# Kuuro-neko/HAI719-Raytracing

Measured on AMD Instinct MI355X. Metric: Msamples/s (pixels x spp / s), Cornell+mesh 1080p@256spp, higher is better.
Workload: dtype f32

## Files before the change

hai719-raytracing_amd/__init__.py:

```python
from __future__ import annotations

import ctypes as C
import os
from typing import Optional

import numpy as np

_HERE = os.path.dirname(os.path.abspath(__file__))
REPO_ROOT = os.path.dirname(_HERE)
ASSET_ROOT = os.path.join(REPO_ROOT, "assets")
TILE = 8

FLAG_GAMMA = 1
FLAG_NO_LDS_TREE = 2
FLAG_WAVE_KERNEL = 4
FLAG_STREAM_KERNEL = 8
FLAG_NO_SHADOW_CULL = 16
FLAG_DUAL_KERNEL = 32
FLAG_EXACT_ONLY = 64
FLAG_MESH_BRUTE = 128

MAT_DIFFUSE, MAT_GLASS, MAT_MIRROR = 0, 1, 2
TEX_NONE, TEX_CHECKER, TEX_IMAGE = 0, 1, 2

# ... 309 lines not shown
        self._check(self._lib.hrt_host_scene_set_skybox(self._h, a.shape[1], a.shape[0], a.ctypes.data))

    def set_sky(self, dark: bool):
        self._check(self._lib.hrt_host_scene_set_sky(self._h, int(dark)))

    def set_kd_params(self, leaf_max: int = 0, max_depth: int = 0):
        self._check(self._lib.hrt_host_scene_set_kd_params(self._h, leaf_max, max_depth))

    def set_kd_builder(self, fn=None, user=None):
        if fn == "gpu":
            fn = C.cast(device_lib().hrt_kd_build_gpu, C.c_void_p)
        elif fn is not None and not isinstance(fn, (int, C.c_void_p)):
            self._kd_builder_keepalive = fn
            fn = C.cast(fn, C.c_void_p)
        self._check(self._lib.hrt_host_scene_set_kd_builder(self._h, fn, user))
        return self

    def flatten(self) -> C.c_void_p:
        d = SceneDescPtr()
        self._check(self._lib.hrt_host_scene_flatten(self._h, C.byref(d)))
        d._owner = self
        return d

    def kd_stats(self, mesh: int = 0) -> dict:
        out = (C.c_uint32 * 6)()
        self._check(self._lib.hrt_host_scene_kd_stats(self._h, mesh, out))
        keys = ["inner", "leaves", "empty_leaves", "depth", "leaf_tri_refs", "units"]
        return dict(zip(keys, list(out)))


def _irregular_stats(self, mesh: int = 0) -> dict:
    out = (C.c_uint32 * 8)()
    self._check(self._lib.hrt_host_scene_irregular_stats(self._h, mesh, out))
    return dict(zip(["out_of_tree", "slivers", "dropped", "pairs", "ref_leaves", "ref_depth", "dead", "entries"], list(out)))


HostScene.irregular_stats = _irregular_stats


def default_camera(aspect: float) -> Camera:
    cam = Camera()
    host_lib().hrt_host_default_camera(aspect, C.byref(cam))
    return cam


_inited = False


def init(device: int = 0):
    global _inited
    lib = device_lib()
    rc = lib.hrt_init(device)
    if rc < 0:
        raise HrtError(f"hrt_init({device}) failed ({rc}): {lib.hrt_last_error().decode()}")
    _inited = True


class DeviceScene:

    def __init__(self, desc: C.c_void_p):
        self._lib = device_lib()
        if not _inited:
            init(int(os.environ.get("LOCAL_RANK", "0")))
        self._h = C.c_void_p()
        self._check(self._lib.hrt_scene_create(desc, C.byref(self._h)))

    def _check(self, rc: int):
        if rc < 0:
            raise HrtError(f"hrt error {rc}: {self._lib.hrt_last_error().decode()}")
        return rc

    def close(self):
        if self._h:
            self._lib.hrt_scene_destroy(self._h)
            self._h = C.c_void_p()

    def __del__(self):
        try:
            self.close()
        except Exception:
            pass

    def render(self, cam: Camera, w: int, h: int, spp: int, seed: int = 1, flags: int = 0):
        out = np.empty((h, w, 3), dtype=np.float32)
        st = Stats()
        self._check(self._lib.hrt_render(self._h, C.byref(cam), w, h, spp, seed, flags, out.ctypes.data, C.byref(st)))
        return out, st

    def last_kernel(self) -> str:
        name = C.create_string_buffer(64)
        self._check(self._lib.hrt_debug_last_kernel(self._h, name, len(name)))
        return name.value.decode()

    def render_tiles(self, cam: Camera, w: int, h: int, spp: int, seed: int, flags: int, rank: int, world: int,
                     d_tiles_ptr: int, stream_ptr: int = 0):
        self._check(self._lib.hrt_render_tiles(self._h, C.byref(cam), w, h, spp, seed, flags, rank, world,
                                               C.c_void_p(d_tiles_ptr), C.c_void_p(stream_ptr)))

    def render_accumulate(self, cam: Camera, w: int, h: int, first_sample: int, n_samples: int, seed: int, flags: int,
                          rank: int, world: int, d_sum_tiles_ptr: int, stream_ptr: int = 0):
        self._check(self._lib.hrt_render_accumulate(self._h, C.byref(cam), w, h, first_sample, n_samples, seed, flags, rank,
                                                    world, C.c_void_p(d_sum_tiles_ptr), C.c_void_p(stream_ptr)))

    def render_adaptive(self, cam: Camera, w: int, h: int, min_spp: int, max_spp: int, threshold: float, seed: int = 1,
                        flags: int = 0, stats: Optional[Stats] = None):
        out = np.empty((h, w, 3), dtype=np.float32)
        spp = np.empty(((h + TILE - 1) // TILE, (w + TILE - 1) // TILE), dtype=np.uint32)
        p = Adaptive(min_spp, max_spp, threshold)
        self._check(self._lib.hrt_render_adaptive(self._h, C.byref(cam), w, h, C.byref(p), seed, flags, out.ctypes.data,
                                                   spp.ctypes.data, None if stats is None else C.byref(stats)))
        return out, spp

    def render_adaptive_tiles(self, cam: Camera, w: int, h: int, min_spp: int, max_spp: int, threshold: float, seed: int,
                              flags: int, rank: int, world: int, d_tiles_ptr: int, d_tile_spp_ptr: int, stream_ptr: int = 0):
        p = Adaptive(min_spp, max_spp, threshold)
        self._check(self._lib.hrt_render_adaptive_tiles(self._h, C.byref(cam), w, h, C.byref(p), seed, flags, rank, world,
                                                        C.c_void_p(d_tiles_ptr), C.c_void_p(d_tile_spp_ptr), C.c_void_p(stream_ptr)))

    def render_features(self, cam: Camera, w: int, h: int, first_sample: int, n_samples: int, seed: int = 1) -> np.ndarray:
        import torch
        d = torch.empty((h, w, FEATURE_FLOATS), dtype=torch.float32, device="cuda")
        s = torch.cuda.current_stream()
        self._check(self._lib.hrt_render_features(self._h, C.byref(cam), w, h, first_sample, n_samples, seed, C.c_void_p(d.data_ptr()),
                                                  C.c_void_p(s.cuda_stream)))
        s.synchronize()
        return d.cpu().numpy()

    def render_denoised(self, cam: Camera, w: int, h: int, spp: int, feature_spp: int, seed: int = 1, flags: int = 0,
                        params: Optional[DenoiseParams] = None, stats: Optional[Stats] = None) -> np.ndarray:
        out = np.empty((h, w, 3), dtype=np.float32)
        p = DenoiseParams() if params is None else params
        self._check(self._lib.hrt_render_denoised(self._h, C.byref(cam), w, h, spp, feature_spp, seed, flags, C.byref(p), out.ctypes.data,
                                                  None if stats is None else C.byref(stats)))
        return out

    def render_denoised_var(self, cam: Camera, w: int, h: int, spp: int, feature_spp: int, seed: int = 1, flags: int = 0,
                            params: Optional[DenoiseVarParams] = None, stats: Optional[Stats] = None, variance: bool = False):
        out = np.empty((h, w, 3), dtype=np.float32)
        var = np.empty((h, w), dtype=np.float32) if variance else None
        p = DenoiseVarParams() if params is None else params
        self._check(self._lib.hrt_render_denoised_var(self._h, C.byref(cam), w, h, spp, feature_spp, seed, flags, C.byref(p),
                                                      out.ctypes.data, None if var is None else var.ctypes.data,
                                                      None if stats is None else C.byref(stats)))
        return (out, var) if variance else out

    def render_temporal(self, history: "History", cam: Camera, w: int, h: int, spp: int, feature_spp: int, seed: int = 1, flags: int = 0,
                        tparams: Optional[TemporalParams] = None, dparams: Optional[DenoiseVarParams] = None,
                        stats: Optional[Stats] = None):
        out = np.empty((h, w, 3), dtype=np.float32)
        hist = np.empty((h, w), dtype=np.float32)
        tp = TemporalParams() if tparams is None else tparams
        self._check(self._lib.hrt_render_temporal(self._h, history._h, C.byref(cam), w, h, spp, feature_spp, seed, flags, C.byref(tp),
                                                  None if dparams is None else C.byref(dparams), out.ctypes.data, hist.ctypes.data,
                                                  None if stats is None else C.byref(stats)))
        return out, hist

    def trace_rays(self, rays, mode: str = "closest", flags: int = 0, normalize: bool = False):
        import torch
        if mode not in _QUERY_MODES:
            raise ValueError(f"trace_rays: mode must be one of {sorted(_QUERY_MODES)} (got {mode!r})")
        q = _QUERY_MODES[mode]
        flags = int(flags) | (RAYS_NORMALIZE if normalize else 0)
        is_torch = isinstance(rays, torch.Tensor)
        if is_torch:
            if (rays.device.type != "cuda" or rays.dtype != torch.float32 or rays.dim() != 2 or rays.shape[1] != RAY_FLOATS
                    or not rays.is_contiguous()):
                raise ValueError("trace_rays: a torch tensor must be a contiguous (n, 8) float32 tensor on the GPU")
            d_rays = rays
        else:
            a = np.ascontiguousarray(rays, dtype=np.float32)
            if a.ndim != 2 or a.shape[1] != RAY_FLOATS:
                raise ValueError(f"trace_rays: rays must have shape (n, {RAY_FLOATS}) (got {a.shape})")
            d_rays = torch.from_numpy(a).to("cuda")
        n, dev = d_rays.shape[0], d_rays.device
        if n > 0x7FFFFFFF:
            raise ValueError(f"trace_rays: at most 2^31 - 1 rays per call (got {n})")
        if q == QUERY_OCCLUDED:
            out = torch.empty((n,), dtype=torch.int32, device=dev)
        else:
            out = torch.empty((n, SHADE_FLOATS if q == QUERY_SHADE else CLOSEST_FLOATS), dtype=torch.float32, device=dev)
        s = torch.cuda.current_stream(dev)
        self._check(self._lib.hrt_trace_rays(self._h, C.c_void_p(d_rays.data_ptr()), n, q, flags, C.c_void_p(out.data_ptr()),
                                             C.c_void_p(s.cuda_stream)))
        if is_torch:
            return out
        r = out.cpu().numpy()
        return r.view(np.uint32) if q == QUERY_OCCLUDED else r

    def trace_radiance(self, rays, spp: int = 1, first_sample: int = 0, seed: int = 1, keys=None, out=None, accumulate: bool = False,
                       flags: int = 0, normalize: bool = False):
        import torch
        flags = int(flags) | (RAYS_NORMALIZE if normalize else 0) | (RADIANCE_ACCUMULATE if accumulate else 0)
        is_torch = isinstance(rays, torch.Tensor)
        if is_torch:
            if (rays.device.type != "cuda" or rays.dtype != torch.float32 or rays.dim() != 2 or rays.shape[1] != RAY_FLOATS
                    or not rays.is_contiguous()):
                raise ValueError("trace_radiance: a torch tensor must be a contiguous (n, 8) float32 tensor on the GPU")
            d_rays = rays
        else:
            a = np.ascontiguousarray(rays, dtype=np.float32)
            if a.ndim != 2 or a.shape[1] != RAY_FLOATS:
                raise ValueError(f"trace_radiance: rays must have shape (n, {RAY_FLOATS}) (got {a.shape})")
        n = rays.shape[0] if is_torch else a.shape[0]
        if n > 0x7FFFFFFF:
            raise ValueError(f"trace_radiance: at most 2^31 - 1 rays per call (got {n})")
        if keys is not None and not is_torch:
            k = np.ascontiguousarray(keys)
            if k.shape != (n,) or k.dtype not in (np.uint32, np.int32):
                raise ValueError(f"trace_radiance: keys must be (n,) uint32 (got {k.shape} {k.dtype})")
        if not is_torch:
            d_rays = torch.from_numpy(a).to("cuda")
        dev = d_rays.device
        d_keys = None
        if keys is not None:
            if is_torch:
                if (not isinstance(keys, torch.Tensor) or keys.device != dev or keys.dtype not in (torch.int32, torch.uint32)
                        or keys.shape != (n,) or not keys.is_contiguous()):
                    raise ValueError("trace_radiance: keys must be a contiguous (n,) int32 tensor on the rays' device")
                d_keys = keys
            else:
                d_keys = torch.from_numpy(k.view(np.int32)).to(dev)
        if out is None:
            if accumulate and first_sample != 0:
                raise ValueError("trace_radiance: accumulate after sample 0 needs the running sums in `out`")
            d_out = torch.zeros((n, 3), dtype=torch.float32, device=dev)
        elif is_torch:
            if (not isinstance(out, torch.Tensor) or out.device != dev or out.dtype != torch.float32 or out.shape != (n, 3)
                    or not out.is_contiguous()):
                raise ValueError("trace_radiance: out must be a contiguous (n, 3) float32 tensor on the rays' device")
            d_out = out
        else:
            o = np.asarray(out)
            if o.shape != (n, 3) or o.dtype != np.float32:
                raise ValueError(f"trace_radiance: out must be (n, 3) float32 (got {o.shape} {o.dtype})")
            d_out = torch.from_numpy(np.ascontiguousarray(o)).to(dev)
        s = torch.cuda.current_stream(dev)
        self._check(self._lib.hrt_trace_radiance(self._h, C.c_void_p(d_rays.data_ptr()),
                                                 None if d_keys is None else C.c_void_p(d_keys.data_ptr()), n, first_sample, spp,
                                                 seed, flags, C.c_void_p(d_out.data_ptr()), C.c_void_p(s.cuda_stream)))
        if is_torch:
            return d_out
        r = d_out.cpu().numpy()
        if out is not None:
            out[...] = r
            return out
        return r

    def render_views(self, cams, w: int, h: int, spp: int, seeds=None, flags: int = 0, out=None, stats: Optional[Stats] = None):
        cams = list(cams)
        n = len(cams)
        seeds = [1] * n if seeds is None else [int(x) for x in seeds]
        if len(seeds) != n:
            raise ValueError(f"render_views: {n} cameras but {len(seeds)} seeds")
        views = (View * max(n, 1))()
        for v, (cam, seed) in enumerate(zip(cams, seeds)):
            views[v].cam = cam
            views[v].seed = seed
        if out is not None:
            import torch
            if (not isinstance(out, torch.Tensor) or out.device.type != "cuda" or out.dtype != torch.float32
                    or tuple(out.shape) != (n, h, w, 3) or not out.is_contiguous()):
                raise ValueError(f"render_views: out must be a contiguous ({n}, {h}, {w}, 3) float32 tensor on the GPU")
            s = torch.cuda.current_stream(out.device)
            self._check(self._lib.hrt_render_views_device(self._h, views, n, w, h, spp, flags, C.c_void_p(out.data_ptr()),
                                                          C.c_void_p(s.cuda_stream)))
            return out
        frames = np.empty((n, h, w, 3), dtype=np.float32)
        self._check(self._lib.hrt_render_views(self._h, views, n, w, h, spp, flags, frames.ctypes.data,
                                               None if stats is None else C.byref(stats)))
        return frames

    def check_last_launch(self):
        self._check(self._lib.hrt_check_last_launch(self._h))

    def last_kernel_ms(self) -> float:
        ms = C.c_double()
        self._check(self._lib.hrt_last_kernel_ms(self._h, C.byref(ms)))
        return ms.value


class History:

    def __init__(self, scene: DeviceScene):
        self._lib = scene._lib
        self._scene = scene
        self._h = C.c_void_p()
        scene._check(self._lib.hrt_history_create(scene._h, C.byref(self._h)))

    def reset(self):
        self._lib.hrt_history_reset(self._h)

    def close(self):
        if self._h:
            self._lib.hrt_history_destroy(self._h)
            self._h = C.c_void_p()

    def __del__(self):
        try:
            self.close()
        except Exception:
            pass


KAT_CAMERA, KAT_TRIANGLE, KAT_AABB, KAT_SPHERE, KAT_QUAD, KAT_OPTICS, KAT_NORMALIZE = range(7)
_KAT_IN = {KAT_CAMERA: 2, KAT_TRIANGLE: 7, KAT_AABB: 7, KAT_SPHERE: 7, KAT_QUAD: 7, KAT_OPTICS: 8, KAT_NORMALIZE: 3}
_KAT_OUT = {KAT_CAMERA: 12, KAT_TRIANGLE: 8, KAT_AABB: 2, KAT_SPHERE: 9, KAT_QUAD: 8, KAT_OPTICS: 8, KAT_NORMALIZE: 3}


def pick_kernel(n_meshes: int, n_lights: int, n_spheres: int, tab_rows: int, tiles: int, spp: int, flags: int = 0, has_list: bool = False,
                n_views: int = 0, kernel: str = "") -> str:
    lib = device_lib()
    name = C.create_string_buffer(64)
    rc = lib.hrt_debug_pick_kernel(C.byref(PickInput(n_meshes, n_lights, n_spheres, tab_rows, tiles, spp, flags, int(has_list), n_views,
                                                     kernel.encode())), name, len(name))
    if rc < 0:
        raise HrtError(f"hrt_debug_pick_kernel failed ({rc}): {lib.hrt_last_error().decode()}")
    return name.value.decode()


def debug_kat(which: int, inp, prim=None, cam: Optional[Camera] = None) -> np.ndarray:
    lib = device_lib()
    a = np.ascontiguousarray(inp, dtype=np.float32).reshape(-1, _KAT_IN[which])
    out = np.empty((a.shape[0], _KAT_OUT[which]), dtype=np.float32)
    pr = None if prim is None else np.ascontiguousarray(prim, dtype=np.float32)
    rc = lib.hrt_debug_kat(which, None if cam is None else C.byref(cam), None if pr is None else pr.ctypes.data, a.ctypes.data,
                           a.shape[0], out.ctypes.data)
    if rc < 0:
        raise HrtError(f"hrt_debug_kat failed ({rc}): {lib.hrt_last_error().decode()}")
    return out


class MultiScene:

    def __init__(self, desc: C.c_void_p, devices):
        global _inited
        self._lib = device_lib()
        self._h = C.c_void_p()
        arr = (C.c_int * len(devices))(*devices)
        rc = self._lib.hrt_multi_create(desc, len(devices), arr, C.byref(self._h))
        if rc < 0:
            raise HrtError(f"hrt error {rc}: {self._lib.hrt_last_error().decode()}")
        self.note = self._lib.hrt_last_error().decode()
        _inited = True

    @property
    def gather(self) -> str:
        return self._lib.hrt_multi_gather(self._h).decode()

    def close(self):
        if self._h:
            self._lib.hrt_multi_destroy(self._h)
            self._h = C.c_void_p()

    def __del__(self):
        try:
            self.close()
        except Exception:
            pass

    def render(self, cam: Camera, w: int, h: int, spp: int, seed: int = 1, flags: int = 0):
        out = np.empty((h, w, 3), dtype=np.float32)
        st = Stats()
        rc = self._lib.hrt_multi_render(self._h, C.byref(cam), w, h, spp, seed, flags, out.ctypes.data, C.byref(st))
        if rc < 0:
            raise HrtError(f"hrt error {rc}: {self._lib.hrt_last_error().decode()}")
        return out, st


def render_multi(desc, cam: Camera, w: int, h: int, spp: int, seed: int, flags: int, devices):
    lib = device_lib()
    out = np.empty((h, w, 3), dtype=np.float32)
    st = Stats()
    arr = (C.c_int * len(devices))(*devices)
    rc = lib.hrt_render_multi(desc, C.byref(cam), w, h, spp, seed, flags, len(devices), arr, out.ctypes.data, C.byref(st))
    if rc < 0:
        raise HrtError(f"hrt error {rc}: {lib.hrt_last_error().decode()}")
    return out, st


def camera_rays(cam: Camera, w: int, h: int, sample: int = 0, seed: int = 1):
    import torch
    lib = device_lib()
    out = torch.empty((w * h, RAY_FLOATS), dtype=torch.float32, device="cuda")
    rc = lib.hrt_camera_rays(C.byref(cam), w, h, sample, seed, C.c_void_p(out.data_ptr()),
                             C.c_void_p(torch.cuda.current_stream().cuda_stream))
    if rc < 0:
        raise HrtError(f"hrt_camera_rays failed ({rc}): {lib.hrt_last_error().decode()}")
    return out


def tiles_total(w: int, h: int) -> int:
    return ((w + TILE - 1) // TILE) * ((h + TILE - 1) // TILE)


def tiles_owned(w: int, h: int, rank: int, world: int) -> int:
    t = tiles_total(w, h)
    return (t - rank + world - 1) // world if rank < t else 0


def assemble_frame(d_gathered_ptr: int, tiles_per_rank_padded: int, w: int, h: int, world: int, d_frame_ptr: int,
                   stream_ptr: int = 0):
    lib = device_lib()
    rc = lib.hrt_assemble_frame(C.c_void_p(d_gathered_ptr), tiles_per_rank_padded, w, h, world,
                                C.c_void_p(d_frame_ptr), C.c_void_p(stream_ptr))
    if rc < 0:
        raise HrtError(f"hrt_assemble_frame failed ({rc}): {lib.hrt_last_error().decode()}")


def assemble_frame_host(gathered: np.ndarray, w: int, h: int, world: int) -> np.ndarray:
    tx = (w + TILE - 1) // TILE
    frame = np.zeros((h, w, 3), dtype=np.float32)
    for t in range(tiles_total(w, h)):
        rank, slot = t % world, t // world
        x0, y0 = (t % tx) * TILE, (t // tx) * TILE
        tile = gathered[rank, slot].reshape(TILE, TILE, 3)
        hh, ww = min(TILE, h - y0), min(TILE, w - x0)
        frame[y0:y0 + hh, x0:x0 + ww] = tile[:hh, :ww]
    return frame


def finalize_tiles(d_sum_tiles_ptr: int, n_tiles: int, total_samples: int, flags: int, d_tiles_ptr: int, stream_ptr: int = 0):
    lib = device_lib()
    rc = lib.hrt_finalize_tiles(C.c_void_p(d_sum_tiles_ptr), n_tiles, total_samples, flags, C.c_void_p(d_tiles_ptr),
                                C.c_void_p(stream_ptr))
    if rc < 0:
        raise HrtError(f"hrt_finalize_tiles failed ({rc}): {lib.hrt_last_error().decode()}")


def denoise_scratch_bytes(w: int, h: int) -> int:
    return int(device_lib().hrt_denoise_scratch_bytes(w, h))


def denoise(d_color_ptr: int, d_features_ptr: int, w: int, h: int, params: Optional[DenoiseParams], flags: int, d_scratch_ptr: int,
            d_out_ptr: int, stream_ptr: int = 0):
    lib = device_lib()
    p = DenoiseParams() if params is None else params
    rc = lib.hrt_denoise(C.c_void_p(d_color_ptr), C.c_void_p(d_features_ptr), w, h, C.byref(p), flags, C.c_void_p(d_scratch_ptr),
                         C.c_void_p(d_out_ptr), C.c_void_p(stream_ptr))
    if rc < 0:
        raise HrtError(f"hrt_denoise failed ({rc}): {lib.hrt_last_error().decode()}")


def denoise_var_scratch_bytes(w: int, h: int) -> int:
    return int(device_lib().hrt_denoise_var_scratch_bytes(w, h))


def denoise_var(d_color_ptr: int, d_color_half_ptr: int, d_features_ptr: int, w: int, h: int, params: Optional[DenoiseVarParams],
                flags: int, d_scratch_ptr: int, d_out_ptr: int, d_variance_out_ptr: int = 0, stream_ptr: int = 0):
    lib = device_lib()
    p = DenoiseVarParams() if params is None else params
    rc = lib.hrt_denoise_var(C.c_void_p(d_color_ptr), C.c_void_p(d_color_half_ptr), C.c_void_p(d_features_ptr), w, h, C.byref(p), flags,
                             C.c_void_p(d_scratch_ptr), C.c_void_p(d_out_ptr), C.c_void_p(d_variance_out_ptr), C.c_void_p(stream_ptr))
    if rc < 0:
        raise HrtError(f"hrt_denoise_var failed ({rc}): {lib.hrt_last_error().decode()}")


def temporal_accumulate(cam: Camera, prev_cam: Optional[Camera], w: int, h: int, d_color_ptr: int, d_color_half_ptr: int, d_features_ptr: int,
                        d_prev_color_ptr: int, d_prev_color_half_ptr: int, d_prev_features_ptr: int, d_prev_history_ptr: int,
                        params: Optional[TemporalParams], d_out_ptr: int, d_out_half_ptr: int, d_history_out_ptr: int, stream_ptr: int = 0):
    lib = device_lib()
    p = TemporalParams() if params is None else params
    ptr = lambda v: C.c_void_p(v) if v else None
    rc = lib.hrt_temporal_accumulate(C.byref(cam), None if prev_cam is None else C.byref(prev_cam), w, h, ptr(d_color_ptr),
                                     ptr(d_color_half_ptr), ptr(d_features_ptr), ptr(d_prev_color_ptr), ptr(d_prev_color_half_ptr),
                                     ptr(d_prev_features_ptr), ptr(d_prev_history_ptr), C.byref(p), ptr(d_out_ptr), ptr(d_out_half_ptr),
                                     ptr(d_history_out_ptr), C.c_void_p(stream_ptr))
    if rc < 0:
        raise HrtError(f"hrt_temporal_accumulate failed ({rc}): {lib.hrt_last_error().decode()}")


def encode_ppm(d_frame_ptr: int, w: int, h: int, fmt: int, d_out_ptr: int, capacity: int, stream_ptr: int = 0) -> int:
    lib = device_lib()
    n = C.c_size_t(0)
    rc = lib.hrt_encode_ppm(C.c_void_p(d_frame_ptr), w, h, fmt, C.c_void_p(d_out_ptr), capacity, C.byref(n), C.c_void_p(stream_ptr))
    if rc < 0:
        raise HrtError(f"hrt_encode_ppm failed ({rc}): {lib.hrt_last_error().decode()}")
    return int(n.value)


def ppm_text_reference(rgb: np.ndarray) -> bytes:
    rgb = np.ascontiguousarray(rgb, dtype=np.float32)
    h, w, _ = rgb.shape
    m = np.where(rgb < np.float32(1.0), rgb, np.float32(1.0))
    v = (np.float32(255.0) * m).astype(np.float32)
    with np.errstate(invalid="ignore"):
        iv = np.where(np.isfinite(v), np.trunc(np.clip(v, -2147483648.0, 255.0)), -2147483648.0).astype(np.int64)
    body = " ".join(str(int(x)) for x in iv.reshape(-1))
    return f"P3\n{w} {h}\n255\n".encode() + body.encode() + b" \n"


def write_ppm(path: str, rgb: np.ndarray):
    rgb = np.ascontiguousarray(rgb, dtype=np.float32)
    lib = device_lib()
    rc = lib.hrt_write_ppm(path.encode(), rgb.ctypes.data, rgb.shape[1], rgb.shape[0])
    if rc < 0:
        raise HrtError(f"hrt_write_ppm failed ({rc}): {lib.hrt_last_error().decode()}")
```

hai719-raytracing_amd/csrc/hrt_api.hip:

```cpp
#include "hrt_kernels.hip"
#include "hrt_dual.hip"
#include "hrt_stream.hip"
#include "hrt_output.hip"
#include "hrt_kat.hip"

#include <dlfcn.h>
#include <rccl/rccl.h>

#include <array>
#include <cfloat>
#include <chrono>
#include <cmath>
#include <cstdio>
#include <cstdlib>
#include <cstddef>
#include <cstring>
#include <functional>
#include <new>
#include <string>
#include <thread>
#include <unordered_map>
#include <vector>

namespace {
// ... 139 lines not shown
            for (int c = 1; c < 3; ++c) if (std::fabs(n[c]) > std::fabs(n[k])) k = c;
            const int a = (k + 1) % 3, b = (k + 2) % 3;
            eps_n = std::fabs(n[a]) + std::fabs(n[b]) + std::fabs(1.0 - std::fabs(n[k]));
            const double dev_ab = (std::fabs(R[k]) + std::fabs(R[b])) / lenR + (std::fabs(U[k]) + std::fabs(U[a])) / lenU;
            const double dev_ba = (std::fabs(R[k]) + std::fabs(R[a])) / lenR + (std::fabs(U[k]) + std::fabs(U[b])) / lenU;
            eps_e = std::min(dev_ab, dev_ba);
            if (eps_n <= 1e-4 && eps_e <= 1e-4 && std::isfinite(eps_n) && std::isfinite(eps_e)) { K = k; ra = dev_ab <= dev_ba ? a : b; }
        }
        if (K >= 0) {
            const int a = (K + 1) % 3, b = (K + 2) % 3;
            (void)ra;
            double lo[3] = {INFINITY, INFINITY, INFINITY}, hi[3] = {-INFINITY, -INFINITY, -INFINITY};
            for (int c = 0; c < 4; ++c)
                for (int x = 0; x < 3; ++x) {
                    const double v = p0[x] + ((c & 1) ? R[x] : 0.0) + ((c & 2) ? U[x] : 0.0);
                    lo[x] = std::min(lo[x], v); hi[x] = std::max(hi[x], v);
                }
            const double widen = (2.0 * eps_e + 2e-6) * (lenR + lenU);
            auto centre = [&](int x) { return (float)(0.5 * (lo[x] + hi[x])); };
            auto half = [&](int x) { return std::nextafter((float)(0.5 * (hi[x] - lo[x]) + widen + 2.4e-7 * (std::fabs(lo[x]) + std::fabs(hi[x]))), INFINITY); };
            const float sgn = n[K] < 0.0 ? -1.f : 1.f;
            const float par = (float)(8.0 * (eps_n + 4e-7));
            const float cq = (float)(2.5e6 * (eps_n + 3e-7));
            const uint32_t bits = ((flags & HRT_QUAD_FLAG_GLASS) ? 1u : 0u) | (sgn < 0.f ? 2u : 0u) | (i << 8);
            sec[K].push_back(make_float4(sgn * q[0].w, centre(a), centre(b), half(a)));
            sec[K].push_back(make_float4(half(b), as_float(bits), par, cq));
            ++count[K];
        } else {
            sec[3].push_back(make_float4(q[0].x, q[0].y, q[0].z, q[0].w));
            sec[3].push_back(make_float4(q[1].y, q[1].z, q[1].x, as_float(flags | (i << 8))));
            sec[3].push_back(make_float4(q[2].x, q[3].x, q[2].y, q[3].y));
            sec[3].push_back(make_float4(q[2].z, q[3].z, q[2].w, q[3].w));
            ++count[3];
        }
    }
    qf.clear();
    for (int k = 0; k < 4; ++k) qf.insert(qf.end(), sec[k].begin(), sec[k].end());
}

void fold_triangle(const H3 c[3], uint32_t id, std::vector<float4> &tris, std::vector<float4> &planes) {
    const H3 e1 = h_sub(c[1], c[0]), e2 = h_sub(c[2], c[0]);
    const H3 nn = h_cross(e1, e2);
    const float norm = h_len(nn);
    const H3 n{nn.x / norm, nn.y / norm, nn.z / norm};
    const float d00 = h_dot(e1, e1), d01 = h_dot(e1, e2), d11 = h_dot(e2, e2);
    const float denom = h_msub(d00, d11, d01, d01);
    planes.push_back(make_float4(n.x, n.y, n.z, h_dot(c[0], n)));
    (void)denom;
    tris.push_back(make_float4(c[0].x, c[0].y, c[0].z, d11));
    tris.push_back(make_float4(e1.x, e1.y, e1.z, d00));
    tris.push_back(make_float4(e2.x, e2.y, e2.z, d01));
    tris.push_back(make_float4(as_float(id), 0.f, 0.f, 0.f));
}

template <class T>
int upload(const std::vector<T> &v, T **dptr) {
    *dptr = nullptr;
    size_t bytes = std::max<size_t>(v.size(), 1) * sizeof(T);
    HIP_TRY(hipMalloc((void **)dptr, bytes));
    if (!v.empty()) HIP_TRY(hipMemcpy(*dptr, v.data(), v.size() * sizeof(T), hipMemcpyHostToDevice));
    return HRT_OK;
}

struct Scratch {
    void *p = nullptr;
    size_t cap = 0;
    template <class T> T *as() const { return (T *)p; }
    void release() {
        if (p) (void)hipFree(p);
        p = nullptr; cap = 0;
    }
    int grow(size_t bytes) {
        if (cap >= bytes) return HRT_OK;
        release();
        HIP_TRY(hipMalloc(&p, bytes));
        cap = bytes;
        return HRT_OK;
    }
};

int check_frame(const std::string &who, uint32_t w, uint32_t h, uint64_t max_pixels) {
    if (!w || !h) return fail(HRT_ERR_INVALID, who + ": w and h must be positive (got " + std::to_string(w) + " x " + std::to_string(h) + ")");
    if ((uint64_t)w * h > max_pixels) return fail(HRT_ERR_INVALID, who + ": image too large: w * h must be at most " + std::to_string(max_pixels));
    return HRT_OK;
}
const uint64_t k_max_pixels = 0x7fffffffull, k_max_records = 0x7fffffffull / 16u;

__host__ __device__ __forceinline__ float margin_scale(float bound, float olen) { return 2e-6f * (bound + olen + 1.f); }

int check_mesh_brute(const std::string &who, uint32_t flags) {
    if ((flags & HRT_FLAG_MESH_BRUTE) && !(flags & HRT_FLAG_EXACT_ONLY)) return fail(HRT_ERR_INVALID, who + ": flags: HRT_FLAG_MESH_BRUTE needs HRT_FLAG_EXACT_ONLY");
    return HRT_OK;
}

enum KernelFamily { KF_LANE, KF_DUAL, KF_STREAM };
enum : uint32_t { KB_LIGHTS = 1u, KB_EXACT = 2u, KB_SPH = 4u, KB_LIST = 8u, KB_VIEWS = 16u };
struct KernelBuild {
    KernelFamily family; uint32_t bits; void (*fn)(const DRender); const char *name;
    uint32_t wg() const { return family == KF_STREAM ? HRT_SP_WG : HRT_WG; }
};
#define HRT_BUILD(k, family, bits) {family, bits, k, #k}
const KernelBuild k_builds[] = {
    HRT_BUILD(hrt_trace_kernel, KF_LANE, 0u),
    HRT_BUILD(hrt_trace_kernel_lights, KF_LANE, KB_LIGHTS),
    HRT_BUILD(hrt_trace_kernel_exact, KF_LANE, KB_EXACT),
    HRT_BUILD(hrt_trace_kernel_lights_exact, KF_LANE, KB_LIGHTS | KB_EXACT),
    HRT_BUILD(hrt_trace_kernel_list, KF_LANE, KB_LIST),
    HRT_BUILD(hrt_trace_kernel_lights_list, KF_LANE, KB_LIGHTS | KB_LIST),
    HRT_BUILD(hrt_trace_kernel_exact_list, KF_LANE, KB_EXACT | KB_LIST),
    HRT_BUILD(hrt_trace_kernel_lights_exact_list, KF_LANE, KB_LIGHTS | KB_EXACT | KB_LIST),
    HRT_BUILD(hrt_trace_kernel_views, KF_LANE, KB_VIEWS),
    HRT_BUILD(hrt_trace_kernel_lights_views, KF_LANE, KB_LIGHTS | KB_VIEWS),
    HRT_BUILD(hrt_trace2_kernel, KF_DUAL, 0u),
    HRT_BUILD(hrt_trace2_kernel_lights, KF_DUAL, KB_LIGHTS),
    HRT_BUILD(hrt_trace2_kernel_list, KF_DUAL, KB_LIST),
    HRT_BUILD(hrt_trace2_kernel_lights_list, KF_DUAL, KB_LIGHTS | KB_LIST),
    HRT_BUILD(hrt_wgstream_kernel, KF_STREAM, 0u),
    HRT_BUILD(hrt_wgstream_kernel_lights, KF_STREAM, KB_LIGHTS),
    HRT_BUILD(hrt_wgstream_kernel_sph, KF_STREAM, KB_SPH),
    HRT_BUILD(hrt_wgstream_kernel_lights_sph, KF_STREAM, KB_LIGHTS | KB_SPH),
    HRT_BUILD(hrt_wgstream_kernel_exact, KF_STREAM, KB_EXACT),
    HRT_BUILD(hrt_wgstream_kernel_lights_exact, KF_STREAM, KB_LIGHTS | KB_EXACT),
    HRT_BUILD(hrt_wgstream_kernel_list, KF_STREAM, KB_LIST),
    HRT_BUILD(hrt_wgstream_kernel_lights_list, KF_STREAM, KB_LIGHTS | KB_LIST),
    HRT_BUILD(hrt_wgstream_kernel_sph_list, KF_STREAM, KB_SPH | KB_LIST),
    HRT_BUILD(hrt_wgstream_kernel_lights_sph_list, KF_STREAM, KB_LIGHTS | KB_SPH | KB_LIST),
    HRT_BUILD(hrt_wgstream_kernel_exact_list, KF_STREAM, KB_EXACT | KB_LIST),
    HRT_BUILD(hrt_wgstream_kernel_lights_exact_list, KF_STREAM, KB_LIGHTS | KB_EXACT | KB_LIST),
    HRT_BUILD(hrt_wgstream_kernel_views, KF_STREAM, KB_VIEWS),
    HRT_BUILD(hrt_wgstream_kernel_lights_views, KF_STREAM, KB_LIGHTS | KB_VIEWS),
    HRT_BUILD(hrt_wgstream_kernel_sph_views, KF_STREAM, KB_SPH | KB_VIEWS),
    HRT_BUILD(hrt_wgstream_kernel_lights_sph_views, KF_STREAM, KB_LIGHTS | KB_SPH | KB_VIEWS),
};

int pick_build(const hrt_pick_input &in, KernelPref pref, const KernelBuild *&row) {
    const uint32_t flags = in.flags;
    const bool stream_fits = (size_t)in.tab_rows * 16u <= 48u * 1024u;
    if ((flags & HRT_FLAG_STREAM_KERNEL) && !stream_fits)
        return fail(HRT_ERR_INVALID, "render: the scene's object tables exceed the 48 KiB the streaming kernel keeps in LDS; use another kernel form");
    const bool stream_pays = in.n_meshes > 0u || in.n_lights > 0u || (in.tiles <= 5120u && in.spp >= 8u);
    const bool stream = stream_fits && !(flags & (HRT_FLAG_WAVE_KERNEL | HRT_FLAG_DUAL_KERNEL)) &&
                        (pref.use_stream == 1 || (flags & HRT_FLAG_STREAM_KERNEL) || (pref.use_stream < 0 && stream_pays));
    const bool exact = (flags & HRT_FLAG_EXACT_ONLY) != 0u;
    if (const int rc = check_mesh_brute("render", flags)) return rc;
    if (exact && (flags & HRT_FLAG_DUAL_KERNEL)) return fail(HRT_ERR_INVALID, "render: no exact-only build of the two-stream kernel");
    const bool dual = !exact && !stream && !in.n_views && (pref.use_dual || (flags & HRT_FLAG_DUAL_KERNEL)) && in.n_meshes > 0u &&
                      !(flags & HRT_FLAG_WAVE_KERNEL);
    const KernelFamily family = stream ? KF_STREAM : (dual ? KF_DUAL : KF_LANE);
    const bool sph = stream && !exact && in.n_spheres >= HRT_SPHERE_FILTER_MIN && in.n_spheres <= 128u;
    const uint32_t bits = (in.n_lights ? KB_LIGHTS : 0u) | (exact ? KB_EXACT : 0u) | (sph ? KB_SPH : 0u) | (in.has_list ? KB_LIST : 0u) |
                          (in.n_views ? KB_VIEWS : 0u);
    for (const KernelBuild &b : k_builds)
        if (b.family == family && b.bits == bits) { row = &b; return HRT_OK; }
    return fail(HRT_ERR_INVALID, std::string("render: there is no build of the ") + (stream ? "streaming" : dual ? "two-stream" : "lane-per-pixel") + " kernel for" +
                                 (in.n_views ? " batched views" : "") + (in.has_list ? " with a tile list" : "") + (exact ? " with HRT_FLAG_EXACT_ONLY" : ""));
}

}

struct hrt_scene {
    DScene d{};
    DScene *d_scene = nullptr;
    DCamera *d_cam = nullptr;
    DCamera *d_cam_aov = nullptr;
    DCamera h_cam{};
    bool cam_valid = false;
    uint32_t lds_units = 0;
    uint32_t max_leaf = 0;
    std::vector<void *> allocations;
    uint32_t *tile_counter = nullptr;
    unsigned long long *stamps = nullptr;
    hipEvent_t ev0 = nullptr, ev1 = nullptr;
    bool timed = false;
    float bound = 0.f;
    Scratch sp_scratch, sp_pool, tiles, frame, ad_compact, ad_words, dn_frame, dn_feat, dn_scratch, dn_out, dnv_half_tiles, dnv_frame_half, dnv_var;
    std::array<Scratch *, 13> scratch() { return {&sp_scratch, &sp_pool, &tiles, &frame, &ad_compact, &ad_words, &dn_frame, &dn_feat, &dn_scratch, &dn_out, &dnv_half_tiles, &dnv_frame_half, &dnv_var}; }
    uint32_t last_grid = 0, last_waves = 0, last_lds = 0;
    const KernelBuild *last_build = nullptr;
    hipStream_t last_stream = nullptr;
    int device = 0;
    DCamera *d_cam_feat = nullptr;
    DCamera h_cam_feat{};
    hipEvent_t ev_feat = nullptr;
    bool feat_used = false;
    hipStream_t feat_stream = nullptr;
    Scratch vw_blocks, vw_tiles, vw_frames;
    DView *h_views = nullptr;
    size_t h_views_cap = 0;
    hipEvent_t ev_views = nullptr, ev_views_done = nullptr;
    bool views_uploading = false, views_used = false;
    hipStream_t views_stream = nullptr;
};

namespace {

int enter_scene(const std::string &who, hrt_scene *s, bool switch_device = true) {
    if (!s) return fail(HRT_ERR_INVALID, who + ": scene is NULL");
    if (!g_rt.ready) return fail(HRT_ERR_STATE, who + ": call hrt_init first");
    return switch_device ? use_device(s->device) : HRT_OK;
}
int enter_render(const std::string &who, hrt_scene *s, const hrt_camera *cam) {
    if (!cam) return fail(HRT_ERR_INVALID, who + ": camera is NULL");
    return enter_scene(who, s);
}

void fill_stats(const hrt_scene *s, hrt_stats *stats, std::chrono::steady_clock::time_point t0, double kernel_ms, uint64_t samples) {
    std::memset(stats, 0, sizeof(*stats));
    stats->kernel_ms = kernel_ms;
    stats->total_ms = std::chrono::duration<double, std::milli>(std::chrono::steady_clock::now() - t0).count();
    stats->samples = samples;
    stats->vgprs = (uint32_t)g_rt.attr.numRegs;
    stats->lds_bytes = s->last_lds;
    stats->waves_launched = s->last_waves;
}

}

#include "hrt_kdbuild.hip"

extern "C" {

const char *hrt_last_error(void) { return g_error.c_str(); }

int hrt_device_count(void) {
    int n = 0;
    if (hipGetDeviceCount(&n) != hipSuccess) return 0;
    return n;
}

int hrt_init(int device_ordinal) {
    int n = 0;
    HIP_TRY(hipGetDeviceCount(&n));
    if (n <= 0) return fail(HRT_ERR_DEVICE, "hrt_init: no HIP device");
    if (device_ordinal < 0 || device_ordinal >= n) return fail(HRT_ERR_INVALID, "hrt_init: device ordinal out of range");
    HIP_TRY(hipSetDevice(device_ordinal));
    hipDeviceProp_t prop;
    HIP_TRY(hipGetDeviceProperties(&prop, device_ordinal));
    g_rt.device = device_ordinal;
    g_rt.cus = prop.multiProcessorCount;
    if ((int)g_rt.dev_cus.size() < n) g_rt.dev_cus.resize((size_t)n, 0);
    if (g_rt.dev_cus[device_ordinal] != 0) { g_rt.ready = true; return HRT_OK; }
    HIP_TRY(hipFuncGetAttributes(&g_rt.attr, (const void *)hrt_trace_kernel));
    uint32_t kb = 36u * (HRT_WG / 256u);
    if (const char *e = std::getenv("HRT_LDS_KB")) kb = (uint32_t)std::max(0, atoi(e));
    if (kb > 160) kb = 160;
    g_rt.lds_budget = kb * 1024u;
    const uint32_t raise[] = {g_rt.lds_budget > 64u * 1024u ? g_rt.lds_budget : 0u, HRT_WG > 256 ? 160u * 1024u : 0u, 160u * 1024u};
    for (const KernelBuild &b : k_builds)
        if (raise[b.family]) HIP_TRY(hipFuncSetAttribute((const void *)b.fn, hipFuncAttributeMaxDynamicSharedMemorySize, (int)raise[b.family]));
    {
        float lut[512];
        for (int c = 0; c < 256; ++c) { lut[c] = (float)(c / 255.); lut[256 + c] = (float)(c / 127.5 - 1.); }
        HIP_TRY(hipMemcpyToSymbol(HIP_SYMBOL(c_u8_lut), lut, sizeof(lut)));
    }
    g_rt.pref = parse_kernel_pref(std::getenv("HRT_KERNEL"));
    g_rt.dev_cus[device_ordinal] = prop.multiProcessorCount;
    g_rt.ready = true;
    return HRT_OK;
}

void hrt_shutdown(void) { g_rt.ready = false; g_rt.dev_cus.clear(); }

void hrt_scene_destroy(hrt_scene *s) {
    if (!s) return;
    if (g_rt.ready) (void)use_device(s->device);
    for (void *p : s->allocations) (void)hipFree(p);
    if (s->tile_counter) (void)hipFree(s->tile_counter);
    if (s->stamps) (void)hipFree(s->stamps);
    if (s->d_scene) (void)hipFree(s->d_scene);
    if (s->d_cam) (void)hipFree(s->d_cam);
    if (s->d_cam_aov) (void)hipFree(s->d_cam_aov);
    for (Scratch *b : s->scratch()) b->release();
    if (s->d_cam_feat) (void)hipFree(s->d_cam_feat);
    if (s->ev_feat) (void)hipEventDestroy(s->ev_feat);
    for (Scratch *b : {&s->vw_blocks, &s->vw_tiles, &s->vw_frames}) b->release();
    if (s->h_views) (void)hipHostFree(s->h_views);
    if (s->ev_views) (void)hipEventDestroy(s->ev_views);
    if (s->ev_views_done) (void)hipEventDestroy(s->ev_views_done);
    if (s->ev0) (void)hipEventDestroy(s->ev0);
    if (s->ev1) (void)hipEventDestroy(s->ev1);
    delete s;
}

static int scene_create_impl(const hrt_scene_desc *desc, hrt_scene *s) {
    const hrt_scene_desc &D = *desc;
    for (uint32_t i = 0; i < D.n_materials; ++i) {
        const hrt_material &m = D.materials[i];
        if (m.image >= (int32_t)D.n_images || m.normal_map >= (int32_t)D.n_images)
            return fail(HRT_ERR_INVALID, "material references an image that does not exist");
        if (m.type < 0 || m.type > 2 || m.texture_type < 0 || m.texture_type > 2)
            return fail(HRT_ERR_INVALID, "material type / texture type out of range");
        if (m.normal_map >= 0 && (D.images[m.normal_map].w < 1 || D.images[m.normal_map].h < 1))
            return fail(HRT_ERR_INVALID, "normal map image is empty");
    }
    for (uint32_t i = 0; i < D.n_spheres; ++i)
        if (D.spheres[i].material < 0 || (uint32_t)D.spheres[i].material >= D.n_materials)
            return fail(HRT_ERR_INVALID, "sphere material out of range");
    for (uint32_t i = 0; i < D.n_quads; ++i)
        if (D.quads[i].material < 0 || (uint32_t)D.quads[i].material >= D.n_materials)
            return fail(HRT_ERR_INVALID, "quad material out of range");
    if (D.skybox_image >= (int32_t)D.n_images) return fail(HRT_ERR_INVALID, "skybox image out of range");
    if (D.n_lights && !D.lights) return fail(HRT_ERR_INVALID, "lights missing");
    if (D.n_meshes > 32u) return fail(HRT_ERR_INVALID, "more than 32 meshes in one scene (the parked-mesh mask is 32 bits)");

    {
        double b = 0.0;
        auto grow = [&](double x, double y, double z, double extra) { b = std::max(b, std::sqrt(x * x + y * y + z * z) + extra); };
        auto mlen = [&](const hrt_material &m) { return std::sqrt((double)m.motion[0] * m.motion[0] + (double)m.motion[1] * m.motion[1] + (double)m.motion[2] * m.motion[2]); };
        for (uint32_t i = 0; i < D.n_spheres; ++i) {
            const hrt_sphere &sp = D.spheres[i];
            grow(sp.center[0], sp.center[1], sp.center[2], std::fabs((double)sp.radius) + mlen(D.materials[sp.material]));
        }
        for (uint32_t i = 0; i < D.n_quads; ++i) {
            const hrt_quad &q = D.quads[i];
            const double ml = mlen(D.materials[q.material]);
            grow(q.v0[0], q.v0[1], q.v0[2], ml);
            grow(q.v1[0], q.v1[1], q.v1[2], ml);
            grow(q.v3[0], q.v3[1], q.v3[2], ml);
            grow((double)q.v1[0] + q.v3[0] - q.v0[0], (double)q.v1[1] + q.v3[1] - q.v0[1], (double)q.v1[2] + q.v3[2] - q.v0[2], ml);
        }
        for (uint32_t mi = 0; mi < D.n_meshes; ++mi)
            for (uint32_t v = 0; v < D.meshes[mi].n_vertices; ++v) {
                const float *p = D.meshes[mi].positions + 3 * (size_t)v;
                grow(p[0] * 1.00001, p[1] * 1.00001, p[2] * 1.00001, 0.0);
            }
        for (uint32_t i = 0; i < D.n_lights; ++i) grow(D.lights[i].pos[0], D.lights[i].pos[1], D.lights[i].pos[2], std::fabs((double)D.lights[i].radius));
        s->bound = (float)b;
    }

    std::vector<float4> spheres, quads, mats, lights;
    for (uint32_t i = 0; i < D.n_spheres; ++i) {
        const hrt_sphere &sp = D.spheres[i];
        const hrt_material &m = D.materials[sp.material];
        spheres.push_back(make_float4(sp.center[0], sp.center[1], sp.center[2], sp.radius));
        spheres.push_back(make_float4(m.motion[0], m.motion[1], m.motion[2], as_float((uint32_t)sp.material)));
    }
    for (uint32_t i = 0; i < D.n_quads; ++i) {
        const hrt_quad &q = D.quads[i];
        const hrt_material &m = D.materials[q.material];
        fold_quad(q, m, quads);
    }
    std::vector<float4> qfilter;
    build_quad_filter(quads, D.n_quads, qfilter, s->d.qf_n);
    std::vector<float4> sfilter;
    {
        const uint32_t ns = D.n_spheres, pairs = (ns + 1u) / 2u;
        for (uint32_t p = 0; p < pairs; ++p) {
            const uint32_t a = 2u * p, b = std::min(2u * p + 1u, ns - 1u);
            const float4 a0 = spheres[2u * a], a1 = spheres[2u * a + 1u], b0 = spheres[2u * b], b1 = spheres[2u * b + 1u];
            sfilter.push_back(make_float4(a0.x, b0.x, a0.y, b0.y));
            sfilter.push_back(make_float4(a0.z, b0.z, a0.w * a0.w, b0.w * b0.w));
            sfilter.push_back(make_float4(a1.x, b1.x, a1.y, b1.y));
            sfilter.push_back(make_float4(a1.z, b1.z, std::fabs(a0.w), std::fabs(b0.w)));
        }
        s->d.sf_pairs = pairs;
        s->d.sf_psize = std::max(1u, (pairs + 63u) / 64u);
    }
    for (uint32_t i = 0; i < D.n_lights; ++i) {
        const hrt_light &l = D.lights[i];
        lights.push_back(make_float4(l.pos[0], l.pos[1], l.pos[2], l.radius));
        lights.push_back(make_float4(l.color[0], l.color[1], l.color[2], 0.f));
    }
    for (uint32_t i = 0; i < D.n_materials; ++i) {
        const hrt_material &m = D.materials[i];
        mats.push_back(make_float4(m.albedo[0], m.albedo[1], m.albedo[2], m.transparency));
        mats.push_back(make_float4(m.index_medium, as_float((uint32_t)m.type), as_float((uint32_t)m.texture_type),
                                   as_float((uint32_t)(m.emissive ? 1 : 0))));
        mats.push_back(make_float4(m.checker1[0], m.checker1[1], m.checker1[2], m.tex_scale_x));
        mats.push_back(make_float4(m.checker2[0], m.checker2[1], m.checker2[2], m.tex_scale_y));
        mats.push_back(make_float4(m.light_color[0], m.light_color[1], m.light_color[2], m.light_intensity));
        mats.push_back(make_float4(as_float((uint32_t)m.image), as_float((uint32_t)m.normal_map), 0.f, 0.f));
        mats.push_back(make_float4(0.f, 0.f, 0.f, 0.f));
        mats.push_back(make_float4(0.f, 0.f, 0.f, 0.f));
    }

    std::vector<DImage> images;
    std::vector<uint32_t> texels;
    for (uint32_t i = 0; i < D.n_images; ++i) {
        const hrt_image &im = D.images[i];
        DImage di;
        di.offset = (uint32_t)texels.size();
        di.w = im.w; di.h = im.h; di.pad = 0;
        if (im.w >= 1 && im.h >= 1) {
            if (!im.rgb) return fail(HRT_ERR_INVALID, "image without pixels");
            const size_t n = (size_t)im.w * im.h;
            for (size_t p = 0; p < n; ++p)
                texels.push_back((uint32_t)im.rgb[3 * p] | ((uint32_t)im.rgb[3 * p + 1] << 8) | ((uint32_t)im.rgb[3 * p + 2] << 16));
        }
        images.push_back(di);
    }

    for (uint32_t i = 0; i < D.n_materials; ++i) {
        const hrt_material &m = D.materials[i];
        if (m.image >= 0) mats[(size_t)HRT_MAT_ROWS * i + 6] = make_float4(as_float(images[m.image].offset), as_float((uint32_t)images[m.image].w), as_float((uint32_t)images[m.image].h), 0.f);
        if (m.normal_map >= 0) mats[(size_t)HRT_MAT_ROWS * i + 7] = make_float4(as_float(images[m.normal_map].offset), as_float((uint32_t)images[m.normal_map].w), as_float((uint32_t)images[m.normal_map].h), 0.f);
    }

    std::vector<DMesh> meshes;
    std::vector<uint4> units;
    std::vector<float4> tris, planes, colors, exceptions;
    std::vector<uint4> vids;
    for (uint32_t mi = 0; mi < D.n_meshes; ++mi) {
        const hrt_mesh &M = D.meshes[mi];
        if (M.material < 0 || (uint32_t)M.material >= D.n_materials) return fail(HRT_ERR_INVALID, "mesh material out of range");
        for (uint32_t k = 0; k < 3 * M.n_triangles; ++k)
            if (M.indices[k] >= M.n_vertices) return fail(HRT_ERR_INVALID, "mesh vertex index out of range");
        if (M.n_leaf_tris && (M.kd_root == HRT_KD_NIL || !M.kd_units || !M.n_kd_units))
            return fail(HRT_ERR_INVALID, "mesh has triangles but no flattened KD-tree");
        if (M.n_exceptions && !M.exceptions) return fail(HRT_ERR_INVALID, "mesh exceptions missing");
        DMesh dm;
        std::memset(&dm, 0, sizeof(dm));
        for (int a = 0; a < 3; ++a) {
            dm.aabb_lo[a] = M.aabb_min[a]; dm.aabb_hi[a] = M.aabb_max[a];
            dm.kd_lo[a] = M.kd_min[a]; dm.kd_hi[a] = M.kd_max[a];
        }
        units.resize((units.size() + 3u) & ~(size_t)3u, make_uint4(0, 0, 0, 0));
        const uint32_t unit_base = (uint32_t)units.size();
        const uint32_t tri_base = (uint32_t)(tris.size() / HRT_TRI_ROWS);
        auto in_range = [&](uint32_t ref) -> bool {
            if (ref == HRT_KD_NIL) return true;
            const uint32_t idx = ref & ~HRT_KD_LEAF;
            return (uint64_t)idx + ((ref & HRT_KD_LEAF) ? 4u : 1u) <= M.n_kd_units;
        };
        if (M.n_leaf_tris) {
            if (M.kd_root == HRT_KD_NIL || !in_range(M.kd_root)) return fail(HRT_ERR_INVALID, "malformed flattened KD-tree");
            std::vector<uint8_t> reached(M.n_kd_units, 0);
            {
                std::vector<uint32_t> stack{M.kd_root};
                reached[M.kd_root & ~HRT_KD_LEAF] = (M.kd_root & HRT_KD_LEAF) ? 2 : 1;
                while (!stack.empty()) {
                    const uint32_t ref = stack.back();
                    stack.pop_back();
                    if (ref & HRT_KD_LEAF) continue;
                    const hrt_kdunit &u = M.kd_units[ref];
                    for (int c = 2; c < 4; ++c) {
                        const uint32_t child = u.w[c];
                        if (child == HRT_KD_NIL || !in_range(child) || reached[child & ~HRT_KD_LEAF]) return fail(HRT_ERR_INVALID, "malformed flattened KD-tree (a nodelet is reached twice through child links)");
                        reached[child & ~HRT_KD_LEAF] = (child & HRT_KD_LEAF) ? 2 : 1;
                        stack.push_back(child);
                    }
                }
            }
            std::vector<uint32_t> new_of(M.n_kd_units, 0xFFFFFFFFu);
            std::vector<uint32_t> order;
            uint32_t cur = 0;
            bool ok = true;
            auto want = [&](uint32_t ref) {
                if (ref == HRT_KD_NIL) return;
                if (!in_range(ref)) { ok = false; return; }
                const uint32_t idx = ref & ~HRT_KD_LEAF;
                if (reached[idx] != ((ref & HRT_KD_LEAF) ? 2 : 1)) { ok = false; return; }
                if (new_of[idx] != 0xFFFFFFFFu) return;
                const uint32_t size = (ref & HRT_KD_LEAF) ? 4u : 2u;
                cur = (cur + size - 1u) & ~(size - 1u);
                new_of[idx] = cur;
                cur += size;
                order.push_back(ref);
            };
            auto inner_ok = [&](const hrt_kdunit &u) { return u.w[1] <= 2u && u.w[2] != HRT_KD_NIL && u.w[3] != HRT_KD_NIL && in_range(u.w[2]) && in_range(u.w[3]); };
            want(M.kd_root);
            for (size_t q = 0; ok && q < order.size(); ++q) {
                const uint32_t ref = order[q], idx = ref & ~HRT_KD_LEAF;
                const hrt_kdunit *u = M.kd_units + idx;
                if (ref & HRT_KD_LEAF) {
                    if ((uint64_t)u[0].w[3] + u[1].w[3] > M.n_leaf_tris) { ok = false; break; }
                    if (u[1].w[3] >= 0xFFFFu) return fail(HRT_ERR_INVALID, "KD leaf with 65535 or more triangles (the resumable walk keeps a 16-bit leaf cursor): build the tree with a smaller leaf_max");
                    s->max_leaf = std::max(s->max_leaf, u[1].w[3]);
                    for (int f = 0; f < 4; ++f) want(u[2].w[f]);
                    want(u[3].w[0]);
                    want(u[3].w[1]);
                } else {
                    if (!inner_ok(*u)) { ok = false; break; }
                    for (int c = 0; c < 2 && ok; ++c) {
                        const uint32_t child = u->w[2 + c];
                        if (child & HRT_KD_LEAF) { want(child); continue; }
                        const hrt_kdunit &y = M.kd_units[child];
                        if (!inner_ok(y)) { ok = false; break; }
                        want(y.w[2]);
                        want(y.w[3]);
                    }
                }
            }
            if (!ok) return fail(HRT_ERR_INVALID, "malformed flattened KD-tree (a link or rope names a unit that is not a nodelet of this tree, or not of that kind)");
            auto tr = [&](uint32_t ref) -> uint32_t { return ref == HRT_KD_NIL ? ref : ((new_of[ref & ~HRT_KD_LEAF] + unit_base) | (ref & HRT_KD_LEAF)); };
            units.resize(unit_base + ((cur + 3u) & ~3u), make_uint4(0, 0, 0, 0));
            for (uint32_t ref : order) {
                const uint32_t idx = ref & ~HRT_KD_LEAF;
                const hrt_kdunit *u = M.kd_units + idx;
                uint4 *o = &units[unit_base + new_of[idx]];
                if (ref & HRT_KD_LEAF) {
                    o[0] = make_uint4(u[0].w[0], u[0].w[1], u[0].w[2], u[0].w[3]);
                    o[1] = make_uint4(u[1].w[0], u[1].w[1], u[1].w[2], u[1].w[3]);
                    o[2] = make_uint4(tr(u[2].w[0]), tr(u[2].w[1]), tr(u[2].w[2]), tr(u[2].w[3]));
                    o[3] = make_uint4(tr(u[3].w[0]), tr(u[3].w[1]), 0, 0);
                } else {
                    uint32_t split[2] = {0, 0}, axis[2] = {3, 3}, exits[4];
                    for (int c = 0; c < 2; ++c) {
                        const uint32_t child = u->w[2 + c];
                        if (child & HRT_KD_LEAF) {
                            exits[2 * c] = exits[2 * c + 1] = tr(child);
                        } else {
                            const hrt_kdunit &y = M.kd_units[child];
                            split[c] = y.w[0]; axis[c] = y.w[1];
                            exits[2 * c] = tr(y.w[2]); exits[2 * c + 1] = tr(y.w[3]);
                        }
                    }
                    o[0] = make_uint4(u->w[0], split[0], split[1], u->w[1] | (axis[0] << 2) | (axis[1] << 4));
                    o[1] = make_uint4(exits[0], exits[1], exits[2], exits[3]);
                }
            }
            dm.root = tr(M.kd_root);
        } else {
            dm.root = HRT_KD_NIL;
        }
        auto push_triangle = [&](uint32_t t) {
            H3 c[3];
            for (int j = 0; j < 3; ++j) {
                const float *p = M.positions + 3 * (size_t)M.indices[3 * (size_t)t + j];
                c[j] = H3{p[0] * HRT_TRIANGLE_SCALING, p[1] * HRT_TRIANGLE_SCALING, p[2] * HRT_TRIANGLE_SCALING};
            }
            fold_triangle(c, t, tris, planes);
        };
        for (uint32_t k = 0; k < M.n_leaf_tris; ++k) {
            const uint32_t t = M.leaf_tris[k];
            if (t >= M.n_triangles) return fail(HRT_ERR_INVALID, "leaf triangle id out of range");
            push_triangle(t);
        }
        dm.tri_base = tri_base;
        dm.n_soup = M.n_leaf_tris;
        dm.exc_base = (uint32_t)(exceptions.size() / 2);
        dm.n_exc = 0;
        if (M.n_exceptions) {
            struct Group { float lo[3], hi[3]; uint32_t tri; std::vector<std::array<float, 7>> boxes; };
            std::vector<Group> groups;
            {
                std::vector<uint32_t> order(M.n_exceptions);
                for (uint32_t k = 0; k < M.n_exceptions; ++k) {
                    if (M.exceptions[k].triangle >= M.n_triangles) return fail(HRT_ERR_INVALID, "exception triangle id out of range");
                    order[k] = k;
                }
                static_assert(offsetof(hrt_tri_exception, box_max) == offsetof(hrt_tri_exception, box_min) + 12, "box_min and box_max are contiguous");
                auto box_cmp = [&](uint32_t x, uint32_t y) { return std::memcmp(M.exceptions[x].box_min, M.exceptions[y].box_min, 24); };
                std::stable_sort(order.begin(), order.end(), [&](uint32_t x, uint32_t y) {
                    const hrt_tri_exception &ex = M.exceptions[x], &ey = M.exceptions[y];
                    return ex.triangle < ey.triangle || (ex.triangle == ey.triangle && ex.group < ey.group);
                });
                for (size_t q = 0; q < order.size(); ++q) {
                    const hrt_tri_exception &e = M.exceptions[order[q]];
                    const bool same_tri = !groups.empty() && groups.back().tri == e.triangle;
                    const bool same_leaf = same_tri && q > 0 && M.exceptions[order[q - 1]].group == e.group;
                    if (!same_tri) {
                        groups.emplace_back();
                        groups.back().tri = e.triangle;
                    }
                    if (same_leaf && box_cmp(order[q - 1], order[q]) == 0) continue;
                    if (!same_leaf && !groups.back().boxes.empty()) groups.back().boxes.back()[6] = 1.f;
                    std::array<float, 7> bx;
                    std::memcpy(bx.data(), e.box_min, 24);
                    bx[6] = 0.f;
                    groups.back().boxes.push_back(bx);
                }
                for (Group &g : groups) g.boxes.back()[6] = 1.f;
                for (Group &g : groups) {
                    double c[3][3];
                    for (int j = 0; j < 3; ++j) {
                        const float *pp = M.positions + 3 * (size_t)M.indices[3 * (size_t)g.tri + j];
                        for (int a = 0; a < 3; ++a) c[j][a] = (double)(pp[a] * HRT_TRIANGLE_SCALING);
                    }
                    double e1[3], e2[3], cr[3];
                    for (int a = 0; a < 3; ++a) { e1[a] = c[1][a] - c[0][a]; e2[a] = c[2][a] - c[0][a]; }
                    cr[0] = e1[1] * e2[2] - e1[2] * e2[1]; cr[1] = e1[2] * e2[0] - e1[0] * e2[2]; cr[2] = e1[0] * e2[1] - e1[1] * e2[0];
                    const double l1 = e1[0] * e1[0] + e1[1] * e1[1] + e1[2] * e1[2], l2 = e2[0] * e2[0] + e2[1] * e2[1] + e2[2] * e2[2];
                    const double sin2 = (cr[0] * cr[0] + cr[1] * cr[1] + cr[2] * cr[2]) / (l1 * l2);
                    const bool own_bounds = std::isfinite(sin2) && sin2 >= 1e-2;
                    for (int a = 0; a < 3; ++a) {
                        double lo = INFINITY, hi = -INFINITY;
                        if (own_bounds) {
                            for (int j = 0; j < 3; ++j) { lo = std::min(lo, c[j][a]); hi = std::max(hi, c[j][a]); }
                        } else {
                            for (const auto &bx : g.boxes) {
                                lo = std::min(lo, (double)std::min(bx[a], bx[3 + a])); hi = std::max(hi, (double)std::max(bx[a], bx[3 + a]));
                            }
                        }
                        double ext = 0.0;
                        for (int x = 0; x < 3; ++x) ext = std::max(ext, std::max(std::fabs(e1[x]), std::fabs(e2[x])));
                        const double pad = (own_bounds ? 1e-3 * ext : 0.0) + 1e-4 * std::max(1.0, std::max(std::fabs(lo), std::fabs(hi)));
                        g.lo[a] = (float)(lo - pad); g.hi[a] = (float)(hi + pad);
                    }
                }
            }
            const size_t first_entry = exceptions.size() / 2;
            struct Emit {
                std::vector<Group> &g;
                std::vector<float4> &out;
                std::vector<float4> &tris;
                const std::function<void(uint32_t)> &push_triangle;
                size_t first_entry;
                void run(size_t lo, size_t hi) {
                    if (hi - lo == 1) {
                        const Group &b = g[lo];
                        const uint32_t slot = (uint32_t)(tris.size() / HRT_TRI_ROWS);
                        push_triangle(b.tri);
                        out.push_back(make_float4(b.lo[0], b.lo[1], b.lo[2], as_float(slot)));
                        out.push_back(make_float4(b.hi[0], b.hi[1], b.hi[2], as_float((uint32_t)b.boxes.size())));
                        for (const auto &bx : b.boxes) {
                            out.push_back(make_float4(bx[0], bx[1], bx[2], as_float(bx[6] != 0.f ? 1u : 0u)));
                            out.push_back(make_float4(bx[3], bx[4], bx[5], 0.f));
                        }
                        return;
                    }
                    float bmin[3] = {INFINITY, INFINITY, INFINITY}, bmax[3] = {-INFINITY, -INFINITY, -INFINITY};
                    float cmin[3] = {INFINITY, INFINITY, INFINITY}, cmax[3] = {-INFINITY, -INFINITY, -INFINITY};
                    for (size_t i = lo; i < hi; ++i)
                        for (int a = 0; a < 3; ++a) {
                            bmin[a] = std::min(bmin[a], g[i].lo[a]); bmax[a] = std::max(bmax[a], g[i].hi[a]);
                            const float c = 0.5f * (g[i].lo[a] + g[i].hi[a]);
                            cmin[a] = std::min(cmin[a], c); cmax[a] = std::max(cmax[a], c);
                        }
                    int axis = 0;
                    for (int a = 1; a < 3; ++a) if (cmax[a] - cmin[a] > cmax[axis] - cmin[axis]) axis = a;
                    const size_t mid = lo + (hi - lo) / 2;
                    std::nth_element(g.begin() + lo, g.begin() + mid, g.begin() + hi, [axis](const Group &x, const Group &y) {
                        const float cx = x.lo[axis] + x.hi[axis], cy = y.lo[axis] + y.hi[axis];
                        return cx < cy || (cx == cy && x.tri < y.tri);
                    });
                    const size_t self = out.size();
                    float pmin[3], pmax[3];
                    for (int a = 0; a < 3; ++a) {
                        const float pad = 1e-4f * std::max(1.f, std::max(std::fabs(bmin[a]), std::fabs(bmax[a])));
                        pmin[a] = bmin[a] - pad; pmax[a] = bmax[a] + pad;
                    }
                    out.push_back(make_float4(pmin[0], pmin[1], pmin[2], as_float(HRT_EXC_INNER)));
                    out.push_back(make_float4(pmax[0], pmax[1], pmax[2], 0.f));
                    run(lo, mid);
                    run(mid, hi);
                    out[self + 1].w = as_float((uint32_t)(out.size() / 2 - first_entry));
                }
            };
            const std::function<void(uint32_t)> pt = push_triangle;
            Emit em{groups, exceptions, tris, pt, first_entry};
            em.run(0, groups.size());
            dm.n_exc = (uint32_t)(exceptions.size() / 2 - first_entry);
        }
        dm.material = (uint32_t)M.material;
        dm.color_type = HRT_COLOR_NONE;
        if (M.color_type == HRT_COLOR_FACE && M.face_colors) {
            dm.color_type = HRT_COLOR_FACE;
            dm.color_base = (uint32_t)colors.size();
            for (uint32_t t = 0; t < M.n_triangles; ++t)
                colors.push_back(make_float4(M.face_colors[3 * t], M.face_colors[3 * t + 1], M.face_colors[3 * t + 2], 0.f));
        } else if (M.color_type == HRT_COLOR_VERTEX && M.vert_colors) {
            dm.color_type = HRT_COLOR_VERTEX;
            dm.vcolor_base = (uint32_t)colors.size();
            for (uint32_t v = 0; v < M.n_vertices; ++v)
                colors.push_back(make_float4(M.vert_colors[3 * v], M.vert_colors[3 * v + 1], M.vert_colors[3 * v + 2], 0.f));
            dm.color_base = (uint32_t)vids.size();
            for (uint32_t t = 0; t < M.n_triangles; ++t)
                vids.push_back(make_uint4(M.indices[3 * t], M.indices[3 * t + 1], M.indices[3 * t + 2], 0));
        }
        meshes.push_back(dm);
    }

    DScene &d = s->d;
    float4 *p4 = nullptr;
    int rc;
#define UP(vec, field, type)                                     \
    {                                                            \
        type *ptr = nullptr;                                     \
        if ((rc = upload(vec, &ptr)) != HRT_OK) return rc;       \
        s->allocations.push_back(ptr);                           \
        d.field = ptr;                                           \
    }
    (void)p4;
    {
        static_assert(sizeof(DMesh) % sizeof(float4) == 0, "mesh records are whole rows");
        std::vector<float4> tabs;
        d.tab_quads = 0;
        tabs.insert(tabs.end(), quads.begin(), quads.end());
        d.tab_mats = (uint32_t)tabs.size();
        tabs.insert(tabs.end(), mats.begin(), mats.end());
        d.tab_spheres = (uint32_t)tabs.size();
        tabs.insert(tabs.end(), spheres.begin(), spheres.end());
        d.tab_meshes = (uint32_t)tabs.size();
        tabs.resize(tabs.size() + meshes.size() * (sizeof(DMesh) / sizeof(float4)));
        if (!meshes.empty()) std::memcpy(&tabs[d.tab_meshes], meshes.data(), meshes.size() * sizeof(DMesh));
        d.tab_sfilter = (uint32_t)tabs.size();
        tabs.insert(tabs.end(), sfilter.begin(), sfilter.end());
        d.tab_exc = (uint32_t)tabs.size();
        d.exc_in_tabs = exceptions.size() <= 1536u ? 1u : 0u;
        if (d.exc_in_tabs) tabs.insert(tabs.end(), exceptions.begin(), exceptions.end());
        d.tab_rows = (uint32_t)tabs.size();
        UP(tabs, tabs, float4)
        d.quads = d.tabs + d.tab_quads;
        d.materials = d.tabs + d.tab_mats;
        d.spheres = d.tabs + d.tab_spheres;
        d.meshes = reinterpret_cast<const DMesh *>(d.tabs + d.tab_meshes);
    }
    UP(qfilter, qfilter, float4)
    UP(units, kd_units, uint4)
    UP(tris, tris, float4)
    UP(planes, tri_planes, float4)
    UP(colors, colors, float4)
    UP(vids, tri_vids, uint4)
    UP(images, images, DImage)
    UP(texels, texels, uint32_t)
    UP(lights, lights, float4)
    UP(exceptions, exceptions, float4)
#undef UP
    d.n_spheres = D.n_spheres; d.n_quads = D.n_quads; d.n_meshes = D.n_meshes; d.n_lights = D.n_lights;
    d.n_images = D.n_images;
    d.n_kd_units = (uint32_t)units.size();
    s->lds_units = std::min<uint32_t>(d.n_kd_units, g_rt.lds_budget / 16u) & ~3u;
    d.dark_sky = D.dark_sky;
    {
        bool finite = true;
        auto mag = [&](float v) { finite = finite && std::isfinite(v); return std::fabs((double)v); };
        auto mag3 = [&](const float *v) { return std::max(mag(v[0]), std::max(mag(v[1]), mag(v[2]))); };
        double albedo = 1.0, emit = 0.0, transmit = 1.0, light = 0.0;
        for (uint32_t i = 0; i < D.n_materials; ++i) {
            const hrt_material &m = D.materials[i];
            const double checker = std::max(mag3(m.checker1), mag3(m.checker2));
            albedo = std::max(albedo, std::max(mag3(m.albedo), checker));
            const double e = std::max(1.0, std::max(mag3(m.light_color), checker)) * mag(m.light_intensity);
            if (m.emissive) emit = std::max(emit, e);
            transmit = std::max(transmit, std::fabs(1.0 - (double)m.transparency));
            finite = finite && std::isfinite(m.transparency);
        }
        for (uint32_t i = 0; i < D.n_lights; ++i) light = std::max(light, mag3(D.lights[i].color));
        for (const float4 &c : colors) albedo = std::max(albedo, std::max(mag(c.x), std::max(mag(c.y), mag(c.z))));
        const double term = std::max(std::max(emit, (double)HRT_MAXBOUNCES + 1.0), (double)D.n_lights * light * albedo * transmit);
        const double bound = std::pow(albedo, (double)HRT_MAXBOUNCES) * term;
        d.prune_ok = (finite && bound < 0.5 * (double)FLT_MAX) ? 1u : 0u;
        if (const char *e = std::getenv("HRT_PRUNE")) if (e[0] == '0') d.prune_ok = 0u;
    }
    d.any_motion = 0u;
    for (uint32_t i = 0; i < D.n_materials; ++i)
        if (!(D.materials[i].motion[0] == 0.f && D.materials[i].motion[1] == 0.f && D.materials[i].motion[2] == 0.f)) d.any_motion = 1u;
    d.skybox_image = (D.skybox_image >= 0 && D.images[D.skybox_image].w >= 1 && D.images[D.skybox_image].h >= 1) ? D.skybox_image : -1;
    HIP_TRY(hipMalloc((void **)&s->tile_counter, sizeof(uint32_t)));
    HIP_TRY(hipMalloc((void **)&s->stamps, 16 * sizeof(unsigned long long)));
    HIP_TRY(hipMemset(s->stamps, 0, 16 * sizeof(unsigned long long)));
    HIP_TRY(hipEventCreate(&s->ev0));
    HIP_TRY(hipEventCreate(&s->ev1));
    HIP_TRY(hipMalloc((void **)&s->d_scene, sizeof(DScene)));
    HIP_TRY(hipMemcpy(s->d_scene, &s->d, sizeof(DScene), hipMemcpyHostToDevice));
    HIP_TRY(hipMalloc((void **)&s->d_cam, sizeof(DCamera)));
    HIP_TRY(hipMalloc((void **)&s->d_cam_aov, sizeof(DCamera)));
    return HRT_OK;
}

int hrt_scene_create(const hrt_scene_desc *desc, hrt_scene **out) {
    if (!desc || !out) return fail(HRT_ERR_INVALID, "hrt_scene_create: NULL argument");
    if (!g_rt.ready) return fail(HRT_ERR_STATE, "hrt_scene_create: call hrt_init first");
    hrt_scene *s = nullptr;
    try {
        s = new hrt_scene();
        s->device = g_rt.device;
        int rc = scene_create_impl(desc, s);
        if (rc != HRT_OK) {
            std::string keep = g_error;
            hrt_scene_destroy(s);
            g_error = keep;
            return rc;
        }
    } catch (const std::exception &e) {
        if (s) hrt_scene_destroy(s);
        return fail(HRT_ERR_STATE, e.what());
    }
    *out = s;
    return HRT_OK;
}

uint32_t hrt_tiles_total(uint32_t w, uint32_t h) { return ((w + HRT_TILE - 1) / HRT_TILE) * ((h + HRT_TILE - 1) / HRT_TILE); }
uint32_t hrt_tiles_owned(uint32_t w, uint32_t h, uint32_t rank, uint32_t world) {
    const uint32_t t = hrt_tiles_total(w, h);
    if (!world || rank >= t) return 0;
    return (t - rank + world - 1) / world;
}

static int make_camera(const hrt_camera *cam, DCamera &C) {
    std::memset(&C, 0, sizeof(C));
    {
        double mv[16], pr[16], mi[16], pi[16];
        for (int k = 0; k < 16; ++k) { mv[k] = 0.0; pr[k] = 0.0; }
        const double Rm[3][3] = {{cam->right[0], cam->right[1], cam->right[2]},
                                 {cam->up[0], cam->up[1], cam->up[2]},
                                 {-(double)cam->forward[0], -(double)cam->forward[1], -(double)cam->forward[2]}};
        for (int r = 0; r < 3; ++r) {
            for (int k = 0; k < 3; ++k) mv[k * 4 + r] = Rm[r][k];
            mv[12 + r] = h_neg_dot3(Rm[r], cam->eye);
        }
        mv[15] = 1.0;
        const double rad = (double)cam->fovy_deg / 2.0 * M_PI / 180.0;
        const double cot = std::cos(rad) / std::sin(rad);
        const double dz = (double)cam->zfar - (double)cam->znear;
        pr[0] = cot / (double)cam->aspect;
        pr[5] = cot;
        pr[10] = -((double)cam->zfar + (double)cam->znear) / dz;
        pr[11] = -1.0;
        pr[14] = h_mul64(h_mul64(-2.0, (double)cam->znear), (double)cam->zfar) / dz;
        if (!host_invert4(mv, mi) || !host_invert4(pr, pi)) return fail(HRT_ERR_INVALID, "render: singular camera matrix");
        static const int p_zero[] = {1, 2, 3, 4, 6, 7, 8, 9, 10, 12, 13}, m_zero[] = {3, 7, 11};
        for (int k : p_zero) if (pi[k] != 0.0) return fail(HRT_ERR_INVALID, "render: projection inverse is not of the gluPerspective form");
        for (int k : m_zero) if (mi[k] != 0.0) return fail(HRT_ERR_INVALID, "render: modelview inverse is not affine");
        bool finite = true;
        for (int k = 0; k < 16; ++k) finite = finite && std::isfinite(mi[k]) && std::isfinite(pi[k]);
        if (!finite) return fail(HRT_ERR_INVALID, "render: camera is not finite");
        const double ri2 = pi[14], ri3 = pi[15];
        for (int a = 0; a < 3; ++a) C.eye[a] = (float)(mi[12 + a] / mi[15]);
        C.pi0 = pi[0]; C.pi5 = pi[5];
        C.pi15 = h_mul64(mi[15], ri3);
        C.inv15 = 1.0 / C.pi15;
        for (int k = 0; k < 3; ++k) {
            C.mx[k] = mi[k];
            C.my[k] = mi[4 + k];
            C.c1[k] = h_mul64(mi[8 + k], ri2);
            C.c2[k] = h_mul64(mi[12 + k], ri3);
        }
    }
    return HRT_OK;
}

static int fill_render(hrt_scene *s, const hrt_camera *cam, uint32_t w, uint32_t h, uint32_t spp, uint64_t seed,
                       uint32_t flags, uint32_t rank, uint32_t world, DRender &R, DCamera &C) {
    const int frc = check_frame("render", w, h, k_max_pixels);
    if (frc != HRT_OK) return frc;
    if (!spp) return fail(HRT_ERR_INVALID, "render: spp must be positive");
    if (w > 65535u || h > 65535u) return fail(HRT_ERR_INVALID, "render: w and h must be below 65536 (tile origins are packed in 16 + 16 bits)");
    if (!world || rank >= world) return fail(HRT_ERR_INVALID, "render: bad rank/world");
    R.scene = s->d_scene;
    R.lds_units = (flags & HRT_FLAG_NO_LDS_TREE) ? 0u : s->lds_units;
    R.err_abs = margin_scale(s->bound, std::sqrt(cam->eye[0] * cam->eye[0] + cam->eye[1] * cam->eye[1] + cam->eye[2] * cam->eye[2]));
    {
        const int crc = make_camera(cam, C);
        if (crc != HRT_OK) return crc;
    }
    R.w = w; R.h = h; R.spp = spp;
    R.seed_lo = (uint32_t)seed; R.seed_hi = (uint32_t)(seed >> 32);
    R.flags = flags;
    R.rank = rank; R.world = world;
    R.tiles_x = (w + HRT_TILE - 1) / HRT_TILE;
    R.tiles_total = hrt_tiles_total(w, h);
    R.tiles_owned = hrt_tiles_owned(w, h, rank, world);
    R.tile_counter = s->tile_counter;
    R.stamps = s->stamps;
    R.tile_list = nullptr;
    return HRT_OK;
}

static int size_stream(hrt_scene *s, const KernelBuild &b, DRender &R, uint32_t &grid, uint32_t &lds_bytes) {
    const uint32_t fixed = (uint32_t)((HRT_SP_GLOBAL ? 0 : SP_FIELDS * HRT_SP_POOL * 4) + HRT_SP_NQ * HRT_SP_POOL * 2 + HRT_SP_STREAMS * sizeof(SpCtl) + sizeof(SpShared) + HRT_SP_UNITS * sizeof(SpUnit) + HRT_SP_UNITS * HRT_SP_MAXG * 4) +
                           ((b.bits & KB_VIEWS) ? HRT_SP_UNITS * HRT_SP_MAXG * 16u : 0u) +
                           2048u + s->d.tab_rows * 16u
#ifdef HRT_WALK_SEG
                           + 2048u
#endif
                           ;
    uint32_t per_cu = (64u * 4u * HRT_SP_MINW) / HRT_SP_WG;
    while (per_cu > 1u && 160u * 1024u / per_cu < fixed + 16u * 1024u) --per_cu;
    const uint32_t room = (160u * 1024u / per_cu - fixed) / 16u;
    if (!(R.flags & HRT_FLAG_NO_LDS_TREE)) R.lds_units = std::min<uint32_t>(s->d.n_kd_units, room) & ~3u;
    lds_bytes = fixed + R.lds_units * 16u;
    grid = std::min<uint32_t>((uint32_t)g_rt.cus * per_cu, R.tiles_owned);
    {
        const uint32_t per_tile = 64u * std::min<uint32_t>(R.spp, HRT_SP_SCHUNK);
        uint32_t glog = 0;
        while ((2u << glog) <= HRT_SP_MAXG && (per_tile << (glog + 1u)) <= HRT_SP_UNIT) ++glog;
        R.sp_group_log2 = glog;
        uint32_t band = 0;
        while (glog == 0u && band < 2u && ((uint64_t)R.tiles_owned << band) < 64ull * grid && (64u >> (band + 1u)) * (uint64_t)std::min<uint32_t>(R.spp, HRT_SP_SCHUNK) >= 4096u) ++band;
        R.sp_band_log2 = band;
    }
    int rc = s->sp_scratch.grow((size_t)grid * HRT_SP_UNITS * HRT_SP_UNIT * 3u * sizeof(float));
    if (rc == HRT_OK && HRT_SP_GLOBAL) rc = s->sp_pool.grow((size_t)grid * SP_FIELDS * HRT_SP_POOL * sizeof(uint32_t));
    if (rc != HRT_OK) return rc;
    R.sp_scratch = s->sp_scratch.as<float>();
    R.sp_pool = s->sp_pool.as<uint32_t>();
    return HRT_OK;
}

static int size_lanes(const KernelBuild &b, DRender &R, uint32_t &grid, uint32_t &lds_bytes) {
    const bool dual = b.family == KF_DUAL;
    lds_bytes = R.lds_units * 16u;
    if (dual) {
        const uint32_t wgs = 1024u / HRT_WG, backup = HRT_DS_FIELDS * HRT_WG * 4u;
        const uint32_t room = (156u * 1024u / wgs - backup) / 16u;
        if (R.lds_units > room) R.lds_units = room & ~3u;
        lds_bytes = R.lds_units * 16u + backup;
    }
    int per_cu = 0;
    HIP_TRY(hipOccupancyMaxActiveBlocksPerMultiprocessor(&per_cu, (const void *)b.fn, HRT_WG, lds_bytes));
    if (per_cu < 1) per_cu = 1;
    grid = (uint32_t)(per_cu * g_rt.cus);
    const uint32_t per_wg = (HRT_WG / 64u) * (dual ? 2u : 1u);
    const uint32_t need = (R.tiles_owned + per_wg - 1u) / per_wg;
    if (grid > need) grid = need;
    R.sp_scratch = nullptr;
    R.sp_pool = nullptr;
    return HRT_OK;
}

struct TraceJob {
    uint32_t w, h, s0, spp;
    uint64_t seed;
    uint32_t flags;
    float *d_tiles;
    void *stream;
    uint32_t rank = 0, world = 1;
    bool accumulate = false;
    const uint32_t *list = nullptr;
    uint32_t list_n = 0;
    uint32_t n_views = 0;
};
static int launch_trace(hrt_scene *s, const hrt_camera *cam, const TraceJob &J) {
    DRender R;
    DCamera C;
    int rc = fill_render(s, cam, J.w, J.h, J.spp, J.seed, J.flags, J.rank, J.world, R, C);
    if (rc != HRT_OK) return rc;
    if (J.list) {
        if (J.list_n > R.tiles_owned) return fail(HRT_ERR_INVALID, "render: tile list longer than the rank's tiles");
        R.tile_list = J.list;
        R.tiles_owned = J.list_n;
    }
    if (J.n_views) {
        R.views = s->vw_blocks.as<DView>();
        R.tiles_owned = J.n_views * R.tiles_total;
    }
    R.cam = s->d_cam;
    if (!J.d_tiles) return fail(HRT_ERR_INVALID, "render: NULL tile buffer");
    if ((uint64_t)J.s0 + J.spp > 0xffffffffull) return fail(HRT_ERR_INVALID, "render: sample index overflows 32 bits");
    R.out_tiles = J.d_tiles;
    R.s0 = J.s0;
    R.accumulate = J.accumulate ? 1u : 0u;
    const bool gamma = (J.flags & HRT_FLAG_GAMMA) && !J.accumulate;
    hipStream_t stream = (hipStream_t)J.stream;
    if (R.tiles_owned == 0) { s->timed = false; return HRT_OK; }
    const KernelBuild *build = nullptr;
    const hrt_pick_input traits{s->d.n_meshes, s->d.n_lights, s->d.n_spheres, s->d.tab_rows, R.tiles_owned, J.spp, J.flags, J.list ? 1u : 0u, J.n_views, nullptr};
    if ((rc = pick_build(traits, g_rt.pref, build)) != HRT_OK) return rc;
    uint32_t grid, lds_bytes;
    rc = build->family == KF_STREAM ? size_stream(s, *build, R, grid, lds_bytes) : size_lanes(*build, R, grid, lds_bytes);
    if (rc != HRT_OK) return rc;
    s->last_grid = grid;
    s->last_lds = lds_bytes;
    s->last_waves = grid * (build->wg() / 64u);
    if (s->timed && s->last_stream != stream) HIP_TRY(hipStreamWaitEvent(stream, s->ev1, 0));
    s->last_stream = stream;
    if (J.n_views) {
        HIP_TRY(hipMemcpyAsync(s->vw_blocks.p, s->h_views, (size_t)J.n_views * sizeof(DView), hipMemcpyHostToDevice, stream));
        HIP_TRY(hipEventRecord(s->ev_views, stream));
        s->views_uploading = true;
    } else if (!s->cam_valid || std::memcmp(&C, &s->h_cam, sizeof(C)) != 0) {
        s->h_cam = C;
        HIP_TRY(hipMemcpyAsync(s->d_cam, &s->h_cam, sizeof(C), hipMemcpyHostToDevice, stream));
        s->cam_valid = true;
    }
    HIP_TRY(hipMemsetAsync(s->tile_counter, 0, sizeof(uint32_t), stream));
    HIP_TRY(hipMemsetAsync(s->stamps, 0, 16 * sizeof(unsigned long long), stream));
    HIP_TRY(hipEventRecord(s->ev0, stream));
    hipLaunchKernelGGL(build->fn, dim3(grid), dim3(build->wg()), lds_bytes, stream, R);
    s->last_build = build;
    HIP_TRY(hipGetLastError());
    HIP_TRY(hipEventRecord(s->ev1, stream));
    if (gamma) {
        const uint32_t n = R.tiles_owned * 64u * 3u;
        hipLaunchKernelGGL(hrt_gamma_kernel, dim3((n + 255) / 256), dim3(256), 0, stream, J.d_tiles, n);
        HIP_TRY(hipGetLastError());
    }
    s->timed = true;
    return HRT_OK;
}

int hrt_render_tiles(hrt_scene *s, const hrt_camera *cam, uint32_t w, uint32_t h, uint32_t spp, uint64_t seed,
                     uint32_t flags, uint32_t rank, uint32_t world, float *d_tiles, void *stream) {
    const int rc = enter_render("hrt_render_tiles", s, cam);
    if (rc != HRT_OK) return rc;
    TraceJob job{w, h, 0u, spp, seed, flags, d_tiles, stream};
    job.rank = rank; job.world = world;
    return launch_trace(s, cam, job);
}

int hrt_render_accumulate(hrt_scene *s, const hrt_camera *cam, uint32_t w, uint32_t h, uint32_t first_sample, uint32_t n_samples,
                          uint64_t seed, uint32_t flags, uint32_t rank, uint32_t world, float *d_sum_tiles, void *stream) {
    const int rc = enter_render("hrt_render_accumulate", s, cam);
    if (rc != HRT_OK) return rc;
    TraceJob job{w, h, first_sample, n_samples, seed, flags, d_sum_tiles, stream};
    job.rank = rank; job.world = world; job.accumulate = true;
    return launch_trace(s, cam, job);
}

int hrt_finalize_tiles(const float *d_sum_tiles, uint32_t n_tiles, uint32_t total_samples, uint32_t flags, float *d_tiles,
                       void *stream_) {
    if (!d_sum_tiles || !d_tiles || !total_samples) return fail(HRT_ERR_INVALID, "hrt_finalize_tiles: bad argument");
    if (!g_rt.ready) return fail(HRT_ERR_STATE, "hrt_finalize_tiles: call hrt_init first");
    if (!n_tiles) return HRT_OK;
    const uint32_t n = n_tiles * 64u * 3u;
    hipLaunchKernelGGL(hrt_finalize_kernel, dim3((n + 255) / 256), dim3(256), 0, (hipStream_t)stream_, d_sum_tiles, d_tiles, n,
                       total_samples, (flags & HRT_FLAG_GAMMA) ? 1u : 0u);
    HIP_TRY(hipGetLastError());
    return HRT_OK;
}

int hrt_encode_ppm(const float *d_frame, uint32_t w, uint32_t h, int format, unsigned char *d_out, size_t capacity,
                   size_t *bytes, void *stream_) {
    if (!d_frame || !d_out || !bytes || !w || !h) return fail(HRT_ERR_INVALID, "hrt_encode_ppm: bad argument");
    if (format != 3 && format != 6) return fail(HRT_ERR_INVALID, "hrt_encode_ppm: format must be 3 (ASCII) or 6 (binary)");
    if (!g_rt.ready) return fail(HRT_ERR_STATE, "hrt_encode_ppm: call hrt_init first");
    { const int frc = check_frame("hrt_encode_ppm", w, h, k_max_records); if (frc != HRT_OK) return frc; }
    hipStream_t stream = (hipStream_t)stream_;
    char head[64];
    const int hl = std::snprintf(head, sizeof(head), "P%d\n%u %u\n255\n", format, w, h);
    const uint32_t npix = w * h;
    if (format == 6) {
        const size_t total = (size_t)hl + (size_t)npix * 3u;
        if (capacity < total) return fail(HRT_ERR_INVALID, "hrt_encode_ppm: output buffer too small (need " + std::to_string(total) + ")");
        HIP_TRY(hipMemcpyAsync(d_out, head, (size_t)hl, hipMemcpyHostToDevice, stream));
        hipLaunchKernelGGL(hrt_ppm6_kernel, dim3((npix * 3u + 255u) / 256u), dim3(256), 0, stream, d_frame, npix * 3u, d_out + hl);
        HIP_TRY(hipGetLastError());
        HIP_TRY(hipStreamSynchronize(stream));
        *bytes = total;
        return HRT_OK;
    }
    const uint32_t nblocks = (npix + 1023u) / 1024u;
    uint32_t *d_len = nullptr;
    HIP_TRY(hipMalloc((void **)&d_len, ((size_t)npix + nblocks) * sizeof(uint32_t)));
    uint32_t *d_block = d_len + npix;
    hipLaunchKernelGGL(hrt_ppm3_measure_kernel, dim3(nblocks), dim3(256), 0, stream, d_frame, npix, d_len, d_block);
    std::vector<uint32_t> block(nblocks);
    hipError_t e = hipMemcpyAsync(block.data(), d_block, nblocks * sizeof(uint32_t), hipMemcpyDeviceToHost, stream);
    if (e == hipSuccess) e = hipStreamSynchronize(stream);
    if (e != hipSuccess) { (void)hipFree(d_len); return fail(HRT_ERR_DEVICE, std::string("hrt_encode_ppm: ") + hipGetErrorString(e)); }
    std::vector<unsigned long long> base(nblocks);
    unsigned long long run = (unsigned long long)hl;
    for (uint32_t b = 0; b < nblocks; ++b) { base[b] = run; run += block[b]; }
    const size_t total = (size_t)run + 1u;
    if (capacity < total) { (void)hipFree(d_len); return fail(HRT_ERR_INVALID, "hrt_encode_ppm: output buffer too small (need " + std::to_string(total) + ")"); }
    unsigned long long *d_base = nullptr;
    e = hipMalloc((void **)&d_base, nblocks * sizeof(unsigned long long));
    if (e == hipSuccess) e = hipMemcpyAsync(d_base, base.data(), nblocks * sizeof(unsigned long long), hipMemcpyHostToDevice, stream);
    if (e == hipSuccess) e = hipMemcpyAsync(d_out, head, (size_t)hl, hipMemcpyHostToDevice, stream);
    const unsigned char nl = '\n';
    if (e == hipSuccess) e = hipMemcpyAsync(d_out + run, &nl, 1, hipMemcpyHostToDevice, stream);
    if (e == hipSuccess) {
        hipLaunchKernelGGL(hrt_ppm3_write_kernel, dim3(nblocks), dim3(256), 0, stream, d_frame, npix, d_len, d_base, d_out);
        e = hipGetLastError();
    }
    if (e == hipSuccess) e = hipStreamSynchronize(stream);
    (void)hipFree(d_len);
    if (d_base) (void)hipFree(d_base);
    if (e != hipSuccess) return fail(HRT_ERR_DEVICE, std::string("hrt_encode_ppm: ") + hipGetErrorString(e));
    *bytes = total;
    return HRT_OK;
}

int hrt_check_last_launch(hrt_scene *s) {
    if (!s) return fail(HRT_ERR_INVALID, "hrt_check_last_launch: NULL scene");
    if (!s->timed) return HRT_OK;
    { const int drc = use_device(s->device); if (drc != HRT_OK) return drc; }
    HIP_TRY(hipEventSynchronize(s->ev1));
    unsigned long long gave_up = 0;
    HIP_TRY(hipMemcpy(&gave_up, s->stamps + 15, sizeof(gave_up), hipMemcpyDeviceToHost));
    if (gave_up) return fail(HRT_ERR_DEVICE, "trace kernel gave up (scheduler cycle bound exceeded): the frame of the last launch is incomplete");
    return HRT_OK;
}

int hrt_last_kernel_ms(hrt_scene *s, double *ms) {
    if (!s || !ms) return fail(HRT_ERR_INVALID, "hrt_last_kernel_ms: NULL argument");
    if (!s->timed) { *ms = 0.0; return HRT_OK; }
    {
        const int rc = hrt_check_last_launch(s);
        if (rc != HRT_OK) return rc;
    }
    float f = 0.f;
    HIP_TRY(hipEventElapsedTime(&f, s->ev0, s->ev1));
    *ms = (double)f;
    return HRT_OK;
}

int hrt_assemble_frame(const float *d_gathered, uint32_t tiles_per_rank_padded, uint32_t w, uint32_t h, uint32_t world,
                       float *d_frame, void *stream_) {
    if (!d_gathered || !d_frame || !w || !h || !world) return fail(HRT_ERR_INVALID, "hrt_assemble_frame: bad argument");
    if (tiles_per_rank_padded < hrt_tiles_owned(w, h, 0, world))
        return fail(HRT_ERR_INVALID, "hrt_assemble_frame: tiles_per_rank_padded too small");
    const uint32_t n = w * h;
    hipLaunchKernelGGL(hrt_assemble_kernel, dim3((n + 255) / 256), dim3(256), 0, (hipStream_t)stream_, d_gathered,
                       tiles_per_rank_padded, w, h, world, d_frame);
    HIP_TRY(hipGetLastError());
    return HRT_OK;
}

int hrt_debug_read_stamps(hrt_scene *s, uint64_t out[16]) {
    if (!s || !out) return fail(HRT_ERR_INVALID, "hrt_debug_read_stamps: NULL argument");
    { const int drc = use_device(s->device); if (drc != HRT_OK) return drc; }
    HIP_TRY(hipDeviceSynchronize());
    HIP_TRY(hipMemcpy(out, s->stamps, 16 * sizeof(uint64_t), hipMemcpyDeviceToHost));
    return HRT_OK;
}

int hrt_debug_pick_kernel(const hrt_pick_input *in, char *name, size_t cap) {
    if (!in || !name || !cap) return fail(HRT_ERR_INVALID, "hrt_debug_pick_kernel: bad argument");
    const KernelBuild *build = nullptr;
    const int rc = pick_build(*in, parse_kernel_pref(in->hrt_kernel), build);
    std::snprintf(name, cap, "%s", build ? build->name : "");
    return rc;
}

int hrt_debug_last_kernel(hrt_scene *s, char *name, size_t cap) {
    if (!s || !name || !cap) return fail(HRT_ERR_INVALID, "hrt_debug_last_kernel: bad argument");
    std::snprintf(name, cap, "%s", s->last_build ? s->last_build->name : "");
    return HRT_OK;
}

int hrt_kernel_info(hrt_stats *out) {
    if (!out) return fail(HRT_ERR_INVALID, "hrt_kernel_info: NULL argument");
    if (!g_rt.ready) return fail(HRT_ERR_STATE, "hrt_kernel_info: call hrt_init first");
    std::memset(out, 0, sizeof(*out));
    out->vgprs = (uint32_t)g_rt.attr.numRegs;
    out->lds_bytes = g_rt.lds_budget;
    return HRT_OK;
}

int hrt_render(hrt_scene *s, const hrt_camera *cam, uint32_t w, uint32_t h, uint32_t spp, uint64_t seed, uint32_t flags,
               float *out_rgb, hrt_stats *stats) {
    if (!out_rgb) return fail(HRT_ERR_INVALID, "hrt_render: NULL output");
    int rc = enter_render("hrt_render", s, cam);
    if (rc != HRT_OK) return rc;
    const auto t0 = std::chrono::steady_clock::now();
    const size_t tiles = hrt_tiles_total(w, h), frame_bytes = (size_t)w * h * 3 * sizeof(float);
    if ((rc = s->tiles.grow(tiles * 64 * 3 * sizeof(float))) != HRT_OK || (rc = s->frame.grow(frame_bytes)) != HRT_OK) return rc;
    rc = hrt_render_tiles(s, cam, w, h, spp, seed, flags, 0, 1, s->tiles.as<float>(), nullptr);
    if (rc != HRT_OK) return rc;
    rc = hrt_assemble_frame(s->tiles.as<float>(), (uint32_t)tiles, w, h, 1, s->frame.as<float>(), nullptr);
    if (rc != HRT_OK) return rc;
    HIP_TRY(hipMemcpy(out_rgb, s->frame.p, frame_bytes, hipMemcpyDeviceToHost));
    rc = hrt_check_last_launch(s);
    if (rc != HRT_OK) return rc;
    if (stats) {
        double ms = 0.0;
        rc = hrt_last_kernel_ms(s, &ms);
        if (rc != HRT_OK) return rc;
        fill_stats(s, stats, t0, ms, (uint64_t)w * h * spp);
    }
    return HRT_OK;
}

int hrt_render_aov(hrt_scene *s, const hrt_camera *cam, uint32_t w, uint32_t h, uint32_t which, float *out_rgb) {
    if (!out_rgb || which > 3u) return fail(HRT_ERR_INVALID, "hrt_render_aov: bad argument");
    DRender R;
    DCamera C;
    int rc = enter_render("hrt_render_aov", s, cam);
    if (rc == HRT_OK) rc = fill_render(s, cam, w, h, 1, 0, 0, 0, 1, R, C);
    if (rc != HRT_OK) return rc;
    HIP_TRY(hipMemcpy(s->d_cam_aov, &C, sizeof(C), hipMemcpyHostToDevice));
    R.cam = s->d_cam_aov;
    float *d = nullptr;
    const size_t bytes = (size_t)w * h * 3 * sizeof(float);
    HIP_TRY(hipMalloc((void **)&d, bytes));
    hipLaunchKernelGGL(hrt_aov_kernel, dim3((w * h + 255) / 256), dim3(256), 0, 0, R, which, d);
    hipError_t e = hipGetLastError();
    if (e == hipSuccess) e = hipMemcpy(out_rgb, d, bytes, hipMemcpyDeviceToHost);
    (void)hipFree(d);
    if (e != hipSuccess) return fail(HRT_ERR_DEVICE, std::string("hrt_render_aov: ") + hipGetErrorString(e));
    return HRT_OK;
}

int hrt_debug_path_stream(uint64_t seed, uint32_t pixel, uint32_t sample, uint32_t n, float *out) {
    if (!out || !n) return fail(HRT_ERR_INVALID, "hrt_debug_path_stream: bad argument");
    if (!g_rt.ready) return fail(HRT_ERR_STATE, "hrt_debug_path_stream: call hrt_init first");
    float *d = nullptr;
    HIP_TRY(hipMalloc((void **)&d, n * sizeof(float)));
    hipLaunchKernelGGL(hrt_stream_kernel, dim3(1), dim3(64), 0, 0, (uint32_t)seed, (uint32_t)(seed >> 32), pixel, sample, n, d);
    hipError_t e = hipGetLastError();
    if (e == hipSuccess) e = hipMemcpy(out, d, n * sizeof(float), hipMemcpyDeviceToHost);
    (void)hipFree(d);
    if (e != hipSuccess) return fail(HRT_ERR_DEVICE, std::string("hrt_debug_path_stream: ") + hipGetErrorString(e));
    return HRT_OK;
}

int hrt_debug_kat(uint32_t which, const hrt_camera *cam, const float *prim, const float *in, uint32_t n, float *out) {
    if (!g_rt.ready) return fail(HRT_ERR_STATE, "hrt_debug_kat: call hrt_init first");
    if (!in || !out || !n) return fail(HRT_ERR_INVALID, "hrt_debug_kat: bad argument");
    static const uint32_t in_w[] = {2, 7, 7, 7, 7, 8, 3}, out_w[] = {12, 8, 2, 9, 8, 8, 3};
    if (which > HRT_KAT_NORMALIZE) return fail(HRT_ERR_INVALID, "hrt_debug_kat: unknown instrument");
    if ((which == HRT_KAT_CAMERA) != (cam != nullptr) || ((which >= HRT_KAT_TRIANGLE && which <= HRT_KAT_QUAD) != (prim != nullptr)))
        return fail(HRT_ERR_INVALID, "hrt_debug_kat: cam is for HRT_KAT_CAMERA, prim for the primitive instruments");
    std::vector<float4> rows, kat_qf;
    std::vector<float> box;
    float err_abs = 0.f;
    DCamera C;
    DScene kat_scene{};
    float4 *d_qf = nullptr;
    DScene *d_scene = nullptr;
    if (which == HRT_KAT_CAMERA) {
        const int rc = make_camera(cam, C);
        if (rc != HRT_OK) return rc;
    } else if (which == HRT_KAT_TRIANGLE) {
        const H3 c[3] = {{prim[0], prim[1], prim[2]}, {prim[3], prim[4], prim[5]}, {prim[6], prim[7], prim[8]}};
        std::vector<float4> rest;
        fold_triangle(c, 0u, rest, rows);
        rows.insert(rows.end(), rest.begin(), rest.end());
    } else if (which == HRT_KAT_AABB) {
        box.assign(prim, prim + 6);
    } else if (which == HRT_KAT_SPHERE) {
        rows.push_back(make_float4(prim[0], prim[1], prim[2], prim[3]));
        rows.push_back(make_float4(prim[4], prim[5], prim[6], as_float(0u)));
    } else if (which == HRT_KAT_QUAD) {
        hrt_quad q;
        std::memset(&q, 0, sizeof(q));
        hrt_material m;
        std::memset(&m, 0, sizeof(m));
        for (int k = 0; k < 3; ++k) { q.v0[k] = prim[k]; q.v1[k] = prim[3 + k]; q.v3[k] = prim[6 + k]; m.motion[k] = prim[9 + k]; }
        m.type = prim[12] != 0.f ? HRT_MAT_GLASS : HRT_MAT_DIFFUSE;
        fold_quad(q, m, rows);
        build_quad_filter(rows, 1u, kat_qf, kat_scene.qf_n);
        double b = 0.0;
        for (int k = 0; k < 13; ++k) b = std::max(b, (double)std::fabs(prim[k]));
        for (size_t k = 0; k < (size_t)n * 7; ++k) if (k % 7 < 3) b = std::max(b, (double)std::fabs(in[k]));
        err_abs = margin_scale((float)(b * 4.0), 0.f);
    }
    void *d_prim = nullptr;
    float *d_in = nullptr, *d_out = nullptr;
    hipError_t e = hipSuccess;
    const size_t in_bytes = (size_t)n * in_w[which] * sizeof(float), out_bytes = (size_t)n * out_w[which] * sizeof(float);
    const void *h_prim = which == HRT_KAT_CAMERA ? (const void *)&C : (which == HRT_KAT_AABB ? (const void *)box.data() : (const void *)rows.data());
    const size_t prim_bytes = which == HRT_KAT_CAMERA ? sizeof(C) : (which == HRT_KAT_AABB ? 6 * sizeof(float) : rows.size() * sizeof(float4));
    if (prim_bytes) e = hipMalloc(&d_prim, prim_bytes);
    if (e == hipSuccess && prim_bytes) e = hipMemcpy(d_prim, h_prim, prim_bytes, hipMemcpyHostToDevice);
    if (e == hipSuccess) e = hipMalloc((void **)&d_in, in_bytes);
    if (e == hipSuccess) e = hipMemcpy(d_in, in, in_bytes, hipMemcpyHostToDevice);
    if (e == hipSuccess) e = hipMalloc((void **)&d_out, out_bytes);
    if (e == hipSuccess) {
        const dim3 grid((n + 255u) / 256u), block(256);
        switch (which) {
            case HRT_KAT_CAMERA: hipLaunchKernelGGL(hrt_kat_camera_kernel, grid, block, 0, 0, (const DCamera *)d_prim, d_in, n, d_out); break;
            case HRT_KAT_TRIANGLE: hipLaunchKernelGGL(hrt_kat_triangle_kernel, grid, block, 0, 0, (const float4 *)d_prim, d_in, n, d_out); break;
            case HRT_KAT_AABB: hipLaunchKernelGGL(hrt_kat_aabb_kernel, grid, block, 0, 0, (const float *)d_prim, d_in, n, d_out); break;
            case HRT_KAT_SPHERE: hipLaunchKernelGGL(hrt_kat_sphere_kernel, grid, block, 0, 0, (const float4 *)d_prim, d_in, n, d_out); break;
            case HRT_KAT_QUAD:
                e = hipMalloc((void **)&d_qf, kat_qf.size() * sizeof(float4));
                if (e == hipSuccess) e = hipMemcpy(d_qf, kat_qf.data(), kat_qf.size() * sizeof(float4), hipMemcpyHostToDevice);
                kat_scene.qfilter = d_qf;
                if (e == hipSuccess) e = hipMalloc((void **)&d_scene, sizeof(DScene));
                if (e == hipSuccess) e = hipMemcpy(d_scene, &kat_scene, sizeof(DScene), hipMemcpyHostToDevice);
                if (e == hipSuccess) hipLaunchKernelGGL(hrt_kat_quad_kernel, grid, block, 0, 0, (const float4 *)d_prim, (const DScene *)d_scene, d_in, n, err_abs, d_out);
                break;
            case HRT_KAT_OPTICS: hipLaunchKernelGGL(hrt_kat_optics_kernel, grid, block, 0, 0, d_in, n, d_out); break;
            default: hipLaunchKernelGGL(hrt_kat_normalize_kernel, grid, block, 0, 0, d_in, n, d_out); break;
        }
        if (e == hipSuccess) e = hipGetLastError();
    }
    if (e == hipSuccess) e = hipMemcpy(out, d_out, out_bytes, hipMemcpyDeviceToHost);
    if (d_qf) (void)hipFree(d_qf);
    if (d_scene) (void)hipFree(d_scene);
    if (d_prim) (void)hipFree(d_prim);
    if (d_in) (void)hipFree(d_in);
    if (d_out) (void)hipFree(d_out);
    if (e != hipSuccess) return fail(HRT_ERR_DEVICE, std::string("hrt_debug_kat: ") + hipGetErrorString(e));
    return HRT_OK;
}

int hrt_write_ppm(const char *path, const float *rgb, uint32_t w, uint32_t h) {
    if (!path || !rgb) return fail(HRT_ERR_INVALID, "hrt_write_ppm: NULL argument");
    FILE *f = std::fopen(path, "wb");
    if (!f) return fail(HRT_ERR_IO, std::string("Could not open file: ") + path);
    std::fprintf(f, "P3\n%u %u\n255\n", w, h);
    const size_t n = (size_t)w * h;
    for (size_t i = 0; i < n; ++i) {
        int c[3];
        for (int k = 0; k < 3; ++k) c[k] = (int)(255.f * std::min<float>(1.f, rgb[3 * i + k]));
        std::fprintf(f, "%d %d %d ", c[0], c[1], c[2]);
    }
    std::fprintf(f, "\n");
    std::fclose(f);
    return HRT_OK;
}

#include "hrt_multi.hip"
#include "hrt_adaptive.hip"
#include "hrt_denoise.hip"
#include "hrt_temporal.hip"
#include "hrt_rays.hip"
#include "hrt_radiance.hip"
#include "hrt_views.hip"

int hrt_kd_build_gpu(const hrt_kd_build_input *in, hrt_kd_build_output *out, void *user) {
    (void)user;
    if (!in || !out || (in->n_refs && (!in->ids || !in->lo || !in->hi))) return fail(HRT_ERR_INVALID, "hrt_kd_build_gpu: bad argument");
    if (!g_rt.ready) return fail(HRT_ERR_STATE, "hrt_kd_build_gpu: call hrt_init first");
    std::memset(out, 0, sizeof(*out));
    {
        const int drc = use_device(g_rt.device);
        if (drc != HRT_OK) return drc;
    }
    try {
        return kd_build_gpu_impl(in, out);
    } catch (const std::exception &e) {
        return fail(HRT_ERR_STATE, std::string("hrt_kd_build_gpu: ") + e.what());
    }
}

}
```

hai719-raytracing_amd/csrc/hrt_kat.hip:

```cpp
#include "hrt_device.h"

namespace hrtk {

__device__ __forceinline__ Ray kat_ray(const float *__restrict__ rays, uint32_t i) {
    const float *r = rays + 7 * (size_t)i;
    Ray ray;
    ray.o = mk(r[0], r[1], r[2]);
    ray.d = normalize(mk(r[3], r[4], r[5]));
    ray.time = r[6];
    return ray;
}

}

extern "C" __global__ void hrt_kat_camera_kernel(const DCamera *cam, const float *__restrict__ uv, uint32_t n, float *__restrict__ out) {
    const uint32_t i = blockIdx.x * blockDim.x + threadIdx.x;
    if (i >= n) return;
    const Ray a = camera_ray<false>((ccam)cam, uv[2 * i], uv[2 * i + 1], 0.f);
    const Ray b = camera_ray<true>((ccam)cam, uv[2 * i], uv[2 * i + 1], 0.f);
    float *o = out + 12 * (size_t)i;
    o[0] = a.o.x; o[1] = a.o.y; o[2] = a.o.z; o[3] = a.d.x; o[4] = a.d.y; o[5] = a.d.z;
    o[6] = b.o.x; o[7] = b.o.y; o[8] = b.o.z; o[9] = b.d.x; o[10] = b.d.y; o[11] = b.d.z;
}

extern "C" __global__ void hrt_kat_triangle_kernel(const float4 *rows, const float *__restrict__ rays, uint32_t n, float *__restrict__ out) {
    const uint32_t i = blockIdx.x * blockDim.x + threadIdx.x;
    if (i >= n) return;
    const Ray ray = kat_ray(rays, i);
    float t = HRT_FLT_MAX, u1 = 0.f, u2 = 0.f;
    const float4 r3 = ld((gf4)rows, 0);
    const bool hit = tri_test_plane((gf4)rows + 1, r3, ray, t, u1, u2);
    float *o = out + 8 * (size_t)i;
    o[0] = hit ? 1.f : 0.f; o[1] = hit ? t : 0.f;
    o[2] = hit ? 1 - u1 - u2 : 0.f; o[3] = hit ? u1 : 0.f; o[4] = hit ? u2 : 0.f;
    o[5] = hit ? r3.x : 0.f; o[6] = hit ? r3.y : 0.f; o[7] = hit ? r3.z : 0.f;
}

extern "C" __global__ void hrt_kat_aabb_kernel(const float *__restrict__ box, const float *__restrict__ rays, uint32_t n, float *__restrict__ out) {
    const uint32_t i = blockIdx.x * blockDim.x + threadIdx.x;
    if (i >= n) return;
    const Ray ray = kat_ray(rays, i);
    GateBox b;
    for (int a = 0; a < 3; ++a) { b.l[a] = box[a]; b.h[a] = box[3 + a]; }
    out[2 * i] = aabb_gate_exact(b, ray) ? 1.f : 0.f;
    out[2 * i + 1] = mesh_gate_box<false>(b, ray, ray_inv<false>(ray)) ? 1.f : 0.f;
}

extern "C" __global__ void hrt_kat_sphere_kernel(const float4 *rows, const float *__restrict__ rays, uint32_t n, float *__restrict__ out) {
    const uint32_t i = blockIdx.x * blockDim.x + threadIdx.x;
    if (i >= n) return;
    const Ray ray = kat_ray(rays, i);
    const float4 r0 = ld((gf4)rows, 0), r1 = ld((gf4)rows, 1);
    float t = 0.f;
    const bool hit = sphere_t(r0, r1, ray, t);
    float *o = out + 9 * (size_t)i;
    for (int k = 0; k < 9; ++k) o[k] = 0.f;
    if (!hit) return;
    const f3 p = ray.o + t * ray.d;
    const f3 nn = normalize(p - (mk(r0) + ray.time * mk(r1)));
    float theta, phi;
    sphere_angles(nn, theta, phi);
    o[0] = 1.f; o[1] = t; o[2] = theta; o[3] = phi; o[4] = nn.x; o[5] = nn.y; o[6] = nn.z; o[7] = p.x; o[8] = p.y;
}

extern "C" __global__ void hrt_kat_quad_kernel(const float4 *rows, const DScene *filter_scene, const float *__restrict__ rays, uint32_t n, float err_abs,
                                               float *__restrict__ out) {
    const uint32_t i = blockIdx.x * blockDim.x + threadIdx.x;
    if (i >= n) return;
    const Ray ray = kat_ray(rays, i);
    float t = 0.f, u = 0.f, v = 0.f;
    const bool hit = hrtk::quad_t((gf4)rows, ray, HRT_FLT_MAX, t, u, v);
    const float4 q1 = ld((gf4)rows, 1);
    Ctx cx;
    cx.S = (cscene)filter_scene; cx.tq = cx.tm = cx.ts = cx.texc = (gf4) nullptr; cx.tmesh = (gmesh) nullptr; cx.lut = (gf1) nullptr; cx.lds = (lu4) nullptr; cx.lds_n = 0; cx.err_abs = err_abs; cx.flags = 0; cx.st = nullptr;
    const uint32_t cand = quad_filter<uint32_t>(cx, ray, HRT_FLT_MAX);
    float *o = out + 8 * (size_t)i;
    o[0] = hit ? 1.f : 0.f; o[1] = hit ? t : 0.f; o[2] = hit ? u : 0.f; o[3] = hit ? v : 0.f;
    o[4] = hit ? q1.x : 0.f; o[5] = hit ? q1.y : 0.f; o[6] = hit ? q1.z : 0.f;
    o[7] = (cand & 1u) ? 1.f : 0.f;
}

extern "C" __global__ void hrt_kat_optics_kernel(const float *__restrict__ in, uint32_t n, float *__restrict__ out) {
    const uint32_t i = blockIdx.x * blockDim.x + threadIdx.x;
    if (i >= n) return;
    const float *a = in + 8 * (size_t)i;
    const f3 d = mk(a[0], a[1], a[2]), nn = mk(a[3], a[4], a[5]);
    const f3 rf = reflect(d, nn), rr = refract(d, nn, a[6]);
    float *o = out + 8 * (size_t)i;
    o[0] = rf.x; o[1] = rf.y; o[2] = rf.z; o[3] = rr.x; o[4] = rr.y; o[5] = rr.z;
    o[6] = reflectance(a[7], a[6]);
    o[7] = (float)pow((double)fabsf(a[7]), 1.0 / 2.2);
}

extern "C" __global__ void hrt_kat_normalize_kernel(const float *__restrict__ in, uint32_t n, float *__restrict__ out) {
    const uint32_t i = blockIdx.x * blockDim.x + threadIdx.x;
    if (i >= n) return;
    const f3 v = normalize(mk(in[3 * i], in[3 * i + 1], in[3 * i + 2]));
    out[3 * i] = v.x; out[3 * i + 1] = v.y; out[3 * i + 2] = v.z;
}
```

hai719-raytracing_amd/csrc/hrt_stream.hip:

```cpp
#include "hrt_device.h"

#ifndef HRT_SP_POOL
#define HRT_SP_POOL 4096
#endif
#ifndef HRT_SP_GLOBAL
#define HRT_SP_GLOBAL 1
#endif
#ifndef HRT_SP_WG
#define HRT_SP_WG 1024
#endif
#ifndef HRT_SP_MINW
#define HRT_SP_MINW 4
#endif
#define HRT_SP_SCHUNK 1024
#ifndef HRT_SP_UNIT
#define HRT_SP_UNIT 8192
#endif
#ifndef HRT_SP_UNITS
#define HRT_SP_UNITS 4
#endif
#define HRT_SP_MAXG 16
#ifndef HRT_SP_TRIPS
#define HRT_SP_TRIPS 6
#endif
#ifndef HRT_SP_TPRIO
#define HRT_SP_TPRIO 3
#endif
#ifndef HRT_SP_VOTE
#define HRT_SP_VOTE 0
#endif
#ifndef HRT_SP_STEPS
#define HRT_SP_STEPS 16
#endif
#ifndef HRT_SP_CYCLE_BOUND
#define HRT_SP_CYCLE_BOUND (1u << 16)
#endif
#ifndef HRT_SP_WAIT_SECONDS
#define HRT_SP_WAIT_SECONDS 900ull
#endif
#ifndef HRT_SP_GIVEUP_AFTER
#define HRT_SP_GIVEUP_AFTER 0u
#endif
#ifndef HRT_SP_STREAMS
#define HRT_SP_STREAMS 2
#endif
#ifndef HRT_SP_NOG5
#define HRT_SP_NOG5 1
#endif
#ifndef HRT_SP_PM4
#define HRT_SP_PM4 1
#endif
#ifndef HRT_SP_PMQ
#define HRT_SP_PMQ 1
#endif
#ifndef HRT_SP_THALF
#define HRT_SP_THALF 0
#endif
#ifndef HRT_SP_DEFER
#define HRT_SP_DEFER 1
#endif
#ifndef HRT_SP_PRUNE
#define HRT_SP_PRUNE 3
#endif
#define HRT_SP_QCAP (HRT_SP_POOL / HRT_SP_STREAMS)
#define HRT_SP_NQ 8

namespace hrtk {

enum { SP_OX = 0, SP_OY, SP_OZ, SP_DX, SP_DY, SP_DZ, SP_HT, SP_HID, SP_HA0, SP_HA1, SP_HTRI, SP_PM,
       SP_WREF, SP_WTE, SP_WKK, SP_WBT, SP_WTRI, SP_WBU, SP_WBV, SP_PAD,
       SP_TM, SP_K0, SP_K1, SP_N,
       SP_TR, SP_TG, SP_TB, SP_RR, SP_RG, SP_RB, SP_RI, SP_REM,
       SP_FIELDS };

struct SpCtl {
    uint32_t cQ[6][2];
    uint32_t cursor;
    uint32_t ngen, gen_n0;
    uint32_t gen_slot, gen_s0;
    uint32_t red_slot;
    uint32_t red_j, red_s0, red_ns;
    uint32_t more;
    uint32_t done, parity;
    uint32_t arrive;
    uint32_t ready;
    uint32_t pad[2];
};
struct SpUnit {
    uint32_t state;
    uint32_t j;
    uint32_t s0, ns;
    uint32_t gen_next, gen_total;
    uint32_t outstanding;
    uint32_t pad;
};
enum { SP_U_FREE = 0, SP_U_READY, SP_U_GENERATING, SP_U_DRAINING, SP_U_REDUCING };
struct SpShared {
    uint32_t lock;
    uint32_t cur;
    uint32_t tiles_done;
    uint32_t abort;
    uint32_t stall;
    uint32_t sections;
    uint32_t pad[2];
};
static_assert(sizeof(SpCtl) % 16 == 0 && sizeof(SpShared) % 16 == 0 && sizeof(SpUnit) % 16 == 0, "the LDS regions behind the control blocks must stay 16-byte aligned");
static_assert(HRT_SP_STREAMS == 1 || HRT_SP_STREAMS == 2, "one or two streams");
static_assert(HRT_SP_UNITS >= 1 && HRT_SP_UNITS <= 4, "a path number carries its unit slot in its two top bits");
static_assert(!HRT_SP_PMQ || (HRT_SP_PM4 && HRT_SP_POOL <= 4096), "a T-queue entry is 12 bits of slot id + 4 bits of meshes");
static_assert(!HRT_SP_NOG5 || HRT_SP_UNIT <= 8192, "g7.w keeps 13 bits of the path's number in its unit beside the bounces left");
static_assert(HRT_SP_QCAP >= 512, "deferring partial chunks needs a queue that can hold a whole chunk whenever fewer than 64 slots are free (6 queues x 63 < QCAP - 64)");

static_assert((HRT_SP_POOL & (HRT_SP_POOL - 1)) == 0 && HRT_SP_POOL <= 65536, "slot ids are 16-bit and masked with HRT_SP_POOL - 1");
static_assert((HRT_SP_GLOBAL ? 0 : SP_FIELDS * HRT_SP_POOL * 4) + HRT_SP_NQ * HRT_SP_POOL * 2 + HRT_SP_MAXG * 8 + 512 <= 160 * 1024,
              "pool + queues do not fit the CU's 160 KB of LDS (with HRT_SP_GLOBAL=0 use -DHRT_SP_POOL=1024)");

struct SpLds {
    uint32_t *st;
    uint16_t *q;
    SpCtl *ctl;
};

#if HRT_SP_GLOBAL
#define SP_AT(field, slot) ((slot) * (uint32_t)SP_FIELDS + (uint32_t)(field))
#else
#define SP_AT(field, slot) ((uint32_t)(field) * (uint32_t)HRT_SP_POOL + (slot))
#endif
#ifndef HRT_SP_NT
#define HRT_SP_NT 0
#endif
template <class T>
struct SpRef {
    T *p;
    __device__ __forceinline__ operator T() const { return (HRT_SP_NT & 1) ? __builtin_nontemporal_load(p) : *p; }
    __device__ __forceinline__ T operator=(T v) const {
        if (HRT_SP_NT & 2) __builtin_nontemporal_store(v, p);
        else *p = v;
        return v;
    }
};
__device__ __forceinline__ SpRef<float> spf(const SpLds &L, int field, uint32_t slot) { return SpRef<float>{reinterpret_cast<float *>(L.st) + SP_AT(field, slot)}; }
__device__ __forceinline__ SpRef<uint32_t> spu(const SpLds &L, int field, uint32_t slot) { return SpRef<uint32_t>{L.st + SP_AT(field, slot)}; }
__device__ __forceinline__ uint4 sp_ld4(const SpLds &L, int g, uint32_t slot) {
#if HRT_SP_GLOBAL
    const v4u v = ((gu4)(L.st + SP_AT(4 * g, slot)))[0];
    return make_uint4(v.x, v.y, v.z, v.w);
#else
    return make_uint4(L.st[SP_AT(4 * g, slot)], L.st[SP_AT(4 * g + 1, slot)], L.st[SP_AT(4 * g + 2, slot)], L.st[SP_AT(4 * g + 3, slot)]);
#endif
}
__device__ __forceinline__ void sp_st4(const SpLds &L, int g, uint32_t slot, uint4 v) {
#if HRT_SP_GLOBAL
    v4u w;
    w.x = v.x; w.y = v.y; w.z = v.z; w.w = v.w;
    *((v4u __attribute__((address_space(1))) *)(L.st + SP_AT(4 * g, slot))) = w;
#else
    L.st[SP_AT(4 * g, slot)] = v.x; L.st[SP_AT(4 * g + 1, slot)] = v.y; L.st[SP_AT(4 * g + 2, slot)] = v.z; L.st[SP_AT(4 * g + 3, slot)] = v.w;
#endif
}
#define SP_PIN1(g) "+v"(g.x), "+v"(g.y), "+v"(g.z), "+v"(g.w)
#if HRT_SP_NOG5
__device__ __forceinline__ uint32_t sp_w7(uint32_t left, uint32_t pnum) { return left | ((pnum & 0x1FFFu) << 3) | (pnum & 0xC0000000u); }
__device__ __forceinline__ uint32_t sp_w7_left(uint32_t w) { return w & 7u; }
__device__ __forceinline__ uint32_t sp_w7_pnum(uint32_t w) { return ((w >> 3) & 0x1FFFu) | (w & 0xC0000000u); }
#else
__device__ __forceinline__ uint32_t sp_w7(uint32_t left, uint32_t) { return left; }
__device__ __forceinline__ uint32_t sp_w7_left(uint32_t w) { return w; }
#endif
__device__ __forceinline__ uint4 sp_pack(float a, float b, float c, float d) { return make_uint4(__float_as_uint(a), __float_as_uint(b), __float_as_uint(c), __float_as_uint(d)); }
__device__ __forceinline__ void sp_unpack_ray_hit(const uint4 g0, const uint4 g1, const uint4 g2, Ray &ray, Hit &h, uint32_t &pm) {
    ray.o = mk(__uint_as_float(g0.x), __uint_as_float(g0.y), __uint_as_float(g0.z));
    ray.d = mk(__uint_as_float(g0.w), __uint_as_float(g1.x), __uint_as_float(g1.y));
    h.t = __uint_as_float(g1.z); h.kind = g1.w >> 28; h.index = g1.w & 0x0FFFFFFFu;
    h.a0 = __uint_as_float(g2.x); h.a1 = __uint_as_float(g2.y); h.tri = g2.z; pm = g2.w;
}
__device__ __forceinline__ void sp_store_ray_hit(const SpLds &L, uint32_t slot, const Ray &ray, const Hit &h, uint32_t pm) {
    sp_st4(L, 0, slot, sp_pack(ray.o.x, ray.o.y, ray.o.z, ray.d.x));
    sp_st4(L, 1, slot, make_uint4(__float_as_uint(ray.d.y), __float_as_uint(ray.d.z), __float_as_uint(h.t), (h.kind << 28) | h.index));
    sp_st4(L, 2, slot, make_uint4(__float_as_uint(h.a0), __float_as_uint(h.a1), h.tri, pm));
}
__device__ __forceinline__ uint16_t *spq(const SpLds &L, int which, uint32_t parity) { return L.q + (2 * which + parity) * HRT_SP_QCAP; }

#define SP_TO_NONE 6u
__device__ __forceinline__ void sp_push_all(const SpLds &L, SpCtl &C, uint32_t out, uint32_t to, uint32_t slot) {
    uint32_t rank = 0, count = 0, leader = 0;
#pragma unroll
    for (uint32_t q = 0; q < 6u; ++q) {
        const uint64_t m = __ballot(to == q);
        if (to == q) {
            rank = __builtin_amdgcn_mbcnt_hi((uint32_t)(m >> 32), __builtin_amdgcn_mbcnt_lo((uint32_t)m, 0u));
            count = (uint32_t)__popcll(m);
            leader = (uint32_t)__builtin_ctzll(m | (1ull << 63));
        }
    }
    uint32_t base = 0;
    if (to < SP_TO_NONE && rank == 0u) base = atomicAdd(&C.cQ[to][out], count);
    base = __shfl(base, (int)leader);
    if (to < SP_TO_NONE) {
        const uint32_t pos = base + rank;
        const uint32_t buf = to == 0u ? 0u : (to == 5u ? 3u : ((to == 2u || to == 3u) ? 1u : 2u));
        const bool back = to == 3u || to == 4u;
        spq(L, (int)buf, out)[back ? (uint32_t)HRT_SP_QCAP - 1u - pos : pos] = (uint16_t)slot;
    }
}

template <bool LIGHTS, bool EXACT = false, bool SPHF = false, bool LIST = false, bool VIEWS = false>
__device__ __forceinline__ void stream_body(const DRender &R) {
    extern __shared__ uint4 s_raw[];
    SpLds L;
#if HRT_SP_GLOBAL
    L.st = R.sp_pool + (size_t)blockIdx.x * ((size_t)SP_FIELDS * HRT_SP_POOL);
    L.q = reinterpret_cast<uint16_t *>(s_raw);
#else
    L.st = reinterpret_cast<uint32_t *>(s_raw);
    L.q = reinterpret_cast<uint16_t *>(L.st + SP_FIELDS * HRT_SP_POOL);
#endif
    L.ctl = reinterpret_cast<SpCtl *>(L.q + HRT_SP_NQ * HRT_SP_POOL);
    SpShared &SH = *reinterpret_cast<SpShared *>(L.ctl + HRT_SP_STREAMS);
    SpUnit *const U = reinterpret_cast<SpUnit *>(&SH + 1);
    uint32_t *tile_xy = reinterpret_cast<uint32_t *>(U + HRT_SP_UNITS);
    uint4 *tile_vw = reinterpret_cast<uint4 *>(tile_xy + HRT_SP_UNITS * HRT_SP_MAXG);
    float *s_lut = VIEWS ? reinterpret_cast<float *>(tile_vw + HRT_SP_UNITS * HRT_SP_MAXG)
                         : reinterpret_cast<float *>(tile_xy + HRT_SP_UNITS * HRT_SP_MAXG);
    float4 *s_tabs = reinterpret_cast<float4 *>(s_lut + 512);
    CtxT<EXACT, true, SPHF> cx;
    cx.S = (cscene)R.scene;
    const uint32_t tab_rows = cx.S->tab_rows;
    uint4 *s_units = reinterpret_cast<uint4 *>(s_tabs + tab_rows);
    cx.set_tables((lf4)s_tabs, (lf1)s_lut, cx.S);
    cx.lds = (lu4)s_units;
    cx.lds_n = R.lds_units;
    cx.err_abs = R.err_abs;
    cx.flags = R.flags;
    unsigned long long stamps_local[17];
    cx.st = stamps_local;
#ifdef HRT_WALK_SEG
    {
        unsigned long long *wseg = reinterpret_cast<unsigned long long *>(s_units + R.lds_units) + (threadIdx.x >> 6) * 16u;
        if ((threadIdx.x & 63u) < 16u) wseg[threadIdx.x & 63u] = 0ull;
        cx.st = wseg;
    }
#endif
    ccam cam = (ccam)R.cam;
    const uint32_t tid = threadIdx.x, lane = tid & 63u;
    {
        gu4 g_units = (gu4)cx.S->kd_units;
        for (uint32_t i = tid; i < cx.lds_n; i += HRT_SP_WG) s_units[i] = ld(g_units, i);
        gf4 g_tabs = (gf4)cx.S->tabs;
        for (uint32_t i = tid; i < tab_rows; i += HRT_SP_WG) s_tabs[i] = ld(g_tabs, i);
        if (tid < 512u) s_lut[tid] = c_u8_lut[tid];
    }
    uint16_t *const q_all = L.q;
    if (tid < HRT_SP_STREAMS) {
        SpCtl &C0 = L.ctl[tid];
        C0.cQ[0][0] = C0.cQ[0][1] = 0;
        for (int k = 0; k < 4; ++k) C0.cQ[1 + k][0] = C0.cQ[1 + k][1] = 0;
        C0.cQ[5][0] = HRT_SP_QCAP; C0.cQ[5][1] = 0;
        C0.parity = 1; C0.done = 0; C0.arrive = 0; C0.ready = 0; C0.cursor = 0; C0.ngen = 0; C0.gen_n0 = 0; C0.gen_slot = 0; C0.gen_s0 = 0;
        C0.red_slot = HRT_SP_UNITS; C0.red_j = 0; C0.red_s0 = 0; C0.red_ns = 0; C0.more = 1;
        if (tid == 0) {
            SH.lock = 0; SH.cur = 0; SH.tiles_done = 0; SH.abort = 0; SH.stall = 0; SH.sections = 0;
            for (int k = 0; k < HRT_SP_UNITS; ++k) { U[k].state = SP_U_FREE; U[k].j = 0; U[k].s0 = 0; U[k].ns = 0; U[k].gen_next = 0; U[k].gen_total = 0; U[k].outstanding = 0; }
        }
    }
    for (uint32_t i = tid; i < HRT_SP_POOL; i += HRT_SP_WG)
        q_all[(i / HRT_SP_QCAP) * (HRT_SP_NQ * HRT_SP_QCAP) + (2 * 3 + 0) * HRT_SP_QCAP + (i % HRT_SP_QCAP)] = (uint16_t)i;
    const bool has_mesh = cx.S->n_meshes != 0u;
    const bool multi_mesh = cx.S->n_meshes > 1u;
#if HRT_SP_PMQ
    const bool pm_in_entry = cx.S->n_meshes <= 4u;
#endif
    const bool prune = !EXACT && HRT_SP_PRUNE != 0 && cx.S->prune_ok != 0u;
    const bool moving = cx.S->any_motion != 0u;
    const bool sky_is_zero = cx.S->skybox_image < 0 && cx.S->dark_sky != 0;
    float *scratch = R.sp_scratch + (size_t)blockIdx.x * ((size_t)HRT_SP_UNITS * HRT_SP_UNIT * 3u);
    const uint32_t glog = R.sp_group_log2, G = 1u << glog, blog = R.sp_band_log2;
    const uint32_t upix = (64u << glog) >> blog, upix_log2 = 6u + glog - blog;
    const uint32_t items = R.tiles_owned << blog;
    auto view_row = [&](uint32_t pnum) { return tile_vw[(pnum >> 30) * HRT_SP_MAXG + (((pnum & 0x3FFFFFFFu) & (upix - 1u)) >> 6)]; };
#define SP_UNI(x) __builtin_amdgcn_readfirstlane(x)

#ifndef HRT_SP_SEG_KIND
#define HRT_SP_SEG_KIND 1
#endif
#ifdef HRT_SP_SEG
    unsigned long long seg[10] = {0, 0, 0, 0, 0, 0, 0, 0, 0, 0}, seg_last = 0;
    bool seg_on = false;
#define SEG_START(on) do { seg_on = (on); if (seg_on) { asm volatile("s_waitcnt vmcnt(0) lgkmcnt(0)" ::: "memory"); seg_last = __builtin_readcyclecounter(); } } while (0)
#define SEG(k) do { if (seg_on) { asm volatile("s_waitcnt vmcnt(0) lgkmcnt(0)" ::: "memory"); const unsigned long long t_ = __builtin_readcyclecounter(); \
                                  seg[k] += t_ - seg_last; seg_last = t_; } } while (0)
#else
#define SEG_START(on) do { } while (0)
#define SEG(k) do { } while (0)
#endif
#ifdef HRT_SP_DEBUG
    unsigned long long dbg_work = 0, dbg_chunks = 0, dbg_cycles = 0, dbg_serial = 0, dbg_wait = 0, dbg_drain = 0, dbg_tail = 0, dbg_tail_cycles = 0;
    unsigned long long dbg_class[6] = {0, 0, 0, 0, 0, 0};
    const unsigned long long dbg_t0 = __builtin_readcyclecounter();
#endif
    const uint32_t per_fold = min((uint32_t)HRT_SP_SCHUNK, (uint32_t)HRT_SP_UNIT / upix);
    auto serial_section = [&](SpCtl &C, uint16_t *qs) {
        const uint32_t par = SP_UNI(C.parity) ^ 1u;
        const uint32_t free_in = SP_UNI(C.cQ[5][par]);
#if HRT_SP_DEFER
        const uint32_t want = free_in & ~63u;
#else
        const uint32_t want = free_in;
#endif
        if (lane == 0) {
            uint32_t spins = 0;
            while (atomicCAS(&SH.lock, 0u, 1u) != 0u) {
                __builtin_amdgcn_s_sleep(1);
                if (++spins > (1u << 22)) {
                    if (R.stamps) { __hip_atomic_store(R.stamps + 15, 0xDEADull, __ATOMIC_RELAXED, __HIP_MEMORY_SCOPE_SYSTEM); R.stamps[14] = 1; }
                    __hip_atomic_store(&SH.abort, 1u, __ATOMIC_RELAXED, __HIP_MEMORY_SCOPE_WORKGROUP);
                    break;
                }
            }
            const uint32_t rs = C.red_slot;
            if (rs < HRT_SP_UNITS) {
                SpUnit &u = U[rs];
                const uint32_t s_next = u.s0 + u.ns;
                if (s_next < R.spp) {
                    u.s0 = s_next; u.ns = min(per_fold, R.spp - s_next); u.gen_next = 0; u.gen_total = upix * u.ns; u.state = SP_U_READY;
                } else {
                    u.state = SP_U_FREE;
                }
            }
            uint32_t red = HRT_SP_UNITS;
            for (uint32_t k = 0; k < HRT_SP_UNITS; ++k)
                if (red == HRT_SP_UNITS && U[k].state == SP_U_DRAINING && __hip_atomic_load(&U[k].outstanding, __ATOMIC_RELAXED, __HIP_MEMORY_SCOPE_WORKGROUP) == 0u) {
                    red = k;
                    U[k].state = SP_U_REDUCING;
                }
            C.red_slot = red;
            if (red < HRT_SP_UNITS) { C.red_j = U[red].j; C.red_s0 = U[red].s0; C.red_ns = U[red].ns; }
            uint32_t ngen = 0, n0 = 0, gs = 0;
            if (want != 0u) {
                uint32_t cur = SH.cur;
                if (U[cur].state != SP_U_GENERATING) {
                    cur = HRT_SP_UNITS;
                    for (uint32_t k = 0; k < HRT_SP_UNITS; ++k)
                        if (cur == HRT_SP_UNITS && U[k].state == SP_U_READY) cur = k;
                    if (cur == HRT_SP_UNITS && SH.tiles_done == 0u)
                        for (uint32_t k = 0; k < HRT_SP_UNITS; ++k)
                            if (cur == HRT_SP_UNITS && U[k].state == SP_U_FREE) {
                                const uint32_t j = atomicAdd(R.tile_counter, G);
                                if (j >= items) { SH.tiles_done = 1u; break; }
                                SpUnit &u = U[k];
                                u.j = j; u.s0 = 0; u.ns = min(per_fold, R.spp); u.gen_next = 0; u.gen_total = upix * u.ns;
                                __hip_atomic_store(&u.outstanding, 0u, __ATOMIC_RELAXED, __HIP_MEMORY_SCOPE_WORKGROUP);
                                for (uint32_t t = 0; t < G; ++t) {
                                    uint32_t xy = 0xFFFFFFFFu;
                                    if (j + t < items) {
                                        const uint32_t tile = VIEWS ? ((j + t) >> blog) % R.tiles_total : R.rank + rank_slot<LIST>(R, (j + t) >> blog) * R.world, band = (j + t) & ((1u << blog) - 1u);
                                        xy = ((tile % R.tiles_x) * 8u) | (((tile / R.tiles_x) * 8u + band * (8u >> blog)) << 16);
                                    }
                                    tile_xy[k * HRT_SP_MAXG + t] = xy;
                                    if (VIEWS) {
                                        const uint32_t view = j + t < items ? ((j + t) >> blog) / R.tiles_total : 0u;
                                        const DView *V = R.views + view;
                                        tile_vw[k * HRT_SP_MAXG + t] = make_uint4(view, V->seed_lo, V->seed_hi, __float_as_uint(V->err_abs));
                                    }
                                }
                                cur = k;
                            }
                    if (cur < HRT_SP_UNITS) { U[cur].state = SP_U_GENERATING; SH.cur = cur; }
                }
                if (cur < HRT_SP_UNITS) {
                    SpUnit &u = U[cur];
                    n0 = u.gen_next;
                    ngen = min(want, u.gen_total - n0);
                    u.gen_next = n0 + ngen;
                    atomicAdd(&u.outstanding, ngen);
                    if (u.gen_next == u.gen_total) u.state = SP_U_DRAINING;
                    gs = cur;
                }
            }
            bool generating = false, idle = SH.tiles_done != 0u;
            for (uint32_t k = 0; k < HRT_SP_UNITS; ++k) {
                generating = generating || U[k].state == SP_U_READY || U[k].state == SP_U_GENERATING || (U[k].state == SP_U_FREE && SH.tiles_done == 0u);
                idle = idle && U[k].state == SP_U_FREE;
            }
            C.ngen = ngen; C.gen_n0 = n0; C.gen_slot = gs; C.gen_s0 = U[gs].s0;
            C.more = generating ? 1u : 0u;
            C.done = idle ? 1u : 0u;
            uint32_t entries = ngen + (red < HRT_SP_UNITS ? 1u : 0u);
            for (int q = 0; q < 5; ++q) entries += (HRT_SP_DEFER && generating) ? (C.cQ[q][par] & ~63u) : C.cQ[q][par];
            const uint32_t stalled = entries != 0u ? (SH.stall = 0u) : ++SH.stall;
            const uint32_t sections = ++SH.sections;
            if (stalled > HRT_SP_CYCLE_BOUND || (HRT_SP_GIVEUP_AFTER != 0u && sections > HRT_SP_GIVEUP_AFTER)) {
                if (R.stamps) {
                    __hip_atomic_store(R.stamps + 15, 0xDEADull, __ATOMIC_RELAXED, __HIP_MEMORY_SCOPE_SYSTEM);
                    R.stamps[14] = 2;
                    for (uint32_t k = 0; k < HRT_SP_UNITS; ++k) R.stamps[8 + k] = ((unsigned long long)U[k].state << 48) | ((unsigned long long)U[k].outstanding << 24) | U[k].gen_next;
                    R.stamps[12] = ((unsigned long long)SH.tiles_done << 32) | SH.cur; R.stamps[13] = ((unsigned long long)want << 32) | C.cQ[0][par];
                }
                __hip_atomic_store(&SH.abort, 1u, __ATOMIC_RELAXED, __HIP_MEMORY_SCOPE_WORKGROUP);
            }
            __hip_atomic_store(&SH.lock, 0u, __ATOMIC_RELEASE, __HIP_MEMORY_SCOPE_WORKGROUP);
        }
        asm volatile("s_waitcnt lgkmcnt(0)" ::: "memory");
        const uint32_t ngen = SP_UNI(C.ngen);
        uint16_t *qFi = qs + (2 * 3 + par) * HRT_SP_QCAP, *qFo = qs + (2 * 3 + (par ^ 1u)) * HRT_SP_QCAP;
        for (uint32_t i = lane; i < free_in - ngen; i += 64u) qFo[i] = qFi[ngen + i];
        const bool defer = HRT_SP_DEFER && SP_UNI(C.more) != 0u;
        const uint32_t cT = SP_UNI(C.cQ[0][par]), rT = defer ? (cT & 63u) : 0u;
        if (lane < rT) qs[(2 * 0 + (par ^ 1u)) * HRT_SP_QCAP + lane] = qs[(2 * 0 + par) * HRT_SP_QCAP + cT - rT + lane];
        uint32_t cKv[4], rK[4], waiting = cT;
#pragma unroll
        for (int k = 0; k < 4; ++k) {
            cKv[k] = SP_UNI(C.cQ[1 + k][par]);
            rK[k] = defer ? (cKv[k] & 63u) : 0u;
            waiting += cKv[k];
            const int which = (k == 1 || k == 2) ? 1 : 2;
            const bool back = !(k == 1 || k == 0);
            const uint16_t *qi = qs + (2 * which + par) * HRT_SP_QCAP;
            uint16_t *qo = qs + (2 * which + (par ^ 1u)) * HRT_SP_QCAP;
            if (lane < rK[k]) {
                const uint32_t e = cKv[k] - rK[k] + lane;
                qo[back ? (uint32_t)HRT_SP_QCAP - 1u - lane : lane] = qi[back ? (uint32_t)HRT_SP_QCAP - 1u - e : e];
            }
        }
        if (lane == 0) {
#pragma unroll
            for (int k = 0; k < 4; ++k) { C.cQ[1 + k][par] = cKv[k] - rK[k]; C.cQ[1 + k][par ^ 1u] = rK[k]; }
            C.cQ[0][par] = cT - rT;
            C.cQ[0][par ^ 1u] = rT;
            C.cQ[5][par ^ 1u] = free_in - ngen;
            C.cursor = 0; C.parity = par;
            C.done = (C.done != 0u && ngen == 0u && waiting == 0u && C.red_slot == HRT_SP_UNITS) ? 1u : 0u;
        }
        asm volatile("s_waitcnt lgkmcnt(0)" ::: "memory");
        if (lane == 0) __hip_atomic_store(&C.ready, C.ready + 1u, __ATOMIC_RELEASE, __HIP_MEMORY_SCOPE_WORKGROUP);
    };
    __syncthreads();
    if (tid < 64u)
        for (uint32_t st = 0; st < HRT_SP_STREAMS; ++st) serial_section(L.ctl[st], q_all + st * (HRT_SP_NQ * HRT_SP_QCAP));
    __syncthreads();
    uint32_t fin[HRT_SP_UNITS];
    for (int k = 0; k < HRT_SP_UNITS; ++k) fin[k] = 0u;

    uint32_t kcyc[HRT_SP_STREAMS], fin_mask = 0u;
    for (uint32_t st = 0; st < HRT_SP_STREAMS; ++st) kcyc[st] = 1u;
    for (uint32_t round = 0;; ++round) {
        const uint32_t st = HRT_SP_STREAMS == 1 ? 0u : (round & 1u);
        if (fin_mask == (1u << HRT_SP_STREAMS) - 1u) break;
        if (fin_mask & (1u << st)) continue;
        SpCtl &C = L.ctl[st];
        L.q = q_all + st * (HRT_SP_NQ * HRT_SP_QCAP);
        {
#ifdef HRT_SP_DEBUG
            const unsigned long long dbg_q0 = __builtin_readcyclecounter();
#endif
            uint32_t spins = 0, aborted = 0;
            const unsigned long long wait_t0 = __builtin_amdgcn_s_memrealtime();
            while (SP_UNI(__hip_atomic_load(&C.ready, __ATOMIC_ACQUIRE, __HIP_MEMORY_SCOPE_WORKGROUP)) < kcyc[st]) {
                __builtin_amdgcn_s_sleep(8);
                aborted = SP_UNI(__hip_atomic_load(&SH.abort, __ATOMIC_RELAXED, __HIP_MEMORY_SCOPE_WORKGROUP));
                if (aborted) break;
                if ((++spins & 1023u) == 0u && (spins >> 10) > 16u && __builtin_amdgcn_s_memrealtime() - wait_t0 > 100000000ull * HRT_SP_WAIT_SECONDS) {
                    if (lane == 0) {
                        if (R.stamps) { __hip_atomic_store(R.stamps + 15, 0xDEADull, __ATOMIC_RELAXED, __HIP_MEMORY_SCOPE_SYSTEM); R.stamps[14] = 3; }
                        __hip_atomic_store(&SH.abort, 1u, __ATOMIC_RELAXED, __HIP_MEMORY_SCOPE_WORKGROUP);
                    }
                    aborted = 1u;
                    break;
                }
            }
#ifdef HRT_SP_DEBUG
            dbg_wait += __builtin_readcyclecounter() - dbg_q0;
#endif
            if (aborted || SP_UNI(__hip_atomic_load(&SH.abort, __ATOMIC_RELAXED, __HIP_MEMORY_SCOPE_WORKGROUP))) break;
        }
        if (SP_UNI(C.done)) { fin_mask |= 1u << st; continue; }
        const uint32_t parity = SP_UNI(C.parity);
        const uint32_t ngen = SP_UNI(C.ngen), n0 = SP_UNI(C.gen_n0), gs = SP_UNI(C.gen_slot), s0 = SP_UNI(C.gen_s0);
        const uint32_t red = SP_UNI(C.red_slot), nR = red < HRT_SP_UNITS ? (upix * 3u + 63u) >> 6 : 0u;
        const uint32_t cTin = SP_UNI(C.cQ[0][parity]);
        const uint32_t cK0 = SP_UNI(C.cQ[1][parity]), cK1 = SP_UNI(C.cQ[2][parity]), cK2 = SP_UNI(C.cQ[3][parity]),
                       cK3 = SP_UNI(C.cQ[4][parity]);
        const uint32_t nT = HRT_SP_THALF ? (cTin + 31u) >> 5 : (cTin + 63u) >> 6, e3 = nT + ((cK3 + 63u) >> 6), e1 = e3 + ((cK1 + 63u) >> 6),
                       e2 = e1 + ((cK2 + 63u) >> 6), e0 = e2 + ((cK0 + 63u) >> 6), nG = (ngen + 63u) >> 6, total = e0 + nG;
        uint16_t *qTi = spq(L, 0, parity);
        uint16_t *qAi = spq(L, 1, parity), *qBi = spq(L, 2, parity);
        uint16_t *qFi = spq(L, 3, parity);
#ifdef HRT_SP_DEBUG
        const unsigned long long dbg_w0 = __builtin_readcyclecounter();
        ++dbg_cycles;
#endif

        for (;;) {
            uint32_t c = 0;
            if (lane == 0) c = atomicAdd(&C.cursor, 1u);
            c = SP_UNI(c);
            if (c >= nR + total) break;
            if (c < nR) {
                const uint32_t i = c * 64u + lane;
                const uint32_t rj = SP_UNI(C.red_j), rs0 = SP_UNI(C.red_s0), rns = SP_UNI(C.red_ns);
                if (i < upix * 3u && rj + i / (192u >> blog) < items) {
                    float *out = R.out_tiles + (size_t)rj * (192u >> blog) + i;
                    float acc = (rs0 != 0u || R.accumulate) ? *out : 0.f;
                    const float *col = scratch + (size_t)red * ((size_t)HRT_SP_UNIT * 3u) + i;
                    const uint32_t stride = upix * 3u;
                    uint32_t sm = 0;
                    for (; sm + 8u <= rns; sm += 8u) {
                        float v[8];
#pragma unroll
                        for (int k = 0; k < 8; ++k) v[k] = col[(size_t)(sm + k) * stride];
#pragma unroll
                        for (int k = 0; k < 8; ++k) acc += v[k];
                    }
                    for (; sm < rns; ++sm) acc += col[(size_t)sm * stride];
                    if (rs0 + rns >= R.spp) {
                        const uint32_t q = i / 3u, p = q & 63u, txy = tile_xy[red * HRT_SP_MAXG + (q >> 6)];
                        const uint32_t px = (txy & 0xFFFFu) + (p & 7u), py = (txy >> 16) + (p >> 3);
                        if (!(px < R.w && py < R.h)) acc = 0.f;
                        else if (!R.accumulate) acc = acc / (float)R.spp;
                    }
                    *out = acc;
                }
                continue;
            }
            c -= nR;
#ifdef HRT_SP_DEBUG
            ++dbg_chunks;
            const unsigned long long dbg_c0 = __builtin_readcyclecounter();
            const uint32_t dbg_k = c < nT ? 0u : (c < e3 ? 1u : (c < e1 ? 2u : (c < e2 ? 3u : (c < e0 ? 4u : 5u))));
#endif
            if (c < nT) {
#if HRT_SP_TPRIO
                __builtin_amdgcn_s_setprio(HRT_SP_TPRIO);
#endif
                const uint32_t e = HRT_SP_THALF ? c * 32u + lane : c * 64u + lane;
                const bool act = e < cTin && (!HRT_SP_THALF || lane < 32u);
                uint32_t slot = 0, kind = 0, pm = 0, ref_in = HRT_KD_NIL, pm_before = 0;
                bool walked = false;
                Ray ray;
                ray.o = mk(0.f, 0.f, 0.f); ray.d = mk(0.f, 0.f, 1.f); ray.time = 0.f;
                Hit h;
                h.kind = 0; h.index = 0; h.t = HRT_FLT_MAX; h.tri = 0; h.a0 = 0.f; h.a1 = 0.f;
                Walk w;
                w.ref = HRT_KD_NIL; w.t_entry = 0.f; w.kk = 0xFFFFu; w.best_t = HRT_FLT_MAX; w.best_tri = 0; w.bu = 0.f; w.bv = 0.f;
                SEG_START(HRT_SP_SEG_KIND == 2);
                if (act) {
#if HRT_SP_PMQ
                    const uint32_t entry = qTi[e];
                    slot = entry & (HRT_SP_POOL - 1u);
#else
                    slot = qTi[e] & (HRT_SP_POOL - 1u);
#endif
#if HRT_SP_PM4
                    uint4 g0 = sp_ld4(L, 0, slot), g1 = sp_ld4(L, 1, slot), g3 = sp_ld4(L, 3, slot), g4 = sp_ld4(L, 4, slot);
                    asm volatile("" : SP_PIN1(g0), SP_PIN1(g1), SP_PIN1(g3), SP_PIN1(g4));
                    {
                        const uint4 z = make_uint4(0u, 0u, 0u, 0u);
                        sp_unpack_ray_hit(g0, g1, z, ray, h, pm);
                    }
                    pm = g4.w;
                    pm_before = __float_as_uint(h.t);
#else
                    uint4 g0 = sp_ld4(L, 0, slot), g1 = sp_ld4(L, 1, slot), g2 = sp_ld4(L, 2, slot), g3 = sp_ld4(L, 3, slot),
                          g4 = sp_ld4(L, 4, slot);
#if HRT_SP_GLOBAL
                    asm volatile("" : SP_PIN1(g0), SP_PIN1(g1), SP_PIN1(g2), SP_PIN1(g3), SP_PIN1(g4));
#endif
                    sp_unpack_ray_hit(g0, g1, g2, ray, h, pm);
                    pm_before = pm;
#endif
#if HRT_SP_PM4
                    w.ref = g4.x; w.t_entry = __uint_as_float(g3.y); w.kk = g3.z; w.best_t = __uint_as_float(g3.w);
                    w.best_tri = g3.x; w.bu = __uint_as_float(g4.y); w.bv = __uint_as_float(g4.z);
#else
                    w.ref = g3.x; w.t_entry = __uint_as_float(g3.y); w.kk = g3.z; w.best_t = __uint_as_float(g3.w);
                    w.best_tri = g4.x; w.bu = __uint_as_float(g4.y); w.bv = __uint_as_float(g4.z);
#endif
#if HRT_SP_PMQ
                    if (pm_in_entry && (entry >> 12) != 0u) { w.ref = HRT_KD_NIL; pm = entry >> 12; }
#endif
                    ref_in = w.ref;
                }
#ifdef HRT_SP_SEG
                asm volatile("" : "+v"(ray.o.x), "+v"(w.t_entry), "+v"(h.t));
#endif
                SEG(0);
                if (act) {
#if HRT_SP_VOTE
                    walked = walk_vote(cx, ray, pm, w, h, HRT_SP_STEPS);
#else
                    walked = multi_mesh ? walk_some_per_lane(cx, ray, pm, w, h, HRT_SP_TRIPS) : walk_some(cx, ray, pm, w, h, HRT_SP_TRIPS);
#endif
                }
                SEG(1);
                if (act) {
                    const uint32_t pm_in = pm_before;
#if HRT_SP_PM4
                    if (__float_as_uint(h.t) != pm_in) {
#else
                    if (pm != pm_in) {
#endif
                        sp_st4(L, 1, slot, make_uint4(__float_as_uint(ray.d.y), __float_as_uint(ray.d.z), __float_as_uint(h.t), (h.kind << 28) | h.index));
                        sp_st4(L, 2, slot, make_uint4(__float_as_uint(h.a0), __float_as_uint(h.a1), h.tri, pm));
                    }
#if HRT_SP_PM4
                    if (!walked) {
                        sp_st4(L, 3, slot, make_uint4(w.best_tri, __float_as_uint(w.t_entry), w.kk, __float_as_uint(w.best_t)));
                        sp_st4(L, 4, slot, make_uint4(w.ref, __float_as_uint(w.bu), __float_as_uint(w.bv), pm));
                    }
                    (void)ref_in;
#else
                    if (!walked) {
                        sp_st4(L, 3, slot, make_uint4(w.ref, __float_as_uint(w.t_entry), w.kk, __float_as_uint(w.best_t)));
                        sp_st4(L, 4, slot, make_uint4(w.best_tri, __float_as_uint(w.bu), __float_as_uint(w.bv), 0u));
                    } else if (ref_in != HRT_KD_NIL) {
                        spu(L, SP_WREF, slot) = HRT_KD_NIL;
                    }
#endif
                    kind = h.kind;
                }
#if HRT_SP_TPRIO
                __builtin_amdgcn_s_setprio(0);
#endif
                sp_push_all(L, C, parity ^ 1u, !act ? SP_TO_NONE : (walked ? 1u + kind : 0u), slot);
                SEG(2);
#ifdef HRT_SP_SEG
                if (seg_on) { seg[7] += 1; seg[6] += (unsigned long long)__popcll(__ballot(act)); seg[5] += (unsigned long long)__popcll(__ballot(act && walked)); }
#endif
            } else {
                const bool is_gen = c >= e0;
                const uint32_t first = is_gen ? e0 : (c < e3 ? nT : (c < e1 ? e3 : (c < e2 ? e1 : e2)));
                const uint32_t fill = is_gen ? ngen : (c < e3 ? cK3 : (c < e1 ? cK1 : (c < e2 ? cK2 : cK0)));
                const bool from_back = !is_gen && (c < e3 || (c >= e1 && c < e2));
                const uint16_t *qHi = (c < e3 || c >= e2) ? qBi : qAi;
                const uint32_t e = (c - first) * 64u + lane;
                const bool act = e < fill;
                uint32_t slot = 0, kind = 0, fin_unit = 0, pnum = 0;
                bool trace = false, freed = false;
                bool ended = false, last_seg = false;
                f3 rad = mk(0.f, 0.f, 0.f);
                SEG_START((HRT_SP_SEG_KIND == 1 && !is_gen && c >= e1 && c < e2) || (HRT_SP_SEG_KIND == 3 && !is_gen && c >= e3 && c < e1) ||
                          (HRT_SP_SEG_KIND == 4 && is_gen) || (HRT_SP_SEG_KIND == 5 && !is_gen && c < e3));
                Ray ray;
                ray.o = mk(0.f, 0.f, 0.f); ray.d = mk(0.f, 0.f, 1.f); ray.time = 0.f;
                if (act && is_gen) {
                    slot = qFi[e] & (HRT_SP_POOL - 1u);
                    const uint32_t n = n0 + e;
                    const uint32_t q = n & (upix - 1u), s = s0 + (n >> upix_log2);
                    const uint32_t p = q & 63u, txy = tile_xy[gs * HRT_SP_MAXG + (q >> 6)];
                    const uint32_t px = (txy & 0xFFFFu) + (p & 7u), py = (txy >> 16) + (p >> 3);
                    if (txy != 0xFFFFFFFFu && px < R.w && py < R.h) {
                        uint4 vw = make_uint4(0u, R.seed_lo, R.seed_hi, 0u);
                        if (VIEWS) { vw = view_row(n | (gs << 30)); cx.err_abs = __uint_as_float(vw.w); }
                        Rng rng;
                        rng.start(vw.y, vw.z, py * R.w + px, R.s0 + s);
                        const float u = ((float)px + rng.next()) / (float)R.w;
                        const float v = ((float)py + rng.next()) / (float)R.h;
                        const float tm = rng.next();
                        if (VIEWS) {
                            for (uint64_t todo = __ballot(1); todo != 0ull;) {
                                const uint32_t view = __builtin_amdgcn_readlane(vw.x, __builtin_ctzll(todo));
                                const bool mine = vw.x == view;
                                if (mine) ray = camera_ray<EXACT>((ccam)&((cview)R.views + view)->cam, u, v, tm);
                                todo &= ~__ballot(mine);
                            }
                        } else {
                            ray = camera_ray<EXACT>(cam, u, v, tm);
                        }
                        pnum = n | (gs << 30);
#if !HRT_SP_NOG5
                        sp_st4(L, 5, slot, make_uint4(__float_as_uint(tm), rng.k0, rng.k1, pnum));
#endif
                        sp_st4(L, 6, slot, sp_pack(1.f, 1.f, 1.f, 0.f));
                        sp_st4(L, 7, slot, make_uint4(0u, 0u, rng.i, sp_w7(6u, pnum)));
                        trace = true;
                    } else {
                        float *o = scratch + (size_t)gs * ((size_t)HRT_SP_UNIT * 3u) + (size_t)n * 3u;
                        o[0] = 0.f; o[1] = 0.f; o[2] = 0.f;
                        freed = true;
                        fin_unit = gs;
                    }
                } else if (act) {
                    slot = qHi[from_back ? (uint32_t)HRT_SP_QCAP - 1u - e : e] & (HRT_SP_POOL - 1u);
#if HRT_SP_NOG5
                    uint4 g0 = sp_ld4(L, 0, slot), g1 = sp_ld4(L, 1, slot), g2 = sp_ld4(L, 2, slot), g6 = sp_ld4(L, 6, slot), g7 = sp_ld4(L, 7, slot);
                    asm volatile("" : SP_PIN1(g0), SP_PIN1(g1), SP_PIN1(g2), SP_PIN1(g6), SP_PIN1(g7));
                    pnum = sp_w7_pnum(g7.w);
                    Rng key;
                    {
                        const uint32_t kn = pnum & 0x3FFFFFFFu, ku = pnum >> 30;
                        const uint32_t kq = kn & (upix - 1u), ks = U[ku].s0 + (kn >> upix_log2);
                        const uint32_t kxy = tile_xy[ku * HRT_SP_MAXG + (kq >> 6)];
                        const uint32_t kx = (kxy & 0xFFFFu) + (kq & 7u), ky = (kxy >> 16) + ((kq & 63u) >> 3);
                        uint4 vw = make_uint4(0u, R.seed_lo, R.seed_hi, 0u);
                        if (VIEWS) { vw = view_row(pnum); cx.err_abs = __uint_as_float(vw.w); }
                        key.start(vw.y, vw.z, ky * R.w + kx, R.s0 + ks);
                        key.i = 2u;
                    }
                    Hit h;
                    uint32_t pm_unused;
                    sp_unpack_ray_hit(g0, g1, g2, ray, h, pm_unused);
                    ray.time = moving ? key.next() : 0.f;
#else
                    uint4 g0 = sp_ld4(L, 0, slot), g1 = sp_ld4(L, 1, slot), g2 = sp_ld4(L, 2, slot), g5 = sp_ld4(L, 5, slot),
                          g6 = sp_ld4(L, 6, slot), g7 = sp_ld4(L, 7, slot);
#if HRT_SP_GLOBAL
                    asm volatile("" : SP_PIN1(g0), SP_PIN1(g1), SP_PIN1(g2), SP_PIN1(g5), SP_PIN1(g6), SP_PIN1(g7));
#endif
                    Hit h;
                    uint32_t pm_unused;
                    sp_unpack_ray_hit(g0, g1, g2, ray, h, pm_unused);
                    ray.time = __uint_as_float(g5.x);
                    pnum = g5.w;
                    if (VIEWS) cx.err_abs = __uint_as_float(view_row(pnum).w);
#endif
                    f3 thr = mk(__uint_as_float(g6.x), __uint_as_float(g6.y), __uint_as_float(g6.z));
                    rad = mk(__uint_as_float(g6.w), __uint_as_float(g7.x), __uint_as_float(g7.y));
                    int remaining = (int)sp_w7_left(g7.w);
#ifdef HRT_SP_SEG
                    asm volatile("" : "+v"(remaining), "+v"(ray.o.x), "+v"(thr.x), "+v"(rad.x));
#endif
                    SEG(0);
                    if (h.kind == 0u) {
                        rad = rad + thr * sky(cx, ray.d, remaining);
                        ended = true;
                    } else {
                        Rng rng;
#if HRT_SP_NOG5
                        rng.k0 = key.k0; rng.k1 = key.k1; rng.i = g7.z;
#else
                        rng.k0 = g5.y; rng.k1 = g5.z; rng.i = g7.z;
#endif
                        const Surface sf = shade(cx, ray, h);
                        SEG(1);
                        f3 direct = mk(0.f, 0.f, 0.f);
                        if (LIGHTS) direct = direct_light(cx, sf, ray, rng);
                        SEG(8);
                        rad = rad + thr * (direct + sf.emission);
                        thr = thr * sf.albedo;
                        scatter(sf, ray, rng);
                        SEG(2);
                        --remaining;
                        ended = (remaining == 0);
                        if ((HRT_SP_PRUNE & 1) && prune && thr.x == 0.f && thr.y == 0.f && thr.z == 0.f) ended = true;
                        if (!ended) {
                            sp_st4(L, 6, slot, sp_pack(thr.x, thr.y, thr.z, rad.x));
                            sp_st4(L, 7, slot, make_uint4(__float_as_uint(rad.y), __float_as_uint(rad.z), rng.i, sp_w7((uint32_t)remaining, pnum)));
                            trace = true;
                            last_seg = (HRT_SP_PRUNE & 2) && !LIGHTS && prune && remaining == 1;
                        }
                    }
                }
                bool to_mesh = false;
                SEG(3);
                Hit hn;
                hn.kind = 0; hn.index = 0; hn.t = HRT_FLT_MAX; hn.tri = 0; hn.a0 = 0.f; hn.a1 = 0.f;
                uint32_t pmn = 0;
                if (trace) {
                    hn = prims_hit(cx, ray);
                    SEG(4);
                    pmn = has_mesh ? mesh_gates(cx, ray) : 0u;
                    SEG(5);
                }
                if (SPHF && trace && hn.kind == 0u && pmn == 0u) {
                    f3 thr = mk(1.f, 1.f, 1.f);
                    int remaining = 6;
                    if (!is_gen) {
                        const uint4 g6 = sp_ld4(L, 6, slot), g7 = sp_ld4(L, 7, slot);
                        thr = mk(__uint_as_float(g6.x), __uint_as_float(g6.y), __uint_as_float(g6.z));
                        rad = mk(__uint_as_float(g6.w), __uint_as_float(g7.x), __uint_as_float(g7.y));
                        remaining = (int)sp_w7_left(g7.w);
                    }
                    rad = rad + thr * sky(cx, ray.d, remaining);
                    trace = false; ended = true; last_seg = false;
                }
                if (last_seg) {
                    bool dead;
                    if (hn.kind == 0u) {
                        dead = sky_is_zero;
                    } else {
                        const uint32_t mat = hn.kind == 1u ? __float_as_uint(ld(cx.ts, HRT_SPHERE_ROWS * hn.index + 1u).w)
                                                           : __float_as_uint(ld(cx.tq, HRT_QUAD_ROWS * hn.index + 4u).w);
                        dead = __float_as_uint(ld(cx.tm, HRT_MAT_ROWS * mat + 1u).w) == 0u;
                    }
                    if (dead) { trace = false; ended = true; }
                }
                if (ended) {
                    const uint32_t n = min(pnum & 0x3FFFFFFFu, (uint32_t)HRT_SP_UNIT - 1u);
                    fin_unit = pnum >> 30;
                    float *o = scratch + (size_t)fin_unit * ((size_t)HRT_SP_UNIT * 3u) + (size_t)n * 3u;
                    o[0] = rad.x / 6.f; o[1] = rad.y / 6.f; o[2] = rad.z / 6.f;
                    freed = true;
                }
                if (trace) {
                    sp_store_ray_hit(L, slot, ray, hn, pmn);
#if HRT_SP_PM4
#if HRT_SP_PMQ
                    if (!pm_in_entry)
#endif
                    if (pmn != 0u) sp_st4(L, 4, slot, make_uint4(HRT_KD_NIL, 0u, 0u, pmn));
#else
                    if (is_gen) spu(L, SP_WREF, slot) = HRT_KD_NIL;
#endif
                    to_mesh = pmn != 0u;
                    kind = hn.kind;
                }
#if HRT_SP_PMQ
                sp_push_all(L, C, parity ^ 1u, trace ? (to_mesh ? 0u : 1u + kind) : (freed ? 5u : SP_TO_NONE), (trace && to_mesh && pm_in_entry) ? (slot | (pmn << 12)) : slot);
#else
                sp_push_all(L, C, parity ^ 1u, trace ? (to_mesh ? 0u : 1u + kind) : (freed ? 5u : SP_TO_NONE), slot);
#endif
#pragma unroll
                for (uint32_t k = 0; k < HRT_SP_UNITS; ++k) fin[k] += (uint32_t)__popcll(__ballot(freed && fin_unit == k));
                SEG(6);
#ifdef HRT_SP_SEG
                if (seg_on) seg[7] += 1;
#endif
            }
#ifdef HRT_SP_DEBUG
            dbg_class[dbg_k] += __builtin_readcyclecounter() - dbg_c0;
#endif
        }
#ifdef HRT_SP_DEBUG
        dbg_work += __builtin_readcyclecounter() - dbg_w0;
        if (ngen == 0u) { dbg_tail += __builtin_readcyclecounter() - dbg_w0; ++dbg_tail_cycles; }
#endif
        asm volatile("s_waitcnt vmcnt(0) lgkmcnt(0)" ::: "memory");
        if (lane == 0) {
#pragma unroll
            for (uint32_t k = 0; k < HRT_SP_UNITS; ++k)
                if (fin[k]) atomicSub(&U[k].outstanding, fin[k]);
        }
#pragma unroll
        for (uint32_t k = 0; k < HRT_SP_UNITS; ++k) fin[k] = 0u;
        uint32_t arrived = 0;
        if (lane == 0) arrived = __hip_atomic_fetch_add(&C.arrive, 1u, __ATOMIC_ACQ_REL, __HIP_MEMORY_SCOPE_WORKGROUP);
        arrived = SP_UNI(arrived);
#ifdef HRT_SP_DEBUG
        const unsigned long long dbg_s0 = __builtin_readcyclecounter();
#endif
        if (arrived + 1u == (HRT_SP_WG / 64u) * kcyc[st]) serial_section(C, L.q);
#ifdef HRT_SP_DEBUG
        dbg_serial += __builtin_readcyclecounter() - dbg_s0;
#endif
        ++kcyc[st];
    }
    L.q = q_all;
    __syncthreads();
    if (SP_UNI(__hip_atomic_load(&SH.abort, __ATOMIC_RELAXED, __HIP_MEMORY_SCOPE_WORKGROUP))) return;

#ifdef HRT_SP_SEG
    if (lane == 0 && R.stamps)
        for (int k = 0; k < 9; ++k) atomicAdd(R.stamps + k, seg[k]);
#endif
#ifdef HRT_WALK_SEG
    if (lane == 0 && R.stamps)
        for (int k = 0; k < 12; ++k) atomicAdd(R.stamps + k, cx.st[k]);
#endif
#ifdef HRT_SP_DEBUG
    if (lane == 0 && R.stamps) {
        atomicAdd(R.stamps + 0, dbg_work); atomicAdd(R.stamps + 1, __builtin_readcyclecounter() - dbg_t0);
        atomicAdd(R.stamps + 2, dbg_cycles); atomicAdd(R.stamps + 3, dbg_chunks); atomicAdd(R.stamps + 4, dbg_serial);
        for (int k = 0; k < 6; ++k) atomicAdd(R.stamps + 5 + k, dbg_class[k]);
        atomicAdd(R.stamps + 11, dbg_wait); atomicAdd(R.stamps + 12, dbg_drain); atomicAdd(R.stamps + 13, dbg_tail); atomicAdd(R.stamps + 14, dbg_tail_cycles);
    }
#endif
#undef SP_UNI
}

}

extern "C" __global__ void __launch_bounds__(HRT_SP_WG, HRT_SP_MINW) hrt_wgstream_kernel(const DRender R) { hrtk::stream_body<false>(R); }
extern "C" __global__ void __launch_bounds__(HRT_SP_WG, HRT_SP_MINW) hrt_wgstream_kernel_lights(const DRender R) { hrtk::stream_body<true>(R); }
extern "C" __global__ void __launch_bounds__(HRT_SP_WG, HRT_SP_MINW) hrt_wgstream_kernel_sph(const DRender R) { hrtk::stream_body<false, false, true>(R); }
extern "C" __global__ void __launch_bounds__(HRT_SP_WG, HRT_SP_MINW) hrt_wgstream_kernel_lights_sph(const DRender R) { hrtk::stream_body<true, false, true>(R); }
extern "C" __global__ void __launch_bounds__(HRT_SP_WG, HRT_SP_MINW) hrt_wgstream_kernel_exact(const DRender R) { hrtk::stream_body<false, true>(R); }
extern "C" __global__ void __launch_bounds__(HRT_SP_WG, HRT_SP_MINW) hrt_wgstream_kernel_lights_exact(const DRender R) { hrtk::stream_body<true, true>(R); }
extern "C" __global__ void __launch_bounds__(HRT_SP_WG, HRT_SP_MINW) hrt_wgstream_kernel_list(const DRender R) { hrtk::stream_body<false, false, false, true>(R); }
extern "C" __global__ void __launch_bounds__(HRT_SP_WG, HRT_SP_MINW) hrt_wgstream_kernel_lights_list(const DRender R) { hrtk::stream_body<true, false, false, true>(R); }
extern "C" __global__ void __launch_bounds__(HRT_SP_WG, HRT_SP_MINW) hrt_wgstream_kernel_sph_list(const DRender R) { hrtk::stream_body<false, false, true, true>(R); }
extern "C" __global__ void __launch_bounds__(HRT_SP_WG, HRT_SP_MINW) hrt_wgstream_kernel_lights_sph_list(const DRender R) { hrtk::stream_body<true, false, true, true>(R); }
extern "C" __global__ void __launch_bounds__(HRT_SP_WG, HRT_SP_MINW) hrt_wgstream_kernel_exact_list(const DRender R) { hrtk::stream_body<false, true, false, true>(R); }
extern "C" __global__ void __launch_bounds__(HRT_SP_WG, HRT_SP_MINW) hrt_wgstream_kernel_lights_exact_list(const DRender R) { hrtk::stream_body<true, true, false, true>(R); }
extern "C" __global__ void __launch_bounds__(HRT_SP_WG, HRT_SP_MINW) hrt_wgstream_kernel_views(const DRender R) { hrtk::stream_body<false, false, false, false, true>(R); }
extern "C" __global__ void __launch_bounds__(HRT_SP_WG, HRT_SP_MINW) hrt_wgstream_kernel_lights_views(const DRender R) { hrtk::stream_body<true, false, false, false, true>(R); }
extern "C" __global__ void __launch_bounds__(HRT_SP_WG, HRT_SP_MINW) hrt_wgstream_kernel_sph_views(const DRender R) { hrtk::stream_body<false, false, true, false, true>(R); }
extern "C" __global__ void __launch_bounds__(HRT_SP_WG, HRT_SP_MINW) hrt_wgstream_kernel_lights_sph_views(const DRender R) { hrtk::stream_body<true, false, true, false, true>(R); }
```

include/hrt.h:

```cpp
#ifndef HRT_H
#define HRT_H

#include <stddef.h>
#include <stdint.h>

#ifdef __cplusplus
extern "C" {
#endif

#define HRT_API __attribute__((visibility("default")))

#define HRT_MAXBOUNCES 6
#define HRT_NB_ECH 10
#define HRT_EPSILON 0.00001
#define HRT_TRIANGLE_SCALING 1.000001f

typedef enum hrt_status {
    HRT_OK = 0,
    HRT_ERR_INVALID = -1,
    HRT_ERR_DEVICE = -2,
    HRT_ERR_STATE = -3,
    HRT_ERR_IO = -4
} hrt_status;

enum { HRT_MAT_DIFFUSE = 0, HRT_MAT_GLASS = 1, HRT_MAT_MIRROR = 2 };
enum { HRT_TEX_NONE = 0, HRT_TEX_CHECKER = 1, HRT_TEX_IMAGE = 2 };
enum { HRT_COLOR_VERTEX = 0, HRT_COLOR_FACE = 1, HRT_COLOR_NONE = 2 };

typedef struct hrt_material {
    float albedo[3];
    float transparency;
    float index_medium;
    int32_t type;
    int32_t texture_type;
    float checker1[3];
    float checker2[3];
    float tex_scale_x, tex_scale_y;
    int32_t emissive;
    float light_color[3];
    float light_intensity;
    int32_t image;
    int32_t normal_map;
    float motion[3];
} hrt_material;

typedef struct hrt_image {
    int32_t w, h;
    const uint8_t *rgb;
} hrt_image;

typedef struct hrt_sphere {
    float center[3];
    float radius;
    int32_t material;
} hrt_sphere;

typedef struct hrt_quad {
    float v0[3], v1[3], v3[3];
    float tangent[3], bitangent[3];
    int32_t material;
} hrt_quad;

typedef struct hrt_light {
    float pos[3];
    float radius;
    float color[3];
} hrt_light;

#define HRT_KD_LEAF 0x80000000u
#define HRT_KD_NIL 0xFFFFFFFFu
typedef struct hrt_kdunit {
    uint32_t w[4];
} hrt_kdunit;

typedef struct hrt_kd_build_input {
    uint32_t n_refs;
    const uint32_t *ids;
    const float *lo, *hi;
    float cell_lo[3], cell_hi[3];
    uint32_t leaf_max, max_depth;
    float cost_traverse, cost_intersect, empty_bonus;
} hrt_kd_build_input;
typedef struct hrt_kd_build_node {
    int32_t axis;
    float split;
    int32_t left, right;
    float lo[3], hi[3];
    uint32_t first_tri, n_tris;
} hrt_kd_build_node;
typedef struct hrt_kd_build_output {
    hrt_kd_build_node *nodes;
    uint32_t n_nodes;
    uint32_t *tris;
    uint32_t n_tris;
    int32_t root;
    uint32_t depth;
} hrt_kd_build_output;
typedef int (*hrt_kd_builder_fn)(const hrt_kd_build_input *in, hrt_kd_build_output *out, void *user);

typedef struct hrt_tri_exception {
    uint32_t triangle;
    float box_min[3], box_max[3];
    uint32_t group;
} hrt_tri_exception;

typedef struct hrt_mesh {
    uint32_t n_vertices, n_triangles;
    const float *positions;
    const uint32_t *indices;
    int32_t color_type;
    const float *vert_colors;
    const float *face_colors;
    float aabb_min[3], aabb_max[3];
    int32_t material;
    uint32_t kd_root;
    float kd_min[3], kd_max[3];
    uint32_t n_kd_units;
    const hrt_kdunit *kd_units;
    uint32_t n_leaf_tris;
    const uint32_t *leaf_tris;
    uint32_t n_exceptions;
    const hrt_tri_exception *exceptions;
} hrt_mesh;

typedef struct hrt_scene_desc {
    uint32_t n_materials;  const hrt_material *materials;
    uint32_t n_spheres;    const hrt_sphere *spheres;
    uint32_t n_quads;      const hrt_quad *quads;
    uint32_t n_meshes;     const hrt_mesh *meshes;
    uint32_t n_lights;     const hrt_light *lights;
    uint32_t n_images;     const hrt_image *images;
    int32_t dark_sky;
    int32_t skybox_image;
} hrt_scene_desc;

typedef struct hrt_camera {
    float eye[3];
    float right[3], up[3], forward[3];
    float fovy_deg;
    float aspect;
    float znear, zfar;
} hrt_camera;

#define HRT_TILE 8

enum {
    HRT_FLAG_GAMMA = 1u,
    HRT_FLAG_NO_LDS_TREE = 2u,
    HRT_FLAG_WAVE_KERNEL = 4u,
    HRT_FLAG_STREAM_KERNEL = 8u,
    HRT_FLAG_NO_SHADOW_CULL = 16u,
    HRT_FLAG_DUAL_KERNEL = 32u,
    HRT_FLAG_EXACT_ONLY = 64u,
    HRT_FLAG_MESH_BRUTE = 128u
};

typedef struct hrt_stats {
    double kernel_ms;
    double total_ms;
    uint64_t samples;
    uint32_t vgprs, sgprs, lds_bytes, waves_launched;
} hrt_stats;

typedef struct hrt_scene hrt_scene;

HRT_API int hrt_init(int device_ordinal);
HRT_API void hrt_shutdown(void);
HRT_API const char *hrt_last_error(void);
HRT_API int hrt_device_count(void);

HRT_API int hrt_scene_create(const hrt_scene_desc *desc, hrt_scene **out);
HRT_API void hrt_scene_destroy(hrt_scene *scene);

HRT_API int hrt_render(hrt_scene *scene, const hrt_camera *cam, uint32_t w, uint32_t h,
               uint32_t spp, uint64_t seed, uint32_t flags, float *out_rgb,
               hrt_stats *stats );

typedef struct hrt_multi hrt_multi;
HRT_API int hrt_multi_create(const hrt_scene_desc *desc, uint32_t n_devices, const int *device_ordinals, hrt_multi **out);
HRT_API int hrt_multi_render(hrt_multi *m, const hrt_camera *cam, uint32_t w, uint32_t h, uint32_t spp, uint64_t seed,
                     uint32_t flags, float *out_rgb, hrt_stats *stats );
HRT_API void hrt_multi_destroy(hrt_multi *m);
HRT_API const char *hrt_multi_gather(const hrt_multi *m);
HRT_API int hrt_render_multi(const hrt_scene_desc *desc, const hrt_camera *cam, uint32_t w, uint32_t h, uint32_t spp,
                     uint64_t seed, uint32_t flags, uint32_t n_devices, const int *device_ordinals, float *out_rgb,
                     hrt_stats *stats );

HRT_API uint32_t hrt_tiles_total(uint32_t w, uint32_t h);
HRT_API uint32_t hrt_tiles_owned(uint32_t w, uint32_t h, uint32_t rank, uint32_t world);
HRT_API int hrt_render_tiles(hrt_scene *scene, const hrt_camera *cam, uint32_t w,
                     uint32_t h, uint32_t spp, uint64_t seed, uint32_t flags,
                     uint32_t rank, uint32_t world,
                     float *d_tiles ,
                     void *stream);
HRT_API int hrt_assemble_frame(const float *d_gathered, uint32_t tiles_per_rank_padded,
                       uint32_t w, uint32_t h, uint32_t world,
                       float *d_frame , void *stream);
HRT_API int hrt_check_last_launch(hrt_scene *scene);
HRT_API int hrt_last_kernel_ms(hrt_scene *scene, double *ms);
HRT_API int hrt_kernel_info(hrt_stats *out);

HRT_API int hrt_render_aov(hrt_scene *scene, const hrt_camera *cam, uint32_t w, uint32_t h,
                   uint32_t which, float *out_rgb);
HRT_API int hrt_debug_path_stream(uint64_t seed, uint32_t pixel, uint32_t sample, uint32_t n, float *out);

enum { HRT_KAT_CAMERA = 0, HRT_KAT_TRIANGLE = 1, HRT_KAT_AABB = 2, HRT_KAT_SPHERE = 3, HRT_KAT_QUAD = 4, HRT_KAT_OPTICS = 5,
       HRT_KAT_NORMALIZE = 6 };
HRT_API int hrt_debug_kat(uint32_t which, const hrt_camera *cam, const float *prim, const float *in, uint32_t n, float *out);

HRT_API int hrt_debug_read_stamps(hrt_scene *scene, uint64_t out[16]);

typedef struct hrt_pick_input {
    uint32_t n_meshes, n_lights, n_spheres, tab_rows;
    uint32_t tiles, spp;
    uint32_t flags, has_list, n_views;
    const char *hrt_kernel;
} hrt_pick_input;
HRT_API int hrt_debug_pick_kernel(const hrt_pick_input *in, char *name, size_t cap);
HRT_API int hrt_debug_last_kernel(hrt_scene *scene, char *name, size_t cap);

HRT_API int hrt_kd_build_gpu(const hrt_kd_build_input *in, hrt_kd_build_output *out, void *user);

HRT_API int hrt_write_ppm(const char *path, const float *rgb, uint32_t w, uint32_t h);

HRT_API int hrt_render_accumulate(hrt_scene *scene, const hrt_camera *cam, uint32_t w, uint32_t h,
                          uint32_t first_sample, uint32_t n_samples, uint64_t seed, uint32_t flags,
                          uint32_t rank, uint32_t world, float *d_sum_tiles, void *stream);
HRT_API int hrt_finalize_tiles(const float *d_sum_tiles, uint32_t n_tiles, uint32_t total_samples, uint32_t flags,
                       float *d_tiles, void *stream);
typedef struct hrt_adaptive {
    uint32_t min_spp, max_spp;
    float threshold;
} hrt_adaptive;
HRT_API int hrt_render_adaptive_tiles(hrt_scene *scene, const hrt_camera *cam, uint32_t w, uint32_t h, const hrt_adaptive *params,
                                      uint64_t seed, uint32_t flags, uint32_t rank, uint32_t world, float *d_tiles,
                                      uint32_t *d_tile_spp, void *stream);
HRT_API int hrt_render_adaptive(hrt_scene *scene, const hrt_camera *cam, uint32_t w, uint32_t h, const hrt_adaptive *params,
                                uint64_t seed, uint32_t flags, float *out_rgb, uint32_t *out_tile_spp, hrt_stats *stats);

#define HRT_FEATURE_FLOATS 12
HRT_API int hrt_render_features(hrt_scene *scene, const hrt_camera *cam, uint32_t w, uint32_t h, uint32_t first_sample, uint32_t n_samples, uint64_t seed, float *d_features, void *stream);
typedef struct hrt_denoise_params {
    uint32_t iterations;
    float sigma_color, sigma_normal, sigma_albedo, sigma_depth;
} hrt_denoise_params;
HRT_API size_t hrt_denoise_scratch_bytes(uint32_t w, uint32_t h);
HRT_API int hrt_denoise(const float *d_color, const float *d_features, uint32_t w, uint32_t h, const hrt_denoise_params *p, uint32_t flags, void *d_scratch, float *d_out, void *stream);
HRT_API int hrt_render_denoised(hrt_scene *scene, const hrt_camera *cam, uint32_t w, uint32_t h, uint32_t spp, uint32_t feature_spp, uint64_t seed, uint32_t flags, const hrt_denoise_params *p, float *out_rgb, hrt_stats *stats);

typedef struct hrt_denoise_var_params {
    uint32_t iterations;
    uint32_t prefilter;
    float sigma_variance, sigma_normal, sigma_albedo, sigma_depth;
    float variance_floor;
} hrt_denoise_var_params;
HRT_API size_t hrt_denoise_var_scratch_bytes(uint32_t w, uint32_t h);
HRT_API int hrt_denoise_var(const float *d_color, const float *d_color_half, const float *d_features, uint32_t w, uint32_t h, const hrt_denoise_var_params *p, uint32_t flags, void *d_scratch, float *d_out, float *d_variance_out, void *stream);
HRT_API int hrt_render_denoised_var(hrt_scene *scene, const hrt_camera *cam, uint32_t w, uint32_t h, uint32_t spp, uint32_t feature_spp, uint64_t seed, uint32_t flags, const hrt_denoise_var_params *p, float *out_rgb, float *out_variance, hrt_stats *stats);

typedef struct hrt_temporal_params {
    float alpha_min;
    float max_history;
    float depth_tol;
    float normal_tol;
    float albedo_tol;
} hrt_temporal_params;
HRT_API int hrt_temporal_accumulate(const hrt_camera *cam, const hrt_camera *prev_cam, uint32_t w, uint32_t h,
    const float *d_color, const float *d_color_half , const float *d_features,
    const float *d_prev_color, const float *d_prev_color_half, const float *d_prev_features, const float *d_prev_history,
    const hrt_temporal_params *p,
    float *d_out, float *d_out_half , float *d_history_out, void *stream);
typedef struct hrt_history hrt_history;
HRT_API int hrt_history_create(hrt_scene *scene, hrt_history **out);
HRT_API void hrt_history_reset(hrt_history *hist);
HRT_API void hrt_history_destroy(hrt_history *hist);
HRT_API int hrt_render_temporal(hrt_scene *scene, hrt_history *hist, const hrt_camera *cam, uint32_t w, uint32_t h,
                                uint32_t spp, uint32_t feature_spp, uint64_t seed, uint32_t flags,
                                const hrt_temporal_params *tp, const hrt_denoise_var_params *dp ,
                                float *out_rgb, float *out_history , hrt_stats *stats);

enum { HRT_QUERY_CLOSEST = 0, HRT_QUERY_SHADE = 1, HRT_QUERY_OCCLUDED = 2 };
#define HRT_RAYS_NORMALIZE 256u
#define HRT_RAY_FLOATS 8
HRT_API int hrt_trace_rays(hrt_scene *scene, const float *d_rays, uint32_t n, uint32_t mode, uint32_t flags, void *d_out, void *stream);

#define HRT_RADIANCE_ACCUMULATE 512u
HRT_API int hrt_trace_radiance(hrt_scene *scene, const float *d_rays, const uint32_t *d_keys, uint32_t n, uint32_t first_sample,
                               uint32_t n_samples, uint64_t seed, uint32_t flags, float *d_out, void *stream);
HRT_API int hrt_camera_rays(const hrt_camera *cam, uint32_t w, uint32_t h, uint32_t sample, uint64_t seed, float *d_rays, void *stream);

typedef struct hrt_view {
    hrt_camera cam;
    uint64_t seed;
} hrt_view;
#define HRT_VIEWS_MAX_TILES (1u << 24)
HRT_API int hrt_render_views_device(hrt_scene *scene, const hrt_view *views, uint32_t n_views, uint32_t w, uint32_t h,
                                    uint32_t spp, uint32_t flags, float *d_frames, void *stream);
HRT_API int hrt_render_views(hrt_scene *scene, const hrt_view *views, uint32_t n_views, uint32_t w, uint32_t h,
                             uint32_t spp, uint32_t flags, float *out_rgb, hrt_stats *stats );

HRT_API int hrt_encode_ppm(const float *d_frame, uint32_t w, uint32_t h, int format, unsigned char *d_out,
                   size_t capacity, size_t *bytes, void *stream);

#ifdef __cplusplus
}
#endif
#endif
```

Baseline: 3503.

## Compact streaming path record into a packed hit word and recompute hit UVs at shade

Shrinks the per-path state in the global streaming pool. The hit kind, index and triangle are packed into one 32-bit word, and the stored barycentrics (a0/a1) and the separate triangle field are dropped. The shade stage instead recomputes UVs for quads and triangles from the ray. This removes one 16-byte group from the trace and shade loads and stores, and it also deletes the LDS-pool, NOG5 and PM4 compile variants. The cost is extra intersection arithmetic at shade time, and soup slots are now limited to 25 bits, which adds a new validation check and a debug kernel that tests the word round trip.

```diff
diff --git a/hai719-raytracing_amd/__init__.py b/hai719-raytracing_amd/__init__.py
--- a/hai719-raytracing_amd/__init__.py
+++ b/hai719-raytracing_amd/__init__.py
@@ -635,9 +635,9 @@
             pass
 
 
-KAT_CAMERA, KAT_TRIANGLE, KAT_AABB, KAT_SPHERE, KAT_QUAD, KAT_OPTICS, KAT_NORMALIZE = range(7)
-_KAT_IN = {KAT_CAMERA: 2, KAT_TRIANGLE: 7, KAT_AABB: 7, KAT_SPHERE: 7, KAT_QUAD: 7, KAT_OPTICS: 8, KAT_NORMALIZE: 3}
-_KAT_OUT = {KAT_CAMERA: 12, KAT_TRIANGLE: 8, KAT_AABB: 2, KAT_SPHERE: 9, KAT_QUAD: 8, KAT_OPTICS: 8, KAT_NORMALIZE: 3}
+KAT_CAMERA, KAT_TRIANGLE, KAT_AABB, KAT_SPHERE, KAT_QUAD, KAT_OPTICS, KAT_NORMALIZE, KAT_HITWORD = range(8)
+_KAT_IN = {KAT_CAMERA: 2, KAT_TRIANGLE: 7, KAT_AABB: 7, KAT_SPHERE: 7, KAT_QUAD: 7, KAT_OPTICS: 8, KAT_NORMALIZE: 3, KAT_HITWORD: 3}
+_KAT_OUT = {KAT_CAMERA: 12, KAT_TRIANGLE: 8, KAT_AABB: 2, KAT_SPHERE: 9, KAT_QUAD: 8, KAT_OPTICS: 8, KAT_NORMALIZE: 3, KAT_HITWORD: 4}
 
 
 def pick_kernel(n_meshes: int, n_lights: int, n_spheres: int, tab_rows: int, tiles: int, spp: int, flags: int = 0, has_list: bool = False,
diff --git a/hai719-raytracing_amd/csrc/hrt_api.hip b/hai719-raytracing_amd/csrc/hrt_api.hip
--- a/hai719-raytracing_amd/csrc/hrt_api.hip
+++ b/hai719-raytracing_amd/csrc/hrt_api.hip
@@ -465,6 +465,13 @@
     if (D.skybox_image >= (int32_t)D.n_images) return fail(HRT_ERR_INVALID, "skybox image out of range");
     if (D.n_lights && !D.lights) return fail(HRT_ERR_INVALID, "lights missing");
     if (D.n_meshes > 32u) return fail(HRT_ERR_INVALID, "more than 32 meshes in one scene (the parked-mesh mask is 32 bits)");
+    {
+        uint64_t rows = 0;
+        for (uint32_t mi = 0; mi < D.n_meshes; ++mi) rows += (uint64_t)D.meshes[mi].n_leaf_tris + std::min(D.meshes[mi].n_exceptions, D.meshes[mi].n_triangles);
+        if (rows > (uint64_t)HRT_MAX_SOUP_SLOTS)
+            return fail(HRT_ERR_INVALID, "triangle soup of " + std::to_string(rows) + " rows (leaf triangles + irregular triangles of all meshes): more than HRT_MAX_SOUP_SLOTS = " +
+                                             std::to_string(HRT_MAX_SOUP_SLOTS) + " (a path record keeps 25 bits of soup slot)");
+    }
 
     {
         double b = 0.0;
@@ -1012,7 +1019,7 @@
 }
 
 static int size_stream(hrt_scene *s, const KernelBuild &b, DRender &R, uint32_t &grid, uint32_t &lds_bytes) {
-    const uint32_t fixed = (uint32_t)((HRT_SP_GLOBAL ? 0 : SP_FIELDS * HRT_SP_POOL * 4) + HRT_SP_NQ * HRT_SP_POOL * 2 + HRT_SP_STREAMS * sizeof(SpCtl) + sizeof(SpShared) + HRT_SP_UNITS * sizeof(SpUnit) + HRT_SP_UNITS * HRT_SP_MAXG * 4) +
+    const uint32_t fixed = (uint32_t)(HRT_SP_NQ * HRT_SP_POOL * 2 + HRT_SP_STREAMS * sizeof(SpCtl) + sizeof(SpShared) + HRT_SP_UNITS * sizeof(SpUnit) + HRT_SP_UNITS * HRT_SP_MAXG * 4) +
                            ((b.bits & KB_VIEWS) ? HRT_SP_UNITS * HRT_SP_MAXG * 16u : 0u) +
                            2048u + s->d.tab_rows * 16u
 #ifdef HRT_WALK_SEG
@@ -1035,7 +1042,7 @@
         R.sp_band_log2 = band;
     }
     int rc = s->sp_scratch.grow((size_t)grid * HRT_SP_UNITS * HRT_SP_UNIT * 3u * sizeof(float));
-    if (rc == HRT_OK && HRT_SP_GLOBAL) rc = s->sp_pool.grow((size_t)grid * SP_FIELDS * HRT_SP_POOL * sizeof(uint32_t));
+    if (rc == HRT_OK) rc = s->sp_pool.grow((size_t)grid * SP_FIELDS * HRT_SP_POOL * sizeof(uint32_t));
     if (rc != HRT_OK) return rc;
     R.sp_scratch = s->sp_scratch.as<float>();
     R.sp_pool = s->sp_pool.as<uint32_t>();
@@ -1343,8 +1350,8 @@
 int hrt_debug_kat(uint32_t which, const hrt_camera *cam, const float *prim, const float *in, uint32_t n, float *out) {
     if (!g_rt.ready) return fail(HRT_ERR_STATE, "hrt_debug_kat: call hrt_init first");
     if (!in || !out || !n) return fail(HRT_ERR_INVALID, "hrt_debug_kat: bad argument");
-    static const uint32_t in_w[] = {2, 7, 7, 7, 7, 8, 3}, out_w[] = {12, 8, 2, 9, 8, 8, 3};
-    if (which > HRT_KAT_NORMALIZE) return fail(HRT_ERR_INVALID, "hrt_debug_kat: unknown instrument");
+    static const uint32_t in_w[] = {2, 7, 7, 7, 7, 8, 3, 3}, out_w[] = {12, 8, 2, 9, 8, 8, 3, 4};
+    if (which > HRT_KAT_HITWORD) return fail(HRT_ERR_INVALID, "hrt_debug_kat: unknown instrument");
     if ((which == HRT_KAT_CAMERA) != (cam != nullptr) || ((which >= HRT_KAT_TRIANGLE && which <= HRT_KAT_QUAD) != (prim != nullptr)))
         return fail(HRT_ERR_INVALID, "hrt_debug_kat: cam is for HRT_KAT_CAMERA, prim for the primitive instruments");
     std::vector<float4> rows, kat_qf;
@@ -1408,6 +1415,7 @@
                 if (e == hipSuccess) hipLaunchKernelGGL(hrt_kat_quad_kernel, grid, block, 0, 0, (const float4 *)d_prim, (const DScene *)d_scene, d_in, n, err_abs, d_out);
                 break;
             case HRT_KAT_OPTICS: hipLaunchKernelGGL(hrt_kat_optics_kernel, grid, block, 0, 0, d_in, n, d_out); break;
+            case HRT_KAT_HITWORD: hipLaunchKernelGGL(hrt_kat_hitword_kernel, grid, block, 0, 0, d_in, n, d_out); break;
             default: hipLaunchKernelGGL(hrt_kat_normalize_kernel, grid, block, 0, 0, d_in, n, d_out); break;
         }
         if (e == hipSuccess) e = hipGetLastError();
diff --git a/hai719-raytracing_amd/csrc/hrt_kat.hip b/hai719-raytracing_amd/csrc/hrt_kat.hip
--- a/hai719-raytracing_amd/csrc/hrt_kat.hip
+++ b/hai719-raytracing_amd/csrc/hrt_kat.hip
@@ -98,3 +98,15 @@
     const f3 v = normalize(mk(in[3 * i], in[3 * i + 1], in[3 * i + 2]));
     out[3 * i] = v.x; out[3 * i + 1] = v.y; out[3 * i + 2] = v.z;
 }
+
+extern "C" __global__ void hrt_kat_hitword_kernel(const float *__restrict__ in, uint32_t n, float *__restrict__ out) {
+    const uint32_t i = blockIdx.x * blockDim.x + threadIdx.x;
+    if (i >= n) return;
+    Hit h;
+    h.kind = __float_as_uint(in[3 * i]); h.index = __float_as_uint(in[3 * i + 1]); h.tri = __float_as_uint(in[3 * i + 2]);
+    h.t = 0.f; h.a0 = 0.f; h.a1 = 0.f;
+    const uint32_t w = hrtk::sp_hit_word(h);
+    Hit g;
+    hrtk::sp_hit_unword(w, g);
+    out[4 * i] = __uint_as_float(w); out[4 * i + 1] = __uint_as_float(g.kind); out[4 * i + 2] = __uint_as_float(g.index); out[4 * i + 3] = __uint_as_float(g.tri);
+}
diff --git a/hai719-raytracing_amd/csrc/hrt_stream.hip b/hai719-raytracing_amd/csrc/hrt_stream.hip
--- a/hai719-raytracing_amd/csrc/hrt_stream.hip
+++ b/hai719-raytracing_amd/csrc/hrt_stream.hip
@@ -2,9 +2,6 @@
 
 #ifndef HRT_SP_POOL
 #define HRT_SP_POOL 4096
-#endif
-#ifndef HRT_SP_GLOBAL
-#define HRT_SP_GLOBAL 1
 #endif
 #ifndef HRT_SP_WG
 #define HRT_SP_WG 1024
@@ -44,12 +41,6 @@
 #ifndef HRT_SP_STREAMS
 #define HRT_SP_STREAMS 2
 #endif
-#ifndef HRT_SP_NOG5
-#define HRT_SP_NOG5 1
-#endif
-#ifndef HRT_SP_PM4
-#define HRT_SP_PM4 1
-#endif
 #ifndef HRT_SP_PMQ
 #define HRT_SP_PMQ 1
 #endif
@@ -67,11 +58,11 @@
 
 namespace hrtk {
 
-enum { SP_OX = 0, SP_OY, SP_OZ, SP_DX, SP_DY, SP_DZ, SP_HT, SP_HID, SP_HA0, SP_HA1, SP_HTRI, SP_PM,
-       SP_WREF, SP_WTE, SP_WKK, SP_WBT, SP_WTRI, SP_WBU, SP_WBV, SP_PAD,
-       SP_TM, SP_K0, SP_K1, SP_N,
+enum { SP_OX = 0, SP_OY, SP_OZ, SP_DX, SP_DY, SP_DZ, SP_HT, SP_HID,
        SP_TR, SP_TG, SP_TB, SP_RR, SP_RG, SP_RB, SP_RI, SP_REM,
-       SP_FIELDS };
+       SP_WTRI, SP_WTE, SP_WKK, SP_WBT, SP_WREF, SP_WBU, SP_WBV, SP_PM,
+       SP_FREE = 24,
+       SP_FIELDS = 32 };
 
 struct SpCtl {
     uint32_t cQ[6][2];
@@ -107,13 +98,12 @@
 static_assert(sizeof(SpCtl) % 16 == 0 && sizeof(SpShared) % 16 == 0 && sizeof(SpUnit) % 16 == 0, "the LDS regions behind the control blocks must stay 16-byte aligned");
 static_assert(HRT_SP_STREAMS == 1 || HRT_SP_STREAMS == 2, "one or two streams");
 static_assert(HRT_SP_UNITS >= 1 && HRT_SP_UNITS <= 4, "a path number carries its unit slot in its two top bits");
-static_assert(!HRT_SP_PMQ || (HRT_SP_PM4 && HRT_SP_POOL <= 4096), "a T-queue entry is 12 bits of slot id + 4 bits of meshes");
-static_assert(!HRT_SP_NOG5 || HRT_SP_UNIT <= 8192, "g7.w keeps 13 bits of the path's number in its unit beside the bounces left");
+static_assert(!HRT_SP_PMQ || HRT_SP_POOL <= 4096, "a T-queue entry is 12 bits of slot id + 4 bits of meshes");
+static_assert(HRT_SP_UNIT <= 8192, "g3.w keeps 13 bits of the path's number in its unit beside the bounces left");
 static_assert(HRT_SP_QCAP >= 512, "deferring partial chunks needs a queue that can hold a whole chunk whenever fewer than 64 slots are free (6 queues x 63 < QCAP - 64)");
 
 static_assert((HRT_SP_POOL & (HRT_SP_POOL - 1)) == 0 && HRT_SP_POOL <= 65536, "slot ids are 16-bit and masked with HRT_SP_POOL - 1");
-static_assert((HRT_SP_GLOBAL ? 0 : SP_FIELDS * HRT_SP_POOL * 4) + HRT_SP_NQ * HRT_SP_POOL * 2 + HRT_SP_MAXG * 8 + 512 <= 160 * 1024,
-              "pool + queues do not fit the CU's 160 KB of LDS (with HRT_SP_GLOBAL=0 use -DHRT_SP_POOL=1024)");
+static_assert(HRT_SP_NQ * HRT_SP_POOL * 2 + HRT_SP_MAXG * 8 + 512 <= 160 * 1024, "the queues do not fit the CU's 160 KB of LDS");
 
 struct SpLds {
     uint32_t *st;
@@ -121,63 +111,56 @@
     SpCtl *ctl;
 };
 
-#if HRT_SP_GLOBAL
 #define SP_AT(field, slot) ((slot) * (uint32_t)SP_FIELDS + (uint32_t)(field))
-#else
-#define SP_AT(field, slot) ((uint32_t)(field) * (uint32_t)HRT_SP_POOL + (slot))
-#endif
-#ifndef HRT_SP_NT
-#define HRT_SP_NT 0
-#endif
-template <class T>
-struct SpRef {
-    T *p;
-    __device__ __forceinline__ operator T() const { return (HRT_SP_NT & 1) ? __builtin_nontemporal_load(p) : *p; }
-    __device__ __forceinline__ T operator=(T v) const {
-        if (HRT_SP_NT & 2) __builtin_nontemporal_store(v, p);
-        else *p = v;
-        return v;
-    }
-};
-__device__ __forceinline__ SpRef<float> spf(const SpLds &L, int field, uint32_t slot) { return SpRef<float>{reinterpret_cast<float *>(L.st) + SP_AT(field, slot)}; }
-__device__ __forceinline__ SpRef<uint32_t> spu(const SpLds &L, int field, uint32_t slot) { return SpRef<uint32_t>{L.st + SP_AT(field, slot)}; }
 __device__ __forceinline__ uint4 sp_ld4(const SpLds &L, int g, uint32_t slot) {
-#if HRT_SP_GLOBAL
     const v4u v = ((gu4)(L.st + SP_AT(4 * g, slot)))[0];
     return make_uint4(v.x, v.y, v.z, v.w);
-#else
-    return make_uint4(L.st[SP_AT(4 * g, slot)], L.st[SP_AT(4 * g + 1, slot)], L.st[SP_AT(4 * g + 2, slot)], L.st[SP_AT(4 * g + 3, slot)]);
-#endif
 }
 __device__ __forceinline__ void sp_st4(const SpLds &L, int g, uint32_t slot, uint4 v) {
-#if HRT_SP_GLOBAL
     v4u w;
     w.x = v.x; w.y = v.y; w.z = v.z; w.w = v.w;
     *((v4u __attribute__((address_space(1))) *)(L.st + SP_AT(4 * g, slot))) = w;
-#else
-    L.st[SP_AT(4 * g, slot)] = v.x; L.st[SP_AT(4 * g + 1, slot)] = v.y; L.st[SP_AT(4 * g + 2, slot)] = v.z; L.st[SP_AT(4 * g + 3, slot)] = v.w;
-#endif
 }
 #define SP_PIN1(g) "+v"(g.x), "+v"(g.y), "+v"(g.z), "+v"(g.w)
-#if HRT_SP_NOG5
 __device__ __forceinline__ uint32_t sp_w7(uint32_t left, uint32_t pnum) { return left | ((pnum & 0x1FFFu) << 3) | (pnum & 0xC0000000u); }
 __device__ __forceinline__ uint32_t sp_w7_left(uint32_t w) { return w & 7u; }
 __device__ __forceinline__ uint32_t sp_w7_pnum(uint32_t w) { return ((w >> 3) & 0x1FFFu) | (w & 0xC0000000u); }
-#else
-__device__ __forceinline__ uint32_t sp_w7(uint32_t left, uint32_t) { return left; }
-__device__ __forceinline__ uint32_t sp_w7_left(uint32_t w) { return w; }
-#endif
+static_assert(HRT_MAX_SOUP_SLOTS == (1u << 25), "the hit word keeps 25 bits of soup slot");
+__device__ __forceinline__ uint32_t sp_hit_word(const Hit &h) {
+    return h.kind == 3u ? (3u << 30) | (h.index << 25) | h.tri : (h.kind << 30) | h.index;
+}
+__device__ __forceinline__ void sp_hit_unword(uint32_t w, Hit &h) {
+    h.kind = w >> 30;
+    const bool mesh = h.kind == 3u;
+    h.index = mesh ? (w >> 25) & 31u : w & 0x3FFFFFFFu;
+    h.tri = mesh ? w & 0x01FFFFFFu : 0u;
+}
 __device__ __forceinline__ uint4 sp_pack(float a, float b, float c, float d) { return make_uint4(__float_as_uint(a), __float_as_uint(b), __float_as_uint(c), __float_as_uint(d)); }
-__device__ __forceinline__ void sp_unpack_ray_hit(const uint4 g0, const uint4 g1, const uint4 g2, Ray &ray, Hit &h, uint32_t &pm) {
+__device__ __forceinline__ void sp_unpack_ray_hit(const uint4 g0, const uint4 g1, Ray &ray, Hit &h) {
     ray.o = mk(__uint_as_float(g0.x), __uint_as_float(g0.y), __uint_as_float(g0.z));
     ray.d = mk(__uint_as_float(g0.w), __uint_as_float(g1.x), __uint_as_float(g1.y));
-    h.t = __uint_as_float(g1.z); h.kind = g1.w >> 28; h.index = g1.w & 0x0FFFFFFFu;
-    h.a0 = __uint_as_float(g2.x); h.a1 = __uint_as_float(g2.y); h.tri = g2.z; pm = g2.w;
-}
-__device__ __forceinline__ void sp_store_ray_hit(const SpLds &L, uint32_t slot, const Ray &ray, const Hit &h, uint32_t pm) {
+    h.t = __uint_as_float(g1.z);
+    sp_hit_unword(g1.w, h);
+    h.a0 = 0.f; h.a1 = 0.f;
+}
+__device__ __forceinline__ uint4 sp_g1(const Ray &ray, const Hit &h) {
+    return make_uint4(__float_as_uint(ray.d.y), __float_as_uint(ray.d.z), __float_as_uint(h.t), sp_hit_word(h));
+}
+__device__ __forceinline__ void sp_store_ray_hit(const SpLds &L, uint32_t slot, const Ray &ray, const Hit &h) {
     sp_st4(L, 0, slot, sp_pack(ray.o.x, ray.o.y, ray.o.z, ray.d.x));
-    sp_st4(L, 1, slot, make_uint4(__float_as_uint(ray.d.y), __float_as_uint(ray.d.z), __float_as_uint(h.t), (h.kind << 28) | h.index));
-    sp_st4(L, 2, slot, make_uint4(__float_as_uint(h.a0), __float_as_uint(h.a1), h.tri, pm));
+    sp_st4(L, 1, slot, sp_g1(ray, h));
+}
+template <class CX>
+__device__ __forceinline__ void sp_hit_uv_square(const CX &cx, const Ray &ray, Hit &h) {
+    float t, u = 0.f, v = 0.f;
+    if (quad_t(cx.tq + HRT_QUAD_ROWS * h.index, ray, HRT_FLT_MAX, t, u, v)) { h.a0 = u; h.a1 = v; }
+}
+template <class CX>
+__device__ __forceinline__ void sp_hit_uv_triangle(const CX &cx, const Ray &ray, Hit &h) {
+    const gf4 tr = (gf4)cx.S->tris + HRT_TRI_ROWS * h.tri;
+    float u1, u2;
+    (void)tri_inside(ld(tr, 0), ld(tr, 1), ld(tr, 2), ray, h.t, u1, u2);
+    h.a0 = u1; h.a1 = u2;
 }
 __device__ __forceinline__ uint16_t *spq(const SpLds &L, int which, uint32_t parity) { return L.q + (2 * which + parity) * HRT_SP_QCAP; }
 
@@ -208,13 +191,8 @@
 __device__ __forceinline__ void stream_body(const DRender &R) {
     extern __shared__ uint4 s_raw[];
     SpLds L;
-#if HRT_SP_GLOBAL
     L.st = R.sp_pool + (size_t)blockIdx.x * ((size_t)SP_FIELDS * HRT_SP_POOL);
     L.q = reinterpret_cast<uint16_t *>(s_raw);
-#else
-    L.st = reinterpret_cast<uint32_t *>(s_raw);
-    L.q = reinterpret_cast<uint16_t *>(L.st + SP_FIELDS * HRT_SP_POOL);
-#endif
     L.ctl = reinterpret_cast<SpCtl *>(L.q + HRT_SP_NQ * HRT_SP_POOL);
     SpShared &SH = *reinterpret_cast<SpShared *>(L.ctl + HRT_SP_STREAMS);
     SpUnit *const U = reinterpret_cast<SpUnit *>(&SH + 1);
@@ -534,7 +512,7 @@
 #endif
                 const uint32_t e = HRT_SP_THALF ? c * 32u + lane : c * 64u + lane;
                 const bool act = e < cTin && (!HRT_SP_THALF || lane < 32u);
-                uint32_t slot = 0, kind = 0, pm = 0, ref_in = HRT_KD_NIL, pm_before = 0;
+                uint32_t slot = 0, kind = 0, pm = 0, t_before = 0;
                 bool walked = false;
                 Ray ray;
                 ray.o = mk(0.f, 0.f, 0.f); ray.d = mk(0.f, 0.f, 1.f); ray.time = 0.f;
@@ -550,35 +528,16 @@
 #else
                     slot = qTi[e] & (HRT_SP_POOL - 1u);
 #endif
-#if HRT_SP_PM4
-                    uint4 g0 = sp_ld4(L, 0, slot), g1 = sp_ld4(L, 1, slot), g3 = sp_ld4(L, 3, slot), g4 = sp_ld4(L, 4, slot);
-                    asm volatile("" : SP_PIN1(g0), SP_PIN1(g1), SP_PIN1(g3), SP_PIN1(g4));
-                    {
-                        const uint4 z = make_uint4(0u, 0u, 0u, 0u);
-                        sp_unpack_ray_hit(g0, g1, z, ray, h, pm);
-                    }
-                    pm = g4.w;
-                    pm_before = __float_as_uint(h.t);
-#else
-                    uint4 g0 = sp_ld4(L, 0, slot), g1 = sp_ld4(L, 1, slot), g2 = sp_ld4(L, 2, slot), g3 = sp_ld4(L, 3, slot),
-                          g4 = sp_ld4(L, 4, slot);
-#if HRT_SP_GLOBAL
-                    asm volatile("" : SP_PIN1(g0), SP_PIN1(g1), SP_PIN1(g2), SP_PIN1(g3), SP_PIN1(g4));
-#endif
-                    sp_unpack_ray_hit(g0, g1, g2, ray, h, pm);
-                    pm_before = pm;
-#endif
-#if HRT_SP_PM4
-                    w.ref = g4.x; w.t_entry = __uint_as_float(g3.y); w.kk = g3.z; w.best_t = __uint_as_float(g3.w);
-                    w.best_tri = g3.x; w.bu = __uint_as_float(g4.y); w.bv = __uint_as_float(g4.z);
-#else
-                    w.ref = g3.x; w.t_entry = __uint_as_float(g3.y); w.kk = g3.z; w.best_t = __uint_as_float(g3.w);
-                    w.best_tri = g4.x; w.bu = __uint_as_float(g4.y); w.bv = __uint_as_float(g4.z);
-#endif
+                    uint4 g0 = sp_ld4(L, 0, slot), g1 = sp_ld4(L, 1, slot), g4 = sp_ld4(L, 4, slot), g5 = sp_ld4(L, 5, slot);
+                    asm volatile("" : SP_PIN1(g0), SP_PIN1(g1), SP_PIN1(g4), SP_PIN1(g5));
+                    sp_unpack_ray_hit(g0, g1, ray, h);
+                    pm = g5.w;
+                    t_before = g1.z;
+                    w.ref = g5.x; w.t_entry = __uint_as_float(g4.y); w.kk = g4.z; w.best_t = __uint_as_float(g4.w);
+                    w.best_tri = g4.x; w.bu = __uint_as_float(g5.y); w.bv = __uint_as_float(g5.z);
 #if HRT_SP_PMQ
                     if (pm_in_entry && (entry >> 12) != 0u) { w.ref = HRT_KD_NIL; pm = entry >> 12; }
 #endif
-                    ref_in = w.ref;
                 }
 #ifdef HRT_SP_SEG
                 asm volatile("" : "+v"(ray.o.x), "+v"(w.t_entry), "+v"(h.t));
@@ -593,29 +552,11 @@
                 }
                 SEG(1);
                 if (act) {
-                    const uint32_t pm_in = pm_before;
-#if HRT_SP_PM4
-                    if (__float_as_uint(h.t) != pm_in) {
-#else
-                    if (pm != pm_in) {
-#endif
-                        sp_st4(L, 1, slot, make_uint4(__float_as_uint(ray.d.y), __float_as_uint(ray.d.z), __float_as_uint(h.t), (h.kind << 28) | h.index));
-                        sp_st4(L, 2, slot, make_uint4(__float_as_uint(h.a0), __float_as_uint(h.a1), h.tri, pm));
+                    if (__float_as_uint(h.t) != t_before) sp_st4(L, 1, slot, sp_g1(ray, h));
+                    if (!walked) {
+                        sp_st4(L, 4, slot, make_uint4(w.best_tri, __float_as_uint(w.t_entry), w.kk, __float_as_uint(w.best_t)));
+                        sp_st4(L, 5, slot, make_uint4(w.ref, __float_as_uint(w.bu), __float_as_uint(w.bv), pm));
                     }
-#if HRT_SP_PM4
-                    if (!walked) {
-                        sp_st4(L, 3, slot, make_uint4(w.best_tri, __float_as_uint(w.t_entry), w.kk, __float_as_uint(w.best_t)));
-                        sp_st4(L, 4, slot, make_uint4(w.ref, __float_as_uint(w.bu), __float_as_uint(w.bv), pm));
-                    }
-                    (void)ref_in;
-#else
-                    if (!walked) {
-                        sp_st4(L, 3, slot, make_uint4(w.ref, __float_as_uint(w.t_entry), w.kk, __float_as_uint(w.best_t)));
-                        sp_st4(L, 4, slot, make_uint4(w.best_tri, __float_as_uint(w.bu), __float_as_uint(w.bv), 0u));
-                    } else if (ref_in != HRT_KD_NIL) {
-                        spu(L, SP_WREF, slot) = HRT_KD_NIL;
-                    }
-#endif
                     kind = h.kind;
                 }
 #if HRT_SP_TPRIO
@@ -667,11 +608,8 @@
                             ray = camera_ray<EXACT>(cam, u, v, tm);
                         }
                         pnum = n | (gs << 30);
-#if !HRT_SP_NOG5
-                        sp_st4(L, 5, slot, make_uint4(__float_as_uint(tm), rng.k0, rng.k1, pnum));
-#endif
-                        sp_st4(L, 6, slot, sp_pack(1.f, 1.f, 1.f, 0.f));
-                        sp_st4(L, 7, slot, make_uint4(0u, 0u, rng.i, sp_w7(6u, pnum)));
+                        sp_st4(L, 2, slot, sp_pack(1.f, 1.f, 1.f, 0.f));
+                        sp_st4(L, 3, slot, make_uint4(0u, 0u, rng.i, sp_w7(6u, pnum)));
                         trace = true;
                     } else {
                         float *o = scratch + (size_t)gs * ((size_t)HRT_SP_UNIT * 3u) + (size_t)n * 3u;
@@ -681,10 +619,9 @@
                     }
                 } else if (act) {
                     slot = qHi[from_back ? (uint32_t)HRT_SP_QCAP - 1u - e : e] & (HRT_SP_POOL - 1u);
-#if HRT_SP_NOG5
-                    uint4 g0 = sp_ld4(L, 0, slot), g1 = sp_ld4(L, 1, slot), g2 = sp_ld4(L, 2, slot), g6 = sp_ld4(L, 6, slot), g7 = sp_ld4(L, 7, slot);
-                    asm volatile("" : SP_PIN1(g0), SP_PIN1(g1), SP_PIN1(g2), SP_PIN1(g6), SP_PIN1(g7));
-                    pnum = sp_w7_pnum(g7.w);
+                    uint4 g0 = sp_ld4(L, 0, slot), g1 = sp_ld4(L, 1, slot), g2 = sp_ld4(L, 2, slot), g3 = sp_ld4(L, 3, slot);
+                    asm volatile("" : SP_PIN1(g0), SP_PIN1(g1), SP_PIN1(g2), SP_PIN1(g3));
+                    pnum = sp_w7_pnum(g3.w);
                     Rng key;
                     {
                         const uint32_t kn = pnum & 0x3FFFFFFFu, ku = pnum >> 30;
@@ -697,25 +634,11 @@
                         key.i = 2u;
                     }
                     Hit h;
-                    uint32_t pm_unused;
-                    sp_unpack_ray_hit(g0, g1, g2, ray, h, pm_unused);
+                    sp_unpack_ray_hit(g0, g1, ray, h);
                     ray.time = moving ? key.next() : 0.f;
-#else
-                    uint4 g0 = sp_ld4(L, 0, slot), g1 = sp_ld4(L, 1, slot), g2 = sp_ld4(L, 2, slot), g5 = sp_ld4(L, 5, slot),
-                          g6 = sp_ld4(L, 6, slot), g7 = sp_ld4(L, 7, slot);
-#if HRT_SP_GLOBAL
-                    asm volatile("" : SP_PIN1(g0), SP_PIN1(g1), SP_PIN1(g2), SP_PIN1(g5), SP_PIN1(g6), SP_PIN1(g7));
-#endif
-                    Hit h;
-                    uint32_t pm_unused;
-                    sp_unpack_ray_hit(g0, g1, g2, ray, h, pm_unused);
-                    ray.time = __uint_as_float(g5.x);
-                    pnum = g5.w;
-                    if (VIEWS) cx.err_abs = __uint_as_float(view_row(pnum).w);
-#endif
-                    f3 thr = mk(__uint_as_float(g6.x), __uint_as_float(g6.y), __uint_as_float(g6.z));
-                    rad = mk(__uint_as_float(g6.w), __uint_as_float(g7.x), __uint_as_float(g7.y));
-                    int remaining = (int)sp_w7_left(g7.w);
+                    f3 thr = mk(__uint_as_float(g2.x), __uint_as_float(g2.y), __uint_as_float(g2.z));
+                    rad = mk(__uint_as_float(g2.w), __uint_as_float(g3.x), __uint_as_float(g3.y));
+                    int remaining = (int)sp_w7_left(g3.w);
 #ifdef HRT_SP_SEG
                     asm volatile("" : "+v"(remaining), "+v"(ray.o.x), "+v"(thr.x), "+v"(rad.x));
 #endif
@@ -725,11 +648,9 @@
                         ended = true;
                     } else {
                         Rng rng;
-#if HRT_SP_NOG5
-                        rng.k0 = key.k0; rng.k1 = key.k1; rng.i = g7.z;
-#else
-                        rng.k0 = g5.y; rng.k1 = g5.z; rng.i = g7.z;
-#endif
+                        rng.k0 = key.k0; rng.k1 = key.k1; rng.i = g3.z;
+                        if (h.kind == 2u) sp_hit_uv_square(cx, ray, h);
+                        else if (h.kind == 3u) sp_hit_uv_triangle(cx, ray, h);
                         const Surface sf = shade(cx, ray, h);
                         SEG(1);
                         f3 direct = mk(0.f, 0.f, 0.f);
@@ -743,8 +664,8 @@
                         ended = (remaining == 0);
                         if ((HRT_SP_PRUNE & 1) && prune && thr.x == 0.f && thr.y == 0.f && thr.z == 0.f) ended = true;
                         if (!ended) {
-                            sp_st4(L, 6, slot, sp_pack(thr.x, thr.y, thr.z, rad.x));
-                            sp_st4(L, 7, slot, make_uint4(__float_as_uint(rad.y), __float_as_uint(rad.z), rng.i, sp_w7((uint32_t)remaining, pnum)));
+                            sp_st4(L, 2, slot, sp_pack(thr.x, thr.y, thr.z, rad.x));
+                            sp_st4(L, 3, slot, make_uint4(__float_as_uint(rad.y), __float_as_uint(rad.z), rng.i, sp_w7((uint32_t)remaining, pnum)));
                             trace = true;
                             last_seg = (HRT_SP_PRUNE & 2) && !LIGHTS && prune && remaining == 1;
                         }
@@ -765,10 +686,10 @@
                     f3 thr = mk(1.f, 1.f, 1.f);
                     int remaining = 6;
                     if (!is_gen) {
-                        const uint4 g6 = sp_ld4(L, 6, slot), g7 = sp_ld4(L, 7, slot);
-                        thr = mk(__uint_as_float(g6.x), __uint_as_float(g6.y), __uint_as_float(g6.z));
-                        rad = mk(__uint_as_float(g6.w), __uint_as_float(g7.x), __uint_as_float(g7.y));
-                        remaining = (int)sp_w7_left(g7.w);
+                        const uint4 g2 = sp_ld4(L, 2, slot), g3 = sp_ld4(L, 3, slot);
+                        thr = mk(__uint_as_float(g2.x), __uint_as_float(g2.y), __uint_as_float(g2.z));
+                        rad = mk(__uint_as_float(g2.w), __uint_as_float(g3.x), __uint_as_float(g3.y));
+                        remaining = (int)sp_w7_left(g3.w);
                     }
                     rad = rad + thr * sky(cx, ray.d, remaining);
                     trace = false; ended = true; last_seg = false;
@@ -792,15 +713,11 @@
                     freed = true;
                 }
                 if (trace) {
-                    sp_store_ray_hit(L, slot, ray, hn, pmn);
-#if HRT_SP_PM4
+                    sp_store_ray_hit(L, slot, ray, hn);
 #if HRT_SP_PMQ
                     if (!pm_in_entry)
 #endif
-                    if (pmn != 0u) sp_st4(L, 4, slot, make_uint4(HRT_KD_NIL, 0u, 0u, pmn));
-#else
-                    if (is_gen) spu(L, SP_WREF, slot) = HRT_KD_NIL;
-#endif
+                    if (pmn != 0u) sp_st4(L, 5, slot, make_uint4(HRT_KD_NIL, 0u, 0u, pmn));
                     to_mesh = pmn != 0u;
                     kind = hn.kind;
                 }
diff --git a/include/hrt.h b/include/hrt.h
--- a/include/hrt.h
+++ b/include/hrt.h
@@ -123,6 +123,7 @@
     const hrt_tri_exception *exceptions;
 } hrt_mesh;
 
+#define HRT_MAX_SOUP_SLOTS (1u << 25)
 typedef struct hrt_scene_desc {
     uint32_t n_materials;  const hrt_material *materials;
     uint32_t n_spheres;    const hrt_sphere *spheres;
@@ -205,7 +206,7 @@
 HRT_API int hrt_debug_path_stream(uint64_t seed, uint32_t pixel, uint32_t sample, uint32_t n, float *out);
 
 enum { HRT_KAT_CAMERA = 0, HRT_KAT_TRIANGLE = 1, HRT_KAT_AABB = 2, HRT_KAT_SPHERE = 3, HRT_KAT_QUAD = 4, HRT_KAT_OPTICS = 5,
-       HRT_KAT_NORMALIZE = 6 };
+       HRT_KAT_NORMALIZE = 6, HRT_KAT_HITWORD = 7 };
 HRT_API int hrt_debug_kat(uint32_t which, const hrt_camera *cam, const float *prim, const float *in, uint32_t n, float *out);
 
 HRT_API int hrt_debug_read_stamps(hrt_scene *scene, uint64_t out[16]);
```

After: 3736, median of 6. +6.6%, better.
